# mikeoliphant/NeuralAudio

Measured on AMD Instinct MI355X. Metric: concurrent 48 kHz real-time streams + Msamples/s/GPU, NAM WaveNet Standard, higher is better.
Workload: dtype f32 (f16x3-split MFMA, f32 accumulate)

## Files before the change

### include/neuralaudio_amd.h

```cpp
#ifndef NEURALAUDIO_AMD_H
#define NEURALAUDIO_AMD_H

#include "NeuralAudioCApi.h"

#ifdef __cplusplus
extern "C" {
#endif

typedef struct NA_Batch NA_Batch;

NA_EXTERN const char* NA_GetLastError(void);
NA_EXTERN int NA_GetDeviceCount(void);
NA_EXTERN const char* NA_GetVersion(void);

NA_EXTERN NeuralModel* NA_CreateModelFromFileUtf8(NeuralModelLoader* loader, const char* utf8Path, int doPrewarm);
NA_EXTERN NeuralModel* NA_CreateModelFromString(NeuralModelLoader* loader, const char* jsonText, const char* extension, int doPrewarm);
NA_EXTERN void NA_SetDevice(NeuralModelLoader* loader, int device);
NA_EXTERN void NA_SetWaveNetMathMode(NeuralModelLoader* loader, int mathMode);
NA_EXTERN void NA_SetLSTMMathMode(NeuralModelLoader* loader, int mathMode);
NA_EXTERN void NA_SetCompositeModelLoadMode(NeuralModelLoader* loader, int loadMode);
NA_EXTERN int NA_IsQualityChangeRealtimeSafe(NeuralModel* model, float newQuality);
NA_EXTERN int NA_ProcessChecked(NeuralModel* model, float* input, float* output, size_t numSamples);
NA_EXTERN void NA_SetDefaultQualityScaleFactor(NeuralModelLoader* loader, float quality);
NA_EXTERN void NA_SetExternalSampleRate(NeuralModelLoader* loader, int sampleRate);
NA_EXTERN int NA_HasQualityScaling(NeuralModel* model);
NA_EXTERN float NA_GetQualityScaleFactor(NeuralModel* model);
NA_EXTERN void NA_SetQualityScaleFactor(NeuralModel* model, float quality);
NA_EXTERN int NA_GetReceptiveFieldSize(NeuralModel* model);
NA_EXTERN int NA_Prewarm(NeuralModel* model);
NA_EXTERN int NA_GetMetadata(NeuralModel* model, const char* fieldName, char* buf, int bufSize);
NA_EXTERN int NA_GetModelVersion(NeuralModel* model, char* buf, int bufSize);

NA_EXTERN NA_Batch* NA_BatchCreate(int device, void* hipStream);
NA_EXTERN void NA_BatchDestroy(NA_Batch* batch);
NA_EXTERN int NA_BatchAddStreams(NA_Batch* batch, NeuralModel* model, float quality, int count, int doPrewarm);
NA_EXTERN int NA_BatchRemoveStreams(NA_Batch* batch, int first, int count);
NA_EXTERN int NA_BatchReserveStreams(NA_Batch* batch, NeuralModel* model, int count, int doPrewarm);
NA_EXTERN int NA_BatchActivateStream(NA_Batch* batch, int stream, float quality);
NA_EXTERN int NA_BatchParkStream(NA_Batch* batch, int stream);
NA_EXTERN int NA_BatchIsParked(NA_Batch* batch, int stream);
NA_EXTERN int NA_BatchFindParked(NA_Batch* batch, NeuralModel* model);
NA_EXTERN int NA_BatchNumParked(NA_Batch* batch);
NA_EXTERN int NA_BatchEnableOutputStage(NA_Batch* batch);
NA_EXTERN int NA_BatchSetStreamGain(NA_Batch* batch, int stream, float gain, int rampSamples);
NA_EXTERN float NA_BatchGetStreamGain(NA_Batch* batch, int stream);
NA_EXTERN int NA_BatchHandover(NA_Batch* batch, int from, int to, float quality, int fadeSamples);
NA_EXTERN int NA_BatchHandoverRemaining(NA_Batch* batch, int stream);
NA_EXTERN int NA_BatchNumStreams(NA_Batch* batch);
NA_EXTERN int NA_BatchNumLiveStreams(NA_Batch* batch);
NA_EXTERN int NA_BatchIsLive(NA_Batch* batch, int stream);
NA_EXTERN int NA_BatchSetQuality(NA_Batch* batch, int stream, float quality);
NA_EXTERN int NA_BatchGetActiveSubModel(NA_Batch* batch, int stream);
NA_EXTERN int NA_BatchIsQualityChangeRealtimeSafe(NA_Batch* batch, int stream, float quality);
NA_EXTERN int NA_BatchPrewarm(NA_Batch* batch, int stream);
NA_EXTERN int NA_BatchProcess(NA_Batch* batch, const float* in, float* out, size_t n);
NA_EXTERN int NA_RegisterHostBuffer(void* ptr, size_t bytes);
NA_EXTERN int NA_UnregisterHostBuffer(void* ptr);
NA_EXTERN int NA_BatchSubmit(NA_Batch* batch, const float* in, size_t n);
NA_EXTERN int NA_BatchCollect(NA_Batch* batch, int ticket, float* out);
NA_EXTERN float* NA_BatchNextInput(NA_Batch* batch, size_t n);
NA_EXTERN const float* NA_BatchOutputView(NA_Batch* batch, int ticket);
NA_EXTERN int NA_BatchProcessDevice(NA_Batch* batch, const float* dIn, float* dOut, size_t n, long inStride, long outStride);
NA_EXTERN int NA_BatchWaitOutputs(NA_Batch* batch);
NA_EXTERN int NA_BatchSynchronize(NA_Batch* batch);
NA_EXTERN int NA_BatchSetWaitLimitMs(NA_Batch* batch, double milliseconds);
NA_EXTERN double NA_BatchGetWaitLimitMs(NA_Batch* batch);
NA_EXTERN int NA_BatchIsBroken(NA_Batch* batch);
NA_EXTERN void* NA_BatchGetHipStream(NA_Batch* batch);
NA_EXTERN int NA_BatchMarkTime(NA_Batch* batch, int which);
NA_EXTERN int NA_BatchWaitMarks(NA_Batch* batch);
NA_EXTERN float NA_BatchElapsedMs(NA_Batch* batch);
NA_EXTERN int NA_BatchUsesHalfLaunches(NA_Batch* batch);
NA_EXTERN int NA_BatchSetResidentLaunch(NA_Batch* batch, int on);
NA_EXTERN int NA_BatchUsesResidentLaunch(NA_Batch* batch);
NA_EXTERN double NA_BatchAlgorithmicBytesPerSample(NA_Batch* batch, int blockFrames);
NA_EXTERN double NA_BatchMacsPerSample(NA_Batch* batch);
NA_EXTERN double NA_BatchStateBytes(NA_Batch* batch);
NA_EXTERN int NA_BatchStreamPackFactor(NA_Batch* batch, int stream);
NA_EXTERN const char* NA_BatchStreamKernelName(NA_Batch* batch, int stream);
NA_EXTERN long long NA_BatchStreamSnapshotBytes(NA_Batch* batch, int stream);
NA_EXTERN long long NA_ModelSnapshotBytes(NeuralModel* model);
NA_EXTERN unsigned long long NA_ModelSnapshotFingerprint(NeuralModel* model);
NA_EXTERN int NA_BatchSaveStreams(NA_Batch* batch, const int* streams, int count, void* buf, size_t capacity, size_t* written);
NA_EXTERN int NA_BatchLoadStreams(NA_Batch* batch, const int* streams, int count, const void* buf, size_t bytes);
NA_EXTERN int NA_SaveModelState(NeuralModel* model, void* buf, size_t capacity, size_t* written);
NA_EXTERN int NA_LoadModelState(NeuralModel* model, const void* buf, size_t bytes);

typedef struct NA_MultiBatch NA_MultiBatch;
NA_EXTERN NA_MultiBatch* NA_MultiCreate(const int* devices, int numDevices);
NA_EXTERN void NA_MultiDestroy(NA_MultiBatch* multi);
NA_EXTERN int NA_MultiAddStreams(NA_MultiBatch* multi, NeuralModel* model, float quality, int count, int doPrewarm);
NA_EXTERN int NA_MultiCommit(NA_MultiBatch* multi);
NA_EXTERN int NA_MultiNumStreams(NA_MultiBatch* multi);
NA_EXTERN int NA_MultiNumShards(NA_MultiBatch* multi);
NA_EXTERN int NA_MultiShardRange(NA_MultiBatch* multi, int shard, int* begin, int* end, int* device);
NA_EXTERN int NA_MultiProcess(NA_MultiBatch* multi, const float* in, float* out, size_t n);
NA_EXTERN int NA_MultiSubmit(NA_MultiBatch* multi, const float* in, size_t n);
NA_EXTERN int NA_MultiCollect(NA_MultiBatch* multi, int ticket, float* out);
NA_EXTERN int NA_MultiSetQuality(NA_MultiBatch* multi, int stream, float quality);
NA_EXTERN int NA_MultiSetFanIn(NA_MultiBatch* multi, int mode);
NA_EXTERN const float* NA_MultiGatheredOutput(NA_MultiBatch* multi, int shard);
NA_EXTERN int NA_RcclAvailable(void);
NA_EXTERN int NA_ShardByCost(const double* cost, int n, int parts, int* bounds);
NA_EXTERN double NA_ModelStreamCost(NeuralModel* model, float quality);

NA_EXTERN int NA_ModelKernelInfo(NeuralModel* model, float quality, int streams, char* kernelBuf, int bufSize, float* inputLimit, int* rangeProven,
	int* weightsOk, int* packFactor);

NA_EXTERN float NA_BatchStreamInputLimit(NA_Batch* batch, int stream);
NA_EXTERN int NA_BatchStreamRangeEvents(NA_Batch* batch, int stream);

typedef struct NA_RenderJob
{
	NeuralModel* model;
	float quality;
	const float* input;
	float* output;
	size_t numSamples;
} NA_RenderJob;
typedef struct NA_RenderOptions
{
	size_t segmentSamples;
	size_t maxSamplesPerPass;
	double waitLimitMs;
} NA_RenderOptions;
typedef struct NA_RenderPlanInfo
{
	long long segments;
	int lead;
	long long segmentSamples;
	long long rowSamples;
	int passes;
	int streams;
	double estimatedMs;
	char kernel[64];
} NA_RenderPlanInfo;
NA_EXTERN int NA_RenderOffline(const NA_RenderJob* jobs, int numJobs, const NA_RenderOptions* opts);
NA_EXTERN int NA_RenderPlan(const NA_RenderJob* jobs, int numJobs, const NA_RenderOptions* opts, NA_RenderPlanInfo* info);

typedef struct NA_ResampleInfo {
	int externalRate, modelRate;
	int ticksExternal, ticksModel;
	int tapsUp, tapsDown;
	int quantum;
	int latencySamples;
	int prototypeLength;
} NA_ResampleInfo;
NA_EXTERN int NA_ResamplePlan(int externalRate, int modelRate, int quantum, NA_ResampleInfo* info);
NA_EXTERN int NA_ResamplePrototype(int externalRate, int modelRate, float* buf, int capacity);
NA_EXTERN long long NA_ResampleModelFrames(int externalRate, int modelRate, int quantum, long long externalSamples);
NA_EXTERN int NA_BatchSetResampling(NA_Batch* batch, int externalRate, int modelRate, int quantum, int maxFrames);
NA_EXTERN int NA_BatchGetResampleInfo(NA_Batch* batch, NA_ResampleInfo* info);
NA_EXTERN void NA_SetResampleToExternalRate(NeuralModelLoader* loader, int on);
NA_EXTERN int NA_GetProcessLatencySamples(NeuralModel* model);
NA_EXTERN int NA_GetModelProcessRate(NeuralModel* model);
NA_EXTERN int NA_RenderOfflineAtRate(const NA_RenderJob* jobs, int numJobs, const NA_RenderOptions* opts, int externalRate);
NA_EXTERN int NA_RenderPlanAtRate(const NA_RenderJob* jobs, int numJobs, const NA_RenderOptions* opts, int externalRate,
                                  NA_RenderPlanInfo* info, NA_ResampleInfo* resample);
NA_EXTERN int NA_MultiSetResampling(NA_MultiBatch* multi, int externalRate, int modelRate, int quantum, int maxFrames);
NA_EXTERN int NA_MultiGetResampleInfo(NA_MultiBatch* multi, NA_ResampleInfo* info);
#ifndef NA_RELEASE
NA_EXTERN int NA_DebugClassifyNam(const char* jsonText);
NA_EXTERN int NA_DebugPackedWeights(NeuralModel* model, int* packFactor, float* out, int capacity);
NA_EXTERN int NA_DebugSplitPlan(NeuralModel* model, int* stages, int stageCapacity, unsigned short* wsplit, long long wsplitCapacity, long long* wsplitCount);
NA_EXTERN void NA_DebugSetWaveNetSpec(int on);
NA_EXTERN int NA_DebugSetRecurrentQuadMin(int streams);
NA_EXTERN long long NA_DebugRecurrentQuadLaunches(void);
NA_EXTERN int NA_DebugRecurrentPlan(NeuralModel* model, int out[6]);
NA_EXTERN int NA_DebugRecurrentShapePlan(int cell, int hidden, int numLayers, int tailLayers, int tailWidth, int tailHistory, int rpl, int forceL2w, int out[6]);
NA_EXTERN long long NA_DebugSnapshotLaunches(void);
NA_EXTERN void NA_DebugSetRcclApi(int mode, int failSendAt, int rendezvousMs);
NA_EXTERN int NA_DebugStallDevice(NA_Batch* batch, double milliseconds);
NA_EXTERN long long NA_DebugDeviceResourceCalls(void);
NA_EXTERN int NA_DebugResampleTap(NA_Batch* batch, float* modelIn, float* modelOut, long long capacityPerRow, int* frames);
NA_EXTERN void NA_DebugSetRenderTap(float* modelIn, float* modelOut, long long capacity);
NA_EXTERN void NA_DebugSetTraceBuffer(void* deviceBuffer);
#endif

#ifdef __cplusplus
}
#endif
#endif
```

### neuralaudio_amd/capi.py

```python
import ctypes as C
import os

_HERE = os.path.dirname(os.path.abspath(__file__))
_SUFFIX = os.environ.get("NA_LIB_SUFFIX", "")
LIB_PATH = (os.path.join(os.path.dirname(_HERE), "tools", "variants", "libNeuralAudioCAPI%s.so" % _SUFFIX) if _SUFFIX
            else os.path.join(_HERE, "libNeuralAudioCAPI.so"))

LEGACY_SYMBOLS = [
    "CreateLoader", "DeleteLoader", "CreateModelFromFile", "DeleteModel", "SetLSTMLoadMode", "SetWaveNetLoadMode",
    "SetAudioInputLevelDBu", "SetDefaultMaxAudioBufferSize", "GetLoadMode", "IsStatic", "SetMaxAudioBufferSize",
    "GetRecommendedInputDBAdjustment", "GetRecommendedOutputDBAdjustment", "GetSampleRate", "Process",
]

NA_SYMBOLS = [
    "NA_GetLastError", "NA_GetDeviceCount", "NA_GetVersion", "NA_CreateModelFromFileUtf8", "NA_CreateModelFromString",
    "NA_SetDevice", "NA_SetDefaultQualityScaleFactor", "NA_SetExternalSampleRate", "NA_HasQualityScaling",
    "NA_GetQualityScaleFactor", "NA_SetQualityScaleFactor", "NA_GetReceptiveFieldSize", "NA_Prewarm", "NA_GetMetadata",
    "NA_GetModelVersion", "NA_BatchCreate", "NA_BatchDestroy", "NA_BatchAddStreams", "NA_BatchNumStreams",
    "NA_BatchSetQuality", "NA_BatchGetActiveSubModel", "NA_BatchPrewarm", "NA_BatchProcess", "NA_BatchProcessDevice",
    "NA_BatchSynchronize", "NA_BatchGetHipStream", "NA_BatchAlgorithmicBytesPerSample", "NA_BatchMacsPerSample",
    "NA_BatchStateBytes", "NA_BatchStreamPackFactor", "NA_BatchStreamKernelName", "NA_DebugSetTraceBuffer", "NA_DebugSetWaveNetSpec", "NA_DebugSetRecurrentQuadMin", "NA_DebugRecurrentQuadLaunches", "NA_RegisterHostBuffer", "NA_UnregisterHostBuffer", "NA_BatchStreamInputLimit", "NA_BatchRemoveStreams", "NA_MultiCreate", "NA_MultiDestroy", "NA_MultiAddStreams", "NA_MultiCommit", "NA_MultiNumStreams", "NA_MultiNumShards", "NA_MultiShardRange", "NA_MultiProcess", "NA_MultiSubmit", "NA_MultiCollect", "NA_MultiSetQuality", "NA_ShardByCost", "NA_ModelStreamCost", "NA_BatchNumLiveStreams", "NA_BatchIsLive", "NA_SetWaveNetMathMode", "NA_SetLSTMMathMode", "NA_SetCompositeModelLoadMode",
    "NA_IsQualityChangeRealtimeSafe", "NA_ProcessChecked", "NA_BatchSubmit", "NA_BatchCollect", "NA_BatchNextInput", "NA_BatchOutputView", "NA_BatchIsQualityChangeRealtimeSafe", "NA_DebugClassifyNam", "NA_DebugPackedWeights", "NA_DebugSplitPlan", "NA_ModelKernelInfo", "NA_BatchStreamRangeEvents", "NA_MultiSetFanIn", "NA_MultiGatheredOutput", "NA_RcclAvailable",
    "NA_BatchMarkTime", "NA_BatchWaitMarks", "NA_BatchElapsedMs", "NA_BatchUsesHalfLaunches", "NA_DebugSetRcclApi", "NA_BatchWaitOutputs", "NA_BatchUsesResidentLaunch", "NA_BatchSetResidentLaunch",
    "NA_BatchSetWaitLimitMs", "NA_BatchGetWaitLimitMs", "NA_BatchIsBroken", "NA_DebugStallDevice",
    "NA_RenderOffline", "NA_RenderPlan",
    "NA_BatchStreamSnapshotBytes", "NA_ModelSnapshotBytes", "NA_ModelSnapshotFingerprint", "NA_BatchSaveStreams", "NA_BatchLoadStreams",
    "NA_SaveModelState", "NA_LoadModelState", "NA_DebugSnapshotLaunches",
    "NA_ResamplePlan", "NA_ResamplePrototype", "NA_ResampleModelFrames", "NA_BatchSetResampling", "NA_BatchGetResampleInfo",
    "NA_SetResampleToExternalRate", "NA_GetProcessLatencySamples", "NA_GetModelProcessRate", "NA_DebugResampleTap",
    "NA_RenderOfflineAtRate", "NA_RenderPlanAtRate", "NA_DebugSetRenderTap", "NA_MultiSetResampling", "NA_MultiGetResampleInfo",
    "NA_BatchReserveStreams", "NA_BatchActivateStream", "NA_BatchParkStream", "NA_BatchIsParked", "NA_BatchFindParked", "NA_BatchNumParked",
    "NA_DebugDeviceResourceCalls", "NA_DebugRecurrentPlan", "NA_DebugRecurrentShapePlan",
    "NA_BatchEnableOutputStage", "NA_BatchSetStreamGain", "NA_BatchGetStreamGain", "NA_BatchHandover", "NA_BatchHandoverRemaining",
]


class NA_RenderJob(C.Structure):
    _fields_ = [("model", C.c_void_p), ("quality", C.c_float), ("input", C.POINTER(C.c_float)), ("output", C.POINTER(C.c_float)),
                ("numSamples", C.c_size_t)]


class NA_RenderOptions(C.Structure):
    _fields_ = [("segmentSamples", C.c_size_t), ("maxSamplesPerPass", C.c_size_t), ("waitLimitMs", C.c_double)]


class NA_RenderPlanInfo(C.Structure):
    _fields_ = [("segments", C.c_longlong), ("lead", C.c_int), ("segmentSamples", C.c_longlong), ("rowSamples", C.c_longlong),
                ("passes", C.c_int), ("streams", C.c_int), ("estimatedMs", C.c_double), ("kernel", C.c_char * 64)]


class NA_ResampleInfo(C.Structure):
    _fields_ = [("externalRate", C.c_int), ("modelRate", C.c_int), ("ticksExternal", C.c_int), ("ticksModel", C.c_int),
                ("tapsUp", C.c_int), ("tapsDown", C.c_int), ("quantum", C.c_int), ("latencySamples", C.c_int),
                ("prototypeLength", C.c_int)]

_lib = None


def load_library():
    global _lib
    if _lib is not None:
        return _lib
    if not os.path.exists(LIB_PATH):
        raise OSError("libNeuralAudioCAPI.so not found at %s -- build it with `python -c 'import __graft_entry__ as g; "
                      "g.build()'` (there is no CPU fallback)" % LIB_PATH)
    lib = C.CDLL(LIB_PATH, mode=C.RTLD_GLOBAL)
    fp = C.POINTER(C.c_float)
    vp = C.c_void_p
    sig = {
        "CreateLoader": (vp, []),
        "DeleteLoader": (None, [vp]),
        "CreateModelFromFile": (vp, [vp, C.c_wchar_p]),
        "DeleteModel": (None, [vp]),
        "SetLSTMLoadMode": (None, [vp, C.c_int]),
        "SetWaveNetLoadMode": (None, [vp, C.c_int]),
        "SetAudioInputLevelDBu": (None, [vp, C.c_float]),
        "SetDefaultMaxAudioBufferSize": (None, [vp, C.c_int]),
        "GetLoadMode": (C.c_int, [vp]),
        "IsStatic": (C.c_bool, [vp]),
        "SetMaxAudioBufferSize": (None, [vp, C.c_int]),
        "GetRecommendedInputDBAdjustment": (C.c_float, [vp]),
        "GetRecommendedOutputDBAdjustment": (C.c_float, [vp]),
        "GetSampleRate": (C.c_float, [vp]),
        "Process": (None, [vp, fp, fp, C.c_size_t]),
        "NA_GetLastError": (C.c_char_p, []),
        "NA_GetDeviceCount": (C.c_int, []),
        "NA_GetVersion": (C.c_char_p, []),
        "NA_CreateModelFromFileUtf8": (vp, [vp, C.c_char_p, C.c_int]),
        "NA_CreateModelFromString": (vp, [vp, C.c_char_p, C.c_char_p, C.c_int]),
        "NA_SetDevice": (None, [vp, C.c_int]),
        "NA_SetDefaultQualityScaleFactor": (None, [vp, C.c_float]),
        "NA_SetExternalSampleRate": (None, [vp, C.c_int]),
        "NA_HasQualityScaling": (C.c_int, [vp]),
        "NA_GetQualityScaleFactor": (C.c_float, [vp]),
        "NA_SetQualityScaleFactor": (None, [vp, C.c_float]),
        "NA_GetReceptiveFieldSize": (C.c_int, [vp]),
        "NA_Prewarm": (C.c_int, [vp]),
        "NA_GetMetadata": (C.c_int, [vp, C.c_char_p, C.c_char_p, C.c_int]),
        "NA_GetModelVersion": (C.c_int, [vp, C.c_char_p, C.c_int]),
        "NA_BatchCreate": (vp, [C.c_int, vp]),
        "NA_BatchDestroy": (None, [vp]),
        "NA_BatchAddStreams": (C.c_int, [vp, vp, C.c_float, C.c_int, C.c_int]),
        "NA_BatchNumStreams": (C.c_int, [vp]),
        "NA_BatchSetQuality": (C.c_int, [vp, C.c_int, C.c_float]),
        "NA_BatchGetActiveSubModel": (C.c_int, [vp, C.c_int]),
        "NA_BatchPrewarm": (C.c_int, [vp, C.c_int]),
        "NA_BatchProcess": (C.c_int, [vp, fp, fp, C.c_size_t]),
        "NA_BatchProcessDevice": (C.c_int, [vp, vp, vp, C.c_size_t, C.c_long, C.c_long]),
        "NA_BatchSynchronize": (C.c_int, [vp]),
        "NA_BatchGetHipStream": (vp, [vp]),
        "NA_BatchMarkTime": (C.c_int, [vp, C.c_int]),
        "NA_BatchWaitMarks": (C.c_int, [vp]),
        "NA_BatchElapsedMs": (C.c_float, [vp]),
        "NA_BatchUsesHalfLaunches": (C.c_int, [vp]),
        "NA_BatchUsesResidentLaunch": (C.c_int, [vp]),
        "NA_BatchSetResidentLaunch": (C.c_int, [vp, C.c_int]),
        "NA_BatchWaitOutputs": (C.c_int, [vp]),
        "NA_BatchSetWaitLimitMs": (C.c_int, [vp, C.c_double]),
        "NA_BatchGetWaitLimitMs": (C.c_double, [vp]),
        "NA_BatchIsBroken": (C.c_int, [vp]),
        "NA_DebugStallDevice": (C.c_int, [vp, C.c_double]),
        "NA_BatchAlgorithmicBytesPerSample": (C.c_double, [vp, C.c_int]),
        "NA_BatchMacsPerSample": (C.c_double, [vp]),
        "NA_BatchStateBytes": (C.c_double, [vp]),
        "NA_BatchStreamPackFactor": (C.c_int, [vp, C.c_int]),
        "NA_BatchStreamKernelName": (C.c_char_p, [vp, C.c_int]),
        "NA_DebugSetTraceBuffer": (None, [vp]),
        "NA_DebugSetWaveNetSpec": (None, [C.c_int]),
        "NA_DebugSetRcclApi": (None, [C.c_int, C.c_int, C.c_int]),
        "NA_DebugSetRecurrentQuadMin": (C.c_int, [C.c_int]),
        "NA_DebugRecurrentQuadLaunches": (C.c_longlong, []),
        "NA_RegisterHostBuffer": (C.c_int, [C.c_void_p, C.c_size_t]),
        "NA_UnregisterHostBuffer": (C.c_int, [C.c_void_p]),
        "NA_BatchStreamInputLimit": (C.c_float, [vp, C.c_int]),
        "NA_BatchRemoveStreams": (C.c_int, [vp, C.c_int, C.c_int]),
        "NA_BatchReserveStreams": (C.c_int, [vp, vp, C.c_int, C.c_int]),
        "NA_BatchActivateStream": (C.c_int, [vp, C.c_int, C.c_float]),
        "NA_BatchParkStream": (C.c_int, [vp, C.c_int]),
        "NA_BatchIsParked": (C.c_int, [vp, C.c_int]),
        "NA_BatchFindParked": (C.c_int, [vp, vp]),
        "NA_BatchNumParked": (C.c_int, [vp]),
        "NA_DebugDeviceResourceCalls": (C.c_longlong, []),
        "NA_BatchEnableOutputStage": (C.c_int, [vp]),
        "NA_BatchSetStreamGain": (C.c_int, [vp, C.c_int, C.c_float, C.c_int]),
        "NA_BatchGetStreamGain": (C.c_float, [vp, C.c_int]),
        "NA_BatchHandover": (C.c_int, [vp, C.c_int, C.c_int, C.c_float, C.c_int]),
        "NA_BatchHandoverRemaining": (C.c_int, [vp, C.c_int]),
        "NA_DebugRecurrentPlan": (C.c_int, [vp, C.POINTER(C.c_int)]),
        "NA_DebugRecurrentShapePlan": (C.c_int, [C.c_int] * 8 + [C.POINTER(C.c_int)]),
        "NA_MultiCreate": (vp, [C.POINTER(C.c_int), C.c_int]),
        "NA_MultiDestroy": (None, [vp]),
        "NA_MultiAddStreams": (C.c_int, [vp, vp, C.c_float, C.c_int, C.c_int]),
        "NA_MultiCommit": (C.c_int, [vp]),
        "NA_MultiNumStreams": (C.c_int, [vp]),
        "NA_MultiNumShards": (C.c_int, [vp]),
        "NA_MultiShardRange": (C.c_int, [vp, C.c_int, C.POINTER(C.c_int), C.POINTER(C.c_int), C.POINTER(C.c_int)]),
        "NA_MultiProcess": (C.c_int, [vp, C.POINTER(C.c_float), C.POINTER(C.c_float), C.c_size_t]),
        "NA_MultiSubmit": (C.c_int, [vp, C.POINTER(C.c_float), C.c_size_t]),
        "NA_MultiCollect": (C.c_int, [vp, C.c_int, C.POINTER(C.c_float)]),
        "NA_MultiSetQuality": (C.c_int, [vp, C.c_int, C.c_float]),
        "NA_ShardByCost": (C.c_int, [C.POINTER(C.c_double), C.c_int, C.c_int, C.POINTER(C.c_int)]),
        "NA_ModelStreamCost": (C.c_double, [vp, C.c_float]),
        "NA_BatchStreamRangeEvents": (C.c_int, [vp, C.c_int]),
        "NA_MultiSetFanIn": (C.c_int, [vp, C.c_int]),
        "NA_MultiGatheredOutput": (vp, [vp, C.c_int]),
        "NA_RcclAvailable": (C.c_int, []),
        "NA_ModelKernelInfo": (C.c_int, [vp, C.c_float, C.c_int, C.c_char_p, C.c_int, fp, C.POINTER(C.c_int), C.POINTER(C.c_int), C.POINTER(C.c_int)]),
        "NA_BatchNumLiveStreams": (C.c_int, [vp]),
        "NA_BatchIsLive": (C.c_int, [vp, C.c_int]),
        "NA_SetWaveNetMathMode": (None, [vp, C.c_int]),
        "NA_SetLSTMMathMode": (None, [vp, C.c_int]),
        "NA_SetCompositeModelLoadMode": (None, [vp, C.c_int]),
        "NA_IsQualityChangeRealtimeSafe": (C.c_int, [vp, C.c_float]),
        "NA_ProcessChecked": (C.c_int, [vp, fp, fp, C.c_size_t]),
        "NA_BatchSubmit": (C.c_int, [vp, fp, C.c_size_t]),
        "NA_BatchCollect": (C.c_int, [vp, C.c_int, fp]),
        "NA_BatchNextInput": (fp, [vp, C.c_size_t]),
        "NA_BatchOutputView": (fp, [vp, C.c_int]),
        "NA_BatchIsQualityChangeRealtimeSafe": (C.c_int, [vp, C.c_int, C.c_float]),
        "NA_DebugClassifyNam": (C.c_int, [C.c_char_p]),
        "NA_DebugPackedWeights": (C.c_int, [vp, C.POINTER(C.c_int), C.POINTER(C.c_float), C.c_int]),
        "NA_RenderOffline": (C.c_int, [C.POINTER(NA_RenderJob), C.c_int, C.POINTER(NA_RenderOptions)]),
        "NA_RenderPlan": (C.c_int, [C.POINTER(NA_RenderJob), C.c_int, C.POINTER(NA_RenderOptions), C.POINTER(NA_RenderPlanInfo)]),
        "NA_BatchStreamSnapshotBytes": (C.c_longlong, [vp, C.c_int]),
        "NA_ModelSnapshotBytes": (C.c_longlong, [vp]),
        "NA_ModelSnapshotFingerprint": (C.c_ulonglong, [vp]),
        "NA_BatchSaveStreams": (C.c_int, [vp, C.POINTER(C.c_int), C.c_int, vp, C.c_size_t, C.POINTER(C.c_size_t)]),
        "NA_BatchLoadStreams": (C.c_int, [vp, C.POINTER(C.c_int), C.c_int, vp, C.c_size_t]),
        "NA_SaveModelState": (C.c_int, [vp, vp, C.c_size_t, C.POINTER(C.c_size_t)]),
        "NA_LoadModelState": (C.c_int, [vp, vp, C.c_size_t]),
        "NA_DebugSnapshotLaunches": (C.c_longlong, []),
        "NA_ResamplePlan": (C.c_int, [C.c_int, C.c_int, C.c_int, C.POINTER(NA_ResampleInfo)]),
        "NA_ResamplePrototype": (C.c_int, [C.c_int, C.c_int, fp, C.c_int]),
        "NA_ResampleModelFrames": (C.c_longlong, [C.c_int, C.c_int, C.c_int, C.c_longlong]),
        "NA_BatchSetResampling": (C.c_int, [vp, C.c_int, C.c_int, C.c_int, C.c_int]),
        "NA_BatchGetResampleInfo": (C.c_int, [vp, C.POINTER(NA_ResampleInfo)]),
        "NA_SetResampleToExternalRate": (None, [vp, C.c_int]),
        "NA_GetProcessLatencySamples": (C.c_int, [vp]),
        "NA_GetModelProcessRate": (C.c_int, [vp]),
        "NA_DebugResampleTap": (C.c_int, [vp, fp, fp, C.c_longlong, C.POINTER(C.c_int)]),
        "NA_RenderOfflineAtRate": (C.c_int, [C.POINTER(NA_RenderJob), C.c_int, C.POINTER(NA_RenderOptions), C.c_int]),
        "NA_RenderPlanAtRate": (C.c_int, [C.POINTER(NA_RenderJob), C.c_int, C.POINTER(NA_RenderOptions), C.c_int, C.POINTER(NA_RenderPlanInfo),
                                          C.POINTER(NA_ResampleInfo)]),
        "NA_DebugSetRenderTap": (None, [fp, fp, C.c_longlong]),
        "NA_MultiSetResampling": (C.c_int, [vp, C.c_int, C.c_int, C.c_int, C.c_int]),
        "NA_MultiGetResampleInfo": (C.c_int, [vp, C.POINTER(NA_ResampleInfo)]),
        "NA_DebugSplitPlan": (C.c_int, [vp, C.POINTER(C.c_int), C.c_int, C.POINTER(C.c_ushort), C.c_longlong, C.POINTER(C.c_longlong)]),
    }
    for name, (res, args) in sig.items():
        try:
            fn = getattr(lib, name)
        except AttributeError:
            if os.environ.get("NA_LIB_SUFFIX") and name.startswith("NA_"):
                continue
            raise
        fn.restype = res
        fn.argtypes = args
    _lib = lib
    return lib


def last_error():
    return load_library().NA_GetLastError().decode("utf-8", "replace")


def device_count():
    return int(load_library().NA_GetDeviceCount())
```

### neuralaudio_amd/csrc/capi.cpp

```cpp
#include <cstring>
#include <cwchar>
#include <string>

#include "neuralaudio_amd.h"
#include "multi_gpu.h"
#include "offline_render.h"
#include "resample.h"
#include "stream_snapshot.h"
#include "neural_model_impl.h"
#include "lstm_launch.h"
#include "wavenet_launch.h"
#include "wavenet_plan.h"
#include "tuning.h"

struct NeuralModel
{
	NeuralAudio::NeuralModel* model;
};

struct NeuralModelLoader
{
	NeuralAudio::NeuralModelLoader* loader;
};

struct NA_Batch
{
	na::GpuBatch* batch;
};

struct NA_MultiBatch
{
	na::MultiGpuBatch* multi;
};

namespace
{
	thread_local std::string g_lastError;

	void SetError(const char* what) { g_lastError = what ? what : "unknown error"; }

	template <typename F>
	int Guard(F&& f)
	{
		try
		{
			f();
			return 0;
		}
		catch (const std::exception& e)
		{
			SetError(e.what());
		}
		catch (...)
		{
			SetError("unknown exception");
		}
		return -1;
	}

	std::string WideToUtf8(const wchar_t* w)
	{
		std::string out;
		if (!w) return out;
		for (; *w; ++w)
		{
			unsigned long cp = (unsigned long)*w;
			if (sizeof(wchar_t) == 2 && cp >= 0xD800 && cp <= 0xDBFF && w[1] >= 0xDC00 && w[1] <= 0xDFFF)
			{
				cp = 0x10000 + ((cp - 0xD800) << 10) + ((unsigned long)w[1] - 0xDC00);
				++w;
			}
			if (cp < 0x80) out.push_back((char)cp);
			else if (cp < 0x800)
			{
				out.push_back((char)(0xC0 | (cp >> 6)));
				out.push_back((char)(0x80 | (cp & 0x3F)));
			}
			else if (cp < 0x10000)
			{
				out.push_back((char)(0xE0 | (cp >> 12)));
				out.push_back((char)(0x80 | ((cp >> 6) & 0x3F)));
				out.push_back((char)(0x80 | (cp & 0x3F)));
			}
			else
			{
				out.push_back((char)(0xF0 | (cp >> 18)));
				out.push_back((char)(0x80 | ((cp >> 12) & 0x3F)));
				out.push_back((char)(0x80 | ((cp >> 6) & 0x3F)));
				out.push_back((char)(0x80 | (cp & 0x3F)));
			}
		}
		return out;
	}

	NeuralModel* Wrap(NeuralAudio::NeuralModel* m)
	{
		if (!m) return nullptr;
		NeuralModel* w = new NeuralModel();
		w->model = m;
		return w;
	}

	int CopyOut(const std::string& s, char* buf, int bufSize)
	{
		if (buf && bufSize > 0)
		{
			const size_t n = std::min((size_t)bufSize - 1, s.size());
			memcpy(buf, s.data(), n);
			buf[n] = 0;
		}
		return (int)s.size();
	}
}

extern "C" {


NeuralModelLoader* CreateLoader(void)
{
	NeuralModelLoader* loader = nullptr;
	Guard([&] {
		loader = new NeuralModelLoader();
		loader->loader = new NeuralAudio::NeuralModelLoader();
	});
	return loader;
}

void DeleteLoader(NeuralModelLoader* loader)
{
	if (!loader) return;
	delete loader->loader;
	delete loader;
}

NeuralModel* CreateModelFromFile(NeuralModelLoader* loader, const wchar_t* modelPath)
{
	NeuralModel* result = nullptr;
	Guard([&] {
		if (!loader || !modelPath) throw std::runtime_error("CreateModelFromFile: null argument");
		NeuralAudio::NeuralModel* m = loader->loader->CreateFromFile(std::filesystem::path(WideToUtf8(modelPath)));
		if (!m) SetError("model file not found or not supported");
		result = Wrap(m);
	});
	return result;
}

void DeleteModel(NeuralModel* model)
{
	if (!model) return;
	delete model->model;
	delete model;
}

void SetLSTMLoadMode(NeuralModelLoader* loader, int loadMode)
{
	if (loader) loader->loader->SetLSTMLoadMode((NeuralAudio::EModelLoadMode)loadMode);
}

void SetWaveNetLoadMode(NeuralModelLoader* loader, int loadMode)
{
	if (loader) loader->loader->SetWaveNetLoadMode((NeuralAudio::EModelLoadMode)loadMode);
}

void SetAudioInputLevelDBu(NeuralModelLoader* loader, float audioDBu)
{
	if (loader) loader->loader->SetAudioInputLevelDBu(audioDBu);
}

void SetDefaultMaxAudioBufferSize(NeuralModelLoader* loader, int maxSize)
{
	if (loader) loader->loader->SetDefaultMaxAudioBufferSize(maxSize);
}

int GetLoadMode(NeuralModel* model) { return model ? (int)model->model->GetLoadMode() : 0; }

bool IsStatic(NeuralModel* model) { return model ? model->model->IsStatic() : false; }

void SetMaxAudioBufferSize(NeuralModel* model, int maxSize)
{
	if (model) model->model->SetMaxAudioBufferSize(maxSize);
}

float GetRecommendedInputDBAdjustment(NeuralModel* model) { return model ? model->model->GetRecommendedInputDBAdjustment() : 0.0f; }

float GetRecommendedOutputDBAdjustment(NeuralModel* model) { return model ? model->model->GetRecommendedOutputDBAdjustment() : 0.0f; }

float GetSampleRate(NeuralModel* model) { return model ? model->model->GetSampleRate() : 0.0f; }

void Process(NeuralModel* model, float* input, float* output, size_t numSamples)
{
	(void)NA_ProcessChecked(model, input, output, numSamples);
}


const char* NA_GetLastError(void) { return g_lastError.c_str(); }

int NA_GetDeviceCount(void) { return na::VisibleDeviceCount(); }

const char* NA_GetVersion(void) { return "neuralaudio_amd 0.1.0 (gfx950)"; }

NeuralModel* NA_CreateModelFromFileUtf8(NeuralModelLoader* loader, const char* utf8Path, int doPrewarm)
{
	NeuralModel* result = nullptr;
	Guard([&] {
		if (!loader || !utf8Path) throw std::runtime_error("NA_CreateModelFromFileUtf8: null argument");
		NeuralAudio::NeuralModel* m = loader->loader->CreateFromFile(std::filesystem::path(std::string(utf8Path)), doPrewarm != 0);
		if (!m) SetError("model file not found or not supported");
		result = Wrap(m);
	});
	return result;
}

NeuralModel* NA_CreateModelFromString(NeuralModelLoader* loader, const char* jsonText, const char* extension, int doPrewarm)
{
	NeuralModel* result = nullptr;
	Guard([&] {
		if (!loader || !jsonText || !extension) throw std::runtime_error("NA_CreateModelFromString: null argument");
		NeuralAudio::NeuralModel* m = loader->loader->CreateFromString(jsonText, std::filesystem::path(std::string(extension)), doPrewarm != 0);
		if (!m) SetError("model not supported");
		result = Wrap(m);
	});
	return result;
}

int NA_ProcessChecked(NeuralModel* model, float* input, float* output, size_t numSamples)
{
	if (!model || !output)
	{
		SetError("Process: null argument");
		return -1;
	}
	const int rc = Guard([&] { model->model->Process(input, output, numSamples); });
	if (rc != 0) memset(output, 0, numSamples * sizeof(float));
	return rc;
}

void NA_SetWaveNetMathMode(NeuralModelLoader* loader, int mathMode)
{
	if (loader) loader->loader->SetWaveNetMathMode(mathMode == 1 ? NeuralAudio::EMathMode::StdMath : NeuralAudio::EMathMode::FastMath);
}

void NA_SetLSTMMathMode(NeuralModelLoader* loader, int mathMode)
{
	if (loader) loader->loader->SetLSTMMathMode(mathMode == 1 ? NeuralAudio::EMathMode::StdMath : NeuralAudio::EMathMode::FastMath);
}

void NA_SetCompositeModelLoadMode(NeuralModelLoader* loader, int loadMode)
{
	if (loader) loader->loader->SetCompositeModelLoadMode(loadMode == 1 ? NeuralAudio::ECompositeModelLoadMode::OnDemand : NeuralAudio::ECompositeModelLoadMode::LoadAll);
}

int NA_IsQualityChangeRealtimeSafe(NeuralModel* model, float newQuality)
{
	return (model && model->model->IsQualityChangeRealtimeSafe(newQuality)) ? 1 : 0;
}

#ifndef NA_RELEASE
int NA_DebugClassifyNam(const char* jsonText)
{
	int r = -1;
	Guard([&] {
		const na::Json j = na::Json::Parse(jsonText ? jsonText : "");
		const std::string v = (j.IsObject() && j.Contains("version") && j.At("version").IsString()) ? j.At("version").AsString() : "";
		r = (na::NAMIsA2(v) ? 1 : 0) | (na::NAMIsA2Standard(j) ? 2 : 0);
	});
	return r;
}
#endif

#ifndef NA_RELEASE
int NA_DebugPackedWeights(NeuralModel* model, int* packFactor, float* out, int capacity)
{
	int r = -1;
	Guard([&] {
		NeuralAudio::GpuModel* gm = model ? dynamic_cast<NeuralAudio::GpuModel*>(model->model) : nullptr;
		if (!gm) throw std::runtime_error("NA_DebugPackedWeights: not a model of this library");
		const auto& lm = gm->GetLoadedModel();
		if (lm->subModels.size() != 1 || lm->subModels[0].desc->kind != na::MODEL_WAVENET)
		{
			if (packFactor) *packFactor = 1;
			r = 0;
			return;
		}
		const na::WaveNetDesc& wn = lm->subModels[0].desc->wavenet;
		const int P = na::WaveNetPackFactor(wn);
		if (packFactor) *packFactor = P;
		if (P < 2)
		{
			r = 0;
			return;
		}
		const bool dense = na::Tuning::Get().wnDense != 0 && na::WaveNetPackCanBeDense(wn, P);
		const na::WaveNetDesc v = na::PackWaveNetDesc(wn, P, dense);
		na::ValidateWaveNetDesc(v);
		const na::WaveNetPlan plan = na::BuildPackedWaveNetPlan(wn, P, dense);
		if (plan.pack != P || plan.splitFastT != 2) throw std::runtime_error("NA_DebugPackedWeights: the packed plan is not a fast split-kernel plan");
		r = (int)v.weights.size();
		if (out)
			for (int i = 0; i < r && i < capacity; i++) out[i] = v.weights[(size_t)i];
	});
	return r;
}
#endif

#ifndef NA_RELEASE
int NA_DebugSplitPlan(NeuralModel* model, int* stages, int stageCapacity, unsigned short* wsplit, long long wsplitCapacity, long long* wsplitCount)
{
	int r = -1;
	Guard([&] {
		NeuralAudio::GpuModel* gm = model ? dynamic_cast<NeuralAudio::GpuModel*>(model->model) : nullptr;
		if (!gm) throw std::runtime_error("NA_DebugSplitPlan: not a model of this library");
		const auto& lm = gm->GetLoadedModel();
		if (lm->subModels.size() != 1 || lm->subModels[0].desc->kind != na::MODEL_WAVENET) throw std::runtime_error("NA_DebugSplitPlan: not a WaveNet");
		const na::WaveNetPlan plan = na::BuildWaveNetPlan(lm->subModels[0].desc->wavenet, true);
		static_assert(sizeof(na::WnSplitStage) == 16 * sizeof(int), "16 ints per stage");
		r = (int)plan.sstages.size();
		if (stages) memcpy(stages, plan.sstages.data(), sizeof(na::WnSplitStage) * (size_t)std::min(r, stageCapacity));
		if (wsplitCount) *wsplitCount = (long long)plan.wsplit.size();
		if (wsplit) memcpy(wsplit, plan.wsplit.data(), sizeof(uint16_t) * (size_t)std::min<long long>((long long)plan.wsplit.size(), wsplitCapacity));
	});
	return r;
}
#endif

#ifndef NA_RELEASE
int NA_DebugRecurrentShapePlan(int cell, int hidden, int numLayers, int tailLayers, int tailWidth, int tailHistory, int rpl, int forceL2w, int out[6])
{
	if (!out || (cell != 0 && cell != 1) || hidden < 1 || numLayers < 0 || tailLayers < 0) return -1;
	const na::RecurrentPlan p = na::RecurrentWavePlan(cell == 1 ? na::LSTM_CELL_GRU : na::LSTM_CELL_LSTM, hidden, numLayers, tailLayers, tailWidth, tailHistory, true, rpl, forceL2w);
	out[0] = p.runs; out[1] = p.waves; out[2] = p.rowsPerLane; out[3] = p.l2w; out[4] = p.headInLoop; out[5] = (int)p.ldsBytes;
	return na::RecurrentWaveShape(hidden, numLayers, tailLayers > 0 ? tailWidth : 0, tailLayers > 0 ? tailHistory : 0) ? 1 : 0;
}
#endif

#ifndef NA_RELEASE
int NA_DebugRecurrentPlan(NeuralModel* model, int out[6])
{
	int r = -1;
	Guard([&] {
		NeuralAudio::GpuModel* gm = model ? dynamic_cast<NeuralAudio::GpuModel*>(model->model) : nullptr;
		if (!gm || !out) throw std::runtime_error("NA_DebugRecurrentPlan: not a model of this library");
		const auto& lm = gm->GetLoadedModel();
		if (lm->subModels.size() != 1 || lm->subModels[0].desc->kind != na::MODEL_LSTM) throw std::runtime_error("NA_DebugRecurrentPlan: not a recurrent model");
		const na::LSTMDesc& d = lm->subModels[0].desc->lstm;
		int tailWidth = 0, tailHistory = 0;
		na::RecurrentTailDims(d, tailWidth, tailHistory);
		const na::RecurrentPlan p = na::RecurrentWavePlan(d.cell == na::CELL_GRU ? na::LSTM_CELL_GRU : na::LSTM_CELL_LSTM, d.hiddenSize, d.numLayers, (int)d.tail.size(),
			tailWidth, tailHistory);
		out[0] = p.runs; out[1] = p.waves; out[2] = p.rowsPerLane; out[3] = p.l2w; out[4] = p.headInLoop; out[5] = (int)p.ldsBytes;
		r = 0;
	});
	return r;
}
#endif

void NA_SetDevice(NeuralModelLoader* loader, int device)
{
	if (loader) loader->loader->SetDevice(device);
}

void NA_SetDefaultQualityScaleFactor(NeuralModelLoader* loader, float quality)
{
	if (loader) loader->loader->SetDefaultQualityScaleFactor(quality);
}

void NA_SetExternalSampleRate(NeuralModelLoader* loader, int sampleRate)
{
	if (loader) loader->loader->SetExternalSampleRate(sampleRate);
}

int NA_HasQualityScaling(NeuralModel* model) { return (model && model->model->HasQualityScaling()) ? 1 : 0; }

float NA_GetQualityScaleFactor(NeuralModel* model) { return model ? model->model->GetQualityScaleFactor() : 1.0f; }

void NA_SetQualityScaleFactor(NeuralModel* model, float quality)
{
	if (model) Guard([&] { model->model->SetQualityScaleFactor(quality); });
}

int NA_GetReceptiveFieldSize(NeuralModel* model) { return model ? model->model->GetReceptiveFieldSize() : -1; }

int NA_Prewarm(NeuralModel* model)
{
	if (!model) return -1;
	return Guard([&] { model->model->Prewarm(); });
}

int NA_GetMetadata(NeuralModel* model, const char* fieldName, char* buf, int bufSize)
{
	if (!model || !fieldName) return -1;
	return CopyOut(model->model->GetMetadata(fieldName), buf, bufSize);
}

int NA_GetModelVersion(NeuralModel* model, char* buf, int bufSize)
{
	if (!model) return -1;
	return CopyOut(model->model->GetModelVersion(), buf, bufSize);
}

NA_Batch* NA_BatchCreate(int device, void* hipStream)
{
	NA_Batch* b = nullptr;
	Guard([&] {
		na::GpuBatch* gb = new na::GpuBatch(device, reinterpret_cast<hipStream_t>(hipStream));
		b = new NA_Batch();
		b->batch = gb;
	});
	return b;
}

void NA_BatchDestroy(NA_Batch* batch)
{
	if (!batch) return;
	Guard([&] { delete batch->batch; });
	delete batch;
}

int NA_BatchAddStreams(NA_Batch* batch, NeuralModel* model, float quality, int count, int doPrewarm)
{
	int first = -1;
	const int rc = Guard([&] {
		if (!batch || !model || count < 1) throw std::runtime_error("NA_BatchAddStreams: bad argument");
		NeuralAudio::GpuModel* gm = dynamic_cast<NeuralAudio::GpuModel*>(model->model);
		if (!gm) throw std::runtime_error("NA_BatchAddStreams: model was not created by this library");
		first = batch->batch->AddStreams(gm->GetLoadedModel(), quality, count, doPrewarm != 0, gm->IsOnDemand());
	});
	return rc == 0 ? first : -1;
}

int NA_BatchReserveStreams(NA_Batch* batch, NeuralModel* model, int count, int doPrewarm)
{
	int first = -1;
	const int rc = Guard([&] {
		if (!batch) throw std::runtime_error("NA_BatchReserveStreams: null batch (NA_BatchCreate fails where no HIP device is visible: there is no CPU fallback)");
		if (!model || count < 1) throw std::runtime_error("NA_BatchReserveStreams: bad argument");
		NeuralAudio::GpuModel* gm = dynamic_cast<NeuralAudio::GpuModel*>(model->model);
		if (!gm) throw std::runtime_error("NA_BatchReserveStreams: model was not created by this library");
		first = batch->batch->ReserveStreams(gm->GetLoadedModel(), count, doPrewarm != 0);
	});
	return rc == 0 ? first : -1;
}

int NA_BatchActivateStream(NA_Batch* batch, int stream, float quality)
{
	return Guard([&] {
		if (!batch) throw std::runtime_error("NA_BatchActivateStream: null batch (NA_BatchCreate fails where no HIP device is visible: there is no CPU fallback)");
		batch->batch->ActivateStream(stream, quality);
	});
}

int NA_BatchParkStream(NA_Batch* batch, int stream)
{
	return Guard([&] {
		if (!batch) throw std::runtime_error("NA_BatchParkStream: null batch (NA_BatchCreate fails where no HIP device is visible: there is no CPU fallback)");
		batch->batch->ParkStream(stream);
	});
}

int NA_BatchIsParked(NA_Batch* batch, int stream) { return (batch && batch->batch->IsParked(stream)) ? 1 : 0; }

int NA_BatchFindParked(NA_Batch* batch, NeuralModel* model)
{
	NeuralAudio::GpuModel* gm = (batch && model) ? dynamic_cast<NeuralAudio::GpuModel*>(model->model) : nullptr;
	return gm ? batch->batch->FindParked(gm->GetLoadedModel().get()) : -1;
}

int NA_BatchNumParked(NA_Batch* batch) { return batch ? batch->batch->NumParked() : -1; }

int NA_BatchEnableOutputStage(NA_Batch* batch)
{
	return Guard([&] {
		if (!batch) throw std::runtime_error("NA_BatchEnableOutputStage: null batch (NA_BatchCreate fails where no HIP device is visible: there is no CPU fallback)");
		batch->batch->EnableOutputStage();
	});
}

int NA_BatchSetStreamGain(NA_Batch* batch, int stream, float gain, int rampSamples)
{
	return Guard([&] {
		if (!batch) throw std::runtime_error("NA_BatchSetStreamGain: null batch (NA_BatchCreate fails where no HIP device is visible: there is no CPU fallback)");
		batch->batch->SetStreamGain(stream, gain, rampSamples);
	});
}

float NA_BatchGetStreamGain(NA_Batch* batch, int stream)
{
	float gain = -1.0f;
	const int rc = Guard([&] {
		if (!batch) throw std::runtime_error("NA_BatchGetStreamGain: null batch (NA_BatchCreate fails where no HIP device is visible: there is no CPU fallback)");
		gain = batch->batch->GetStreamGain(stream);
	});
	return rc == 0 ? gain : -1.0f;
}

int NA_BatchHandover(NA_Batch* batch, int from, int to, float quality, int fadeSamples)
{
	return Guard([&] {
		if (!batch) throw std::runtime_error("NA_BatchHandover: null batch (NA_BatchCreate fails where no HIP device is visible: there is no CPU fallback)");
		batch->batch->Handover(from, to, quality, fadeSamples);
	});
}

int NA_BatchHandoverRemaining(NA_Batch* batch, int stream)
{
	int left = 0;
	const int rc = Guard([&] {
		if (!batch) throw std::runtime_error("NA_BatchHandoverRemaining: null batch (NA_BatchCreate fails where no HIP device is visible: there is no CPU fallback)");
		left = batch->batch->HandoverRemaining(stream);
	});
	return rc == 0 ? left : -1;
}

#ifndef NA_RELEASE
long long NA_DebugDeviceResourceCalls(void) { return na::DeviceResourceCalls(); }
#endif

int NA_BatchNumStreams(NA_Batch* batch) { return batch ? batch->batch->NumStreams() : -1; }

int NA_BatchNumLiveStreams(NA_Batch* batch) { return batch ? batch->batch->NumLiveStreams() : -1; }

int NA_BatchIsLive(NA_Batch* batch, int stream) { return (batch && batch->batch->IsLive(stream)) ? 1 : 0; }

int NA_BatchRemoveStreams(NA_Batch* batch, int first, int count)
{
	if (!batch) return -1;
	return Guard([&] { batch->batch->RemoveStreams(first, count); });
}

namespace
{
	NeuralAudio::GpuModel* OwnModel(NeuralModel* model, const char* who)
	{
		NeuralAudio::GpuModel* gm = model ? dynamic_cast<NeuralAudio::GpuModel*>(model->model) : nullptr;
		if (!gm) throw std::runtime_error(std::string(who) + ": model is null or was not created by this library");
		return gm;
	}
}

long long NA_BatchStreamSnapshotBytes(NA_Batch* batch, int stream)
{
	long long n = -1;
	Guard([&] {
		if (!batch) throw std::runtime_error("NA_BatchStreamSnapshotBytes: null batch");
		n = (long long)batch->batch->StreamSnapshotBytes(stream);
	});
	return n;
}

long long NA_ModelSnapshotBytes(NeuralModel* model)
{
	long long n = -1;
	Guard([&] { n = (long long)na::SnapshotBytes(*OwnModel(model, "NA_ModelSnapshotBytes")->GetLoadedModel()); });
	return n;
}

unsigned long long NA_ModelSnapshotFingerprint(NeuralModel* model)
{
	unsigned long long f = 0;
	Guard([&] { f = na::ModelFingerprint(*OwnModel(model, "NA_ModelSnapshotFingerprint")->GetLoadedModel()); });
	return f;
}

int NA_BatchSaveStreams(NA_Batch* batch, const int* streams, int count, void* buf, size_t capacity, size_t* written)
{
	if (written) *written = 0;
	return Guard([&] {
		if (!batch) throw std::runtime_error("NA_BatchSaveStreams: null batch (a batch needs a HIP device: there is no host-side stream state)");
		const size_t need = batch->batch->SaveStreams(streams, count, buf, capacity);
		if (written) *written = need;
		if (need > capacity) throw std::runtime_error("NA_BatchSaveStreams: buffer too small: " + std::to_string(need) + " bytes needed, " + std::to_string(capacity) + " given");
	});
}

int NA_BatchLoadStreams(NA_Batch* batch, const int* streams, int count, const void* buf, size_t bytes)
{
	return Guard([&] {
		if (!batch) throw std::runtime_error("NA_BatchLoadStreams: null batch (a batch needs a HIP device: there is no host-side stream state)");
		batch->batch->LoadStreams(streams, count, buf, bytes);
	});
}

int NA_SaveModelState(NeuralModel* model, void* buf, size_t capacity, size_t* written)
{
	if (written) *written = 0;
	return Guard([&] {
		const size_t need = OwnModel(model, "NA_SaveModelState")->SaveState(buf, capacity);
		if (written) *written = need;
		if (need > capacity) throw std::runtime_error("NA_SaveModelState: buffer too small: " + std::to_string(need) + " bytes needed, " + std::to_string(capacity) + " given");
	});
}

int NA_LoadModelState(NeuralModel* model, const void* buf, size_t bytes)
{
	return Guard([&] { OwnModel(model, "NA_LoadModelState")->LoadState(buf, bytes); });
}

#ifndef NA_RELEASE
long long NA_DebugSnapshotLaunches(void) { return na::SnapshotKernelLaunches(); }
#endif

int NA_BatchSetQuality(NA_Batch* batch, int stream, float quality)
{
	if (!batch) return -1;
	return Guard([&] { batch->batch->SetQuality(stream, quality); });
}

int NA_BatchIsQualityChangeRealtimeSafe(NA_Batch* batch, int stream, float quality)
{
	int safe = 0;
	if (!batch) return 0;
	Guard([&] { safe = batch->batch->IsQualityChangeRealtimeSafe(stream, quality) ? 1 : 0; });
	return safe;
}

int NA_BatchGetActiveSubModel(NA_Batch* batch, int stream)
{
	int idx = -1;
	if (!batch) return -1;
	Guard([&] { idx = batch->batch->GetActiveSubModel(stream); });
	return idx;
}

int NA_BatchPrewarm(NA_Batch* batch, int stream)
{
	if (!batch) return -1;
	return Guard([&] {
		if (stream >= 0) batch->batch->Prewarm(stream);
		else
			for (int s = 0; s < batch->batch->NumStreams(); s++)
				if (!batch->batch->IsParked(s)) batch->batch->Prewarm(s);
	});
}

int NA_BatchProcess(NA_Batch* batch, const float* in, float* out, size_t n)
{
	if (!batch || !out)
	{
		SetError("NA_BatchProcess: null argument");
		return -1;
	}
	const int rc = Guard([&] { batch->batch->ProcessHost(in, out, n); });
	if (rc != 0) memset(out, 0, (size_t)batch->batch->NumStreams() * n * sizeof(float));
	return rc;
}

int NA_RegisterHostBuffer(void* ptr, size_t bytes)
{
	return Guard([&] {
		std::string error;
		if (!na::RegisterHostBuffer(ptr, bytes, error)) throw std::runtime_error(error);
	});
}

int NA_UnregisterHostBuffer(void* ptr) { return na::UnregisterHostBuffer(ptr) ? 0 : -1; }

int NA_BatchSubmit(NA_Batch* batch, const float* in, size_t n)
{
	int ticket = -1;
	if (!batch) return -1;
	const int rc = Guard([&] { ticket = batch->batch->Submit(in, n); });
	return rc == 0 ? ticket : -1;
}

int NA_BatchCollect(NA_Batch* batch, int ticket, float* out)
{
	if (!batch) return -1;
	return Guard([&] { batch->batch->Collect(ticket, out); });
}

float* NA_BatchNextInput(NA_Batch* batch, size_t n)
{
	float* ptr = nullptr;
	if (!batch) return nullptr;
	Guard([&] { ptr = batch->batch->NextInput(n); });
	return ptr;
}

const float* NA_BatchOutputView(NA_Batch* batch, int ticket)
{
	const float* ptr = nullptr;
	if (!batch) return nullptr;
	Guard([&] { ptr = batch->batch->OutputView(ticket); });
	return ptr;
}

int NA_BatchProcessDevice(NA_Batch* batch, const float* dIn, float* dOut, size_t n, long inStride, long outStride)
{
	if (!batch) return -1;
	return Guard([&] { batch->batch->ProcessDevice(dIn, dOut, n, inStride, outStride); });
}

int NA_BatchSynchronize(NA_Batch* batch)
{
	if (!batch) return -1;
	return Guard([&] { batch->batch->Synchronize(); });
}

int NA_BatchSetWaitLimitMs(NA_Batch* batch, double milliseconds)
{
	if (!batch) return -1;
	batch->batch->SetWaitLimitMs(milliseconds);
	return 0;
}

double NA_BatchGetWaitLimitMs(NA_Batch* batch) { return batch ? batch->batch->GetWaitLimitMs() : 0.0; }

int NA_BatchIsBroken(NA_Batch* batch) { return (batch && batch->batch->IsBroken()) ? 1 : 0; }

#ifndef NA_RELEASE
int NA_DebugStallDevice(NA_Batch* batch, double milliseconds)
{
	if (!batch) return -1;
	return Guard([&] { batch->batch->DebugStallDevice(milliseconds); });
}
#endif

void* NA_BatchGetHipStream(NA_Batch* batch) { return batch ? reinterpret_cast<void*>(batch->batch->GetStream()) : nullptr; }

int NA_BatchMarkTime(NA_Batch* batch, int which)
{
	if (!batch) return -1;
	return Guard([&] { batch->batch->MarkTime(which); });
}

int NA_BatchWaitMarks(NA_Batch* batch)
{
	if (!batch) return -1;
	return Guard([&] { batch->batch->WaitMarks(); });
}

float NA_BatchElapsedMs(NA_Batch* batch)
{
	if (!batch) return -1.0f;
	float ms = -1.0f;
	return Guard([&] { ms = batch->batch->ElapsedMs(); }) == 0 ? ms : -1.0f;
}

int NA_BatchUsesHalfLaunches(NA_Batch* batch) { return batch && batch->batch->UsesHalfLaunches() ? 1 : 0; }
int NA_BatchSetResidentLaunch(NA_Batch* batch, int on)
{
	if (!batch) return -1;
	return Guard([&] { batch->batch->SetResidentLaunch(on != 0); });
}
int NA_BatchUsesResidentLaunch(NA_Batch* batch) { return batch && batch->batch->UsesResidentLaunch() ? 1 : 0; }

int NA_BatchWaitOutputs(NA_Batch* batch)
{
	if (!batch) return -1;
	return Guard([&] { batch->batch->WaitOutputs(); });
}

double NA_BatchAlgorithmicBytesPerSample(NA_Batch* batch, int blockFrames)
{
	return batch ? batch->batch->AlgorithmicBytesPerSample(blockFrames) : 0.0;
}

double NA_BatchMacsPerSample(NA_Batch* batch) { return batch ? batch->batch->MacsPerSample() : 0.0; }

float NA_BatchStreamInputLimit(NA_Batch* batch, int stream)
{
	try { return batch ? batch->batch->StreamInputLimit(stream) : 0.0f; }
	catch (...) { return 0.0f; }
}

int NA_ShardByCost(const double* cost, int n, int parts, int* bounds)
{
	return Guard([&] {
		if (!cost && n > 0) throw std::runtime_error("NA_ShardByCost: bad argument");
		if (!bounds) throw std::runtime_error("NA_ShardByCost: bad argument");
		const std::vector<int> b = na::ShardByCost(cost, n, parts);
		for (size_t i = 0; i < b.size(); i++) bounds[i] = b[i];
	});
}

double NA_ModelStreamCost(NeuralModel* model, float quality)
{
	double c = -1.0;
	Guard([&] {
		NeuralAudio::GpuModel* gm = model ? dynamic_cast<NeuralAudio::GpuModel*>(model->model) : nullptr;
		if (!gm) throw std::runtime_error("NA_ModelStreamCost: model was not created by this library");
		c = na::EstimateStreamCost(*gm->GetLoadedModel(), quality);
	});
	return c;
}

int NA_ModelKernelInfo(NeuralModel* model, float quality, int streams, char* kernelBuf, int bufSize, float* inputLimit, int* rangeProven, int* weightsOk, int* packFactor)
{
	int r = -1;
	Guard([&] {
		NeuralAudio::GpuModel* gm = model ? dynamic_cast<NeuralAudio::GpuModel*>(model->model) : nullptr;
		if (!gm) throw std::runtime_error("NA_ModelKernelInfo: model was not created by this library");
		const na::ModelKernelInfo info = na::PredictModelKernel(*gm->GetLoadedModel(), quality, streams);
		if (kernelBuf && bufSize > 0)
		{
			strncpy(kernelBuf, info.kernel, (size_t)bufSize - 1);
			kernelBuf[bufSize - 1] = 0;
		}
		if (inputLimit) *inputLimit = info.inputLimit;
		if (rangeProven) *rangeProven = info.rangeProven ? 1 : 0;
		if (weightsOk) *weightsOk = info.weightsOk ? 1 : 0;
		if (packFactor) *packFactor = info.pack;
		r = 0;
	});
	return r;
}

int NA_BatchStreamRangeEvents(NA_Batch* b, int stream)
{
	int r = -1;
	Guard([&] {
		if (!b) throw std::runtime_error("NA_BatchStreamRangeEvents: null batch");
		r = b->batch->StreamRangeEvents(stream);
	});
	return r;
}

NA_MultiBatch* NA_MultiCreate(const int* devices, int numDevices)
{
	NA_MultiBatch* mb = nullptr;
	Guard([&] {
		if (!devices || numDevices < 1) throw std::runtime_error("NA_MultiCreate: bad argument");
		na::MultiGpuBatch* m = new na::MultiGpuBatch(std::vector<int>(devices, devices + numDevices));
		mb = new NA_MultiBatch{ m };
	});
	return mb;
}

void NA_MultiDestroy(NA_MultiBatch* mb)
{
	if (!mb) return;
	Guard([&] { delete mb->multi; });
	delete mb;
}

int NA_MultiAddStreams(NA_MultiBatch* mb, NeuralModel* model, float quality, int count, int doPrewarm)
{
	int first = -1;
	const int rc = Guard([&] {
		NeuralAudio::GpuModel* gm = (mb && model) ? dynamic_cast<NeuralAudio::GpuModel*>(model->model) : nullptr;
		if (!gm || count < 1) throw std::runtime_error("NA_MultiAddStreams: bad argument");
		first = mb->multi->AddStreams(gm->GetLoadedModel(), quality, count, doPrewarm != 0, gm->IsOnDemand());
	});
	return rc == 0 ? first : -1;
}

int NA_MultiCommit(NA_MultiBatch* mb)
{
	if (!mb) return -1;
	return Guard([&] { mb->multi->Commit(); });
}

int NA_MultiNumStreams(NA_MultiBatch* mb) { return mb ? mb->multi->NumStreams() : -1; }
int NA_MultiNumShards(NA_MultiBatch* mb) { return mb ? mb->multi->NumShards() : -1; }

int NA_MultiShardRange(NA_MultiBatch* mb, int shard, int* begin, int* end, int* device)
{
	if (!mb) return -1;
	return Guard([&] {
		int b = 0, e = 0, d = 0;
		mb->multi->ShardRange(shard, b, e, d);
		if (begin) *begin = b;
		if (end) *end = e;
		if (device) *device = d;
	});
}

int NA_MultiProcess(NA_MultiBatch* mb, const float* in, float* out, size_t n)
{
	if (!mb || !in || !out) return -1;
	return Guard([&] { mb->multi->Process(in, out, n); });
}

int NA_MultiSubmit(NA_MultiBatch* mb, const float* in, size_t n)
{
	int ticket = -1;
	if (!mb || !in) return -1;
	const int rc = Guard([&] { ticket = mb->multi->Submit(in, n); });
	return rc == 0 ? ticket : -1;
}

int NA_MultiCollect(NA_MultiBatch* mb, int ticket, float* out)
{
	if (!mb) return -1;
	return Guard([&] { mb->multi->Collect(ticket, out); });
}

int NA_MultiSetFanIn(NA_MultiBatch* mb, int mode)
{
	if (!mb) return -1;
	return Guard([&] {
		if (mode != 0 && mode != 1) throw std::runtime_error("NA_MultiSetFanIn: mode must be 0 (host rows) or 1 (RCCL)");
		mb->multi->SetFanIn(mode == 1 ? na::MultiGpuBatch::FanIn::Rccl : na::MultiGpuBatch::FanIn::HostRows);
	});
}

const float* NA_MultiGatheredOutput(NA_MultiBatch* mb, int shard)
{
	const float* p = nullptr;
	if (!mb) return nullptr;
	Guard([&] { p = mb->multi->GatheredOutput(shard); });
	return p;
}

int NA_RcclAvailable(void)
{
	int ok = 0;
	Guard([&] {
		std::string error;
		if (na::rccl::Load(error) == nullptr) throw std::runtime_error(error);
		ok = 1;
	});
	return ok;
}

#ifndef NA_RELEASE
void NA_DebugSetRcclApi(int mode, int failSendAt, int rendezvousMs)
{
	na::rccl::LoopbackConfigure(failSendAt, rendezvousMs);
	na::rccl::SetOverride(mode == 1 ? na::rccl::LoopbackApi() : nullptr);
}
#endif

int NA_MultiSetQuality(NA_MultiBatch* mb, int stream, float quality)
{
	if (!mb) return -1;
	return Guard([&] { mb->multi->SetQuality(stream, quality); });
}

#ifndef NA_RELEASE
void NA_DebugSetWaveNetSpec(int on) { na::SetWaveNetSpecEnabled(on != 0); }
#endif

#ifndef NA_RELEASE
int NA_DebugSetRecurrentQuadMin(int streams) { return na::SetRecurrentQuadMinStreams(streams); }
#endif

#ifndef NA_RELEASE
long long NA_DebugRecurrentQuadLaunches(void) { return (long long)na::RecurrentQuadLaunches(); }
#endif

#ifndef NA_RELEASE
void NA_DebugSetTraceBuffer(void* deviceBuffer) { na::SetWaveNetTraceBuffer(reinterpret_cast<long long*>(deviceBuffer)); }
#endif

double NA_BatchStateBytes(NA_Batch* batch) { return batch ? (double)batch->batch->StateBytes() : 0.0; }

const char* NA_BatchStreamKernelName(NA_Batch* batch, int stream)
{
	try { return batch ? batch->batch->StreamKernelName(stream) : ""; }
	catch (...) { return ""; }
}

int NA_BatchStreamPackFactor(NA_Batch* batch, int stream)
{
	try { return batch ? batch->batch->StreamPackFactor(stream) : 0; }
	catch (...) { return 0; }
}


namespace
{
	int RenderJobs(const NA_RenderJob* jobs, int numJobs, const NA_RenderOptions* opts, std::vector<na::RenderJobDesc>& out, na::RenderOptionsDesc& o)
	{
		if (!jobs) throw std::runtime_error("offline render: jobs is NULL");
		if (numJobs <= 0) throw std::runtime_error("offline render: numJobs must be >= 1");
		int device = -1;
		out.clear();
		for (int j = 0; j < numJobs; j++)
		{
			const NA_RenderJob& job = jobs[j];
			NeuralAudio::GpuModel* gm = job.model ? dynamic_cast<NeuralAudio::GpuModel*>(job.model->model) : nullptr;
			if (!job.model) throw std::runtime_error("offline render: job " + std::to_string(j) + " has a NULL model");
			if (!gm) throw std::runtime_error("offline render: job " + std::to_string(j) + ": model was not created by this library");
			if (device < 0) device = gm->GetDevice();
			else if (gm->GetDevice() != device) throw std::runtime_error("offline render: the jobs' models are on different devices");
			na::RenderJobDesc d;
			d.model = gm->GetLoadedModel();
			d.quality = job.quality;
			d.input = job.input;
			d.output = job.output;
			d.numSamples = job.numSamples;
			out.push_back(d);
		}
		o = na::RenderOptionsDesc();
		if (opts)
		{
			o.segmentSamples = opts->segmentSamples;
			o.maxSamplesPerPass = opts->maxSamplesPerPass;
			o.waitLimitMs = opts->waitLimitMs;
		}
		return device;
	}
}

namespace
{
	void FillRenderPlanInfo(const na::RenderPlan& p, const std::string& kernel, NA_RenderPlanInfo* info)
	{
		memset(info, 0, sizeof(*info));
		info->segments = p.segments;
		info->lead = p.lead;
		info->segmentSamples = p.stride > 0 ? p.stride : 0;
		info->rowSamples = p.rowSamples;
		info->passes = p.passes;
		info->streams = p.rows;
		info->estimatedMs = p.estimatedMs;
		strncpy(info->kernel, kernel.c_str(), sizeof(info->kernel) - 1);
	}
}

int NA_RenderOffline(const NA_RenderJob* jobs, int numJobs, const NA_RenderOptions* opts)
{
	return Guard([&] {
		std::vector<na::RenderJobDesc> js;
		na::RenderOptionsDesc o;
		const int device = RenderJobs(jobs, numJobs, opts, js, o);
		na::RenderOffline(js, o, device);
	});
}

int NA_RenderPlan(const NA_RenderJob* jobs, int numJobs, const NA_RenderOptions* opts, NA_RenderPlanInfo* info)
{
	return Guard([&] {
		if (!info) throw std::runtime_error("NA_RenderPlan: info is NULL");
		std::vector<na::RenderJobDesc> js;
		na::RenderOptionsDesc o;
		const int device = RenderJobs(jobs, numJobs, opts, js, o);
		std::string kernel;
		FillRenderPlanInfo(na::PlanOfflineRenderOn(js, o, device, &kernel), kernel, info);
	});
}


namespace
{
	void FillResampleInfo(const na::ResamplePlan& p, NA_ResampleInfo* info);
}

int NA_RenderOfflineAtRate(const NA_RenderJob* jobs, int numJobs, const NA_RenderOptions* opts, int externalRate)
{
	return Guard([&] {
		std::vector<na::RenderJobDesc> js;
		na::RenderOptionsDesc o;
		const int device = RenderJobs(jobs, numJobs, opts, js, o);
		na::RenderOfflineAtRate(js, o, device, externalRate);
	});
}

int NA_RenderPlanAtRate(const NA_RenderJob* jobs, int numJobs, const NA_RenderOptions* opts, int externalRate, NA_RenderPlanInfo* info, NA_ResampleInfo* resample)
{
	return Guard([&] {
		if (!info) throw std::runtime_error("NA_RenderPlanAtRate: info is NULL");
		std::vector<na::RenderJobDesc> js;
		na::RenderOptionsDesc o;
		const int device = RenderJobs(jobs, numJobs, opts, js, o);
		std::string kernel;
		na::ResamplePlan first;
		FillRenderPlanInfo(na::PlanOfflineRenderAtRateOn(js, o, device, externalRate, &kernel, &first), kernel, info);
		if (resample) FillResampleInfo(first, resample);
	});
}

#ifndef NA_RELEASE
void NA_DebugSetRenderTap(float* modelIn, float* modelOut, long long capacity) { na::SetRenderTap(modelIn, modelOut, capacity); }
#endif

int NA_MultiSetResampling(NA_MultiBatch* mb, int externalRate, int modelRate, int quantum, int maxFrames)
{
	return Guard([&] {
		if (!mb) throw std::runtime_error("NA_MultiSetResampling: null multi batch");
		mb->multi->SetResampling(externalRate, modelRate, quantum, maxFrames);
	});
}

int NA_MultiGetResampleInfo(NA_MultiBatch* mb, NA_ResampleInfo* info)
{
	return Guard([&] {
		if (!mb || !info) throw std::runtime_error("NA_MultiGetResampleInfo: null argument");
		FillResampleInfo(mb->multi->ResamplingPlan(), info);
	});
}

namespace
{
	void FillResampleInfo(const na::ResamplePlan& p, NA_ResampleInfo* info)
	{
		memset(info, 0, sizeof(*info));
		info->externalRate = p.externalRate;
		info->modelRate = p.modelRate;
		info->ticksExternal = p.te;
		info->ticksModel = p.tm;
		info->tapsUp = p.tapsUp;
		info->tapsDown = p.tapsDown;
		info->quantum = p.quantum;
		info->latencySamples = p.latency;
		info->prototypeLength = p.K;
	}
}

int NA_ResamplePlan(int externalRate, int modelRate, int quantum, NA_ResampleInfo* info)
{
	return Guard([&] {
		if (!info) throw std::runtime_error("NA_ResamplePlan: info is NULL");
		FillResampleInfo(na::PlanResampling(externalRate, modelRate, quantum), info);
	});
}

int NA_ResamplePrototype(int externalRate, int modelRate, float* buf, int capacity)
{
	int k = -1;
	Guard([&] {
		const na::ResamplePlan p = na::PlanResampling(externalRate, modelRate, 0);
		const std::vector<float> h = na::ResamplePrototype(p);
		if (buf && capacity > 0) memcpy(buf, h.data(), sizeof(float) * std::min((size_t)capacity, h.size()));
		k = (int)h.size();
	});
	return k;
}

long long NA_ResampleModelFrames(int externalRate, int modelRate, int quantum, long long externalSamples)
{
	long long frames = -1;
	Guard([&] {
		if (externalSamples < 0) throw std::runtime_error("NA_ResampleModelFrames: negative sample count");
		frames = na::PlanResampling(externalRate, modelRate, quantum).ModelFrames(externalSamples);
	});
	return frames;
}

int NA_BatchSetResampling(NA_Batch* batch, int externalRate, int modelRate, int quantum, int maxFrames)
{
	return Guard([&] {
		if (!batch) throw std::runtime_error("NA_BatchSetResampling: null batch");
		batch->batch->SetResampling(externalRate, modelRate, quantum, maxFrames);
	});
}

int NA_BatchGetResampleInfo(NA_Batch* batch, NA_ResampleInfo* info)
{
	return Guard([&] {
		if (!batch || !info) throw std::runtime_error("NA_BatchGetResampleInfo: null argument");
		FillResampleInfo(batch->batch->ResamplingPlan(), info);
	});
}

void NA_SetResampleToExternalRate(NeuralModelLoader* loader, int on)
{
	if (loader) loader->loader->SetResampleToExternalRate(on != 0);
}

int NA_GetProcessLatencySamples(NeuralModel* model)
{
	NeuralAudio::GpuModel* gm = model ? dynamic_cast<NeuralAudio::GpuModel*>(model->model) : nullptr;
	return gm ? gm->GetProcessLatencySamples() : 0;
}

int NA_GetModelProcessRate(NeuralModel* model)
{
	NeuralAudio::GpuModel* gm = model ? dynamic_cast<NeuralAudio::GpuModel*>(model->model) : nullptr;
	return gm ? gm->GetLoadedModel()->ProcessRate() : 0;
}

#ifndef NA_RELEASE
int NA_DebugResampleTap(NA_Batch* batch, float* modelIn, float* modelOut, long long capacityPerRow, int* frames)
{
	return Guard([&] {
		if (!batch) throw std::runtime_error("NA_DebugResampleTap: null batch");
		const int f = batch->batch->DebugResampleTap(modelIn, modelOut, capacityPerRow);
		if (frames) *frames = f;
	});
}
#endif

}
```

### neuralaudio_amd/csrc/wavenet_launch.h

```cpp
#pragma once

#include <cstring>
#include <vector>

#include <hip/hip_runtime_api.h>

#include "device_resources.h"
#include "tuning.h"
#include "wavenet_dev.h"

namespace na
{
	constexpr int WN_FRAME_MAX_GROUPS = 8;
	struct WnFrameGroup
	{
		const WnModelDev* model;
		float* state;
		const int* slots;
		const int* rows;
		int numStreams, slot0, row0;
		int pack;
	};
	hipError_t LaunchWaveNetFrameFused(const WnFrameGroup* groups, int numGroups, const float* in, float* out, long inStride, long outStride, int n,
		hipStream_t stream);

	hipError_t LaunchWaveNetSplitFused(const WnFrameGroup* groups, int numGroups, const float* in, float* out, long inStride, long outStride, int n,
		hipStream_t stream, int sharing = 1);

	constexpr int WN_SHARING_BEYOND_CACHE = 1 << 16;
	inline int WnBeyondCacheBit(size_t stateBytes)
	{
		const Tuning& t = Tuning::Get();
		return (!t.wnNtOff && stateBytes > ((size_t)t.wnNtFromMB << 20)) ? WN_SHARING_BEYOND_CACHE : 0;
	}
	hipError_t LaunchWaveNetSpecFused(const WnFrameGroup* groups, int numGroups, const float* in, float* out, long inStride, long outStride, int n,
		hipStream_t stream, int sharing = 1);
	hipError_t LaunchStallKernel(double ms, hipStream_t stream);
	struct WnLaunchTable
	{
		struct Entry
		{
			void* dev = nullptr;
			std::vector<char> host;
		};
		std::vector<Entry> entries;
		unsigned long generation = 0;
		bool prepareOnly = false;
		WnLaunchTable() = default;
		WnLaunchTable(const WnLaunchTable&) = delete;
		WnLaunchTable& operator=(const WnLaunchTable&) = delete;
		~WnLaunchTable() { Clear(); }
		void Clear()
		{
			for (Entry& e : entries)
				if (e.dev) (void)CountedHipFree(e.dev);
			entries.clear();
		}
		void NewGeneration(unsigned long g)
		{
			if (g != generation) Clear();
			generation = g;
		}
		hipError_t Ensure(const void* fresh, size_t bytes, hipStream_t stream, const void** dev)
		{
			for (const Entry& e : entries)
				if (e.host.size() == bytes && memcmp(e.host.data(), fresh, bytes) == 0)
				{
					*dev = e.dev;
					return hipSuccess;
				}
			hipStreamCaptureStatus capturing = hipStreamCaptureStatusNone;
			(void)hipStreamIsCapturing(stream, &capturing);
			if (capturing != hipStreamCaptureStatusNone) return hipErrorStreamCaptureUnsupported;
			if (entries.size() >= 16) Clear();
			Entry e;
			hipError_t err = CountedHipMalloc(&e.dev, bytes);
			if (err != hipSuccess) return err;
			err = hipMemcpy(e.dev, fresh, bytes, hipMemcpyHostToDevice);
			if (err != hipSuccess)
			{
				(void)CountedHipFree(e.dev);
				return err;
			}
			e.host.assign(static_cast<const char*>(fresh), static_cast<const char*>(fresh) + bytes);
			*dev = e.dev;
			entries.push_back(std::move(e));
			return hipSuccess;
		}
	};
	hipError_t LaunchWaveNetSpecTable(const WnFrameGroup* groups, int numGroups, const float* in, float* out, long inStride, long outStride, int n,
		hipStream_t stream, WnLaunchTable& table);

	constexpr int RESIDENT_RING = 64;
	struct ResidentCmd
	{
		const float* in;
		float* out;
		long inStride, outStride;
		unsigned long long seq;
		unsigned long long check;
		unsigned long long pad[2];
	};
#ifdef __HIPCC__
	__host__ __device__
#endif
	inline unsigned long long ResidentCmdCheck(unsigned long long in, unsigned long long out, unsigned long long inStride, unsigned long long outStride, unsigned long long seq)
	{
		return seq * 0x9E3779B97F4A7C15ull + in * 0xC2B2AE3D27D4EB4Full + out * 0x165667B19E3779F9ull + inStride * 0xD6E8FEB86659FD93ull + outStride * 0xFF51AFD7ED558CCDull + 1ull;
	}
	struct ResidentCtrl
	{
		unsigned long long exitAfter;
		unsigned long long pad0[7];
		ResidentCmd cmd[RESIDENT_RING];
	};
	struct ResidentStatus
	{
		unsigned long long completed;
		unsigned long long pad1[7];
	};
	static_assert(sizeof(ResidentCmd) == 64 && sizeof(ResidentCtrl) == 64 + 64 * RESIDENT_RING && sizeof(ResidentStatus) == 64, "command ring layout");
	struct ResidentArgs
	{
		const ResidentCtrl* ctrl;
		ResidentStatus* status;
		unsigned* doneCount;
		unsigned* wgDone;
		unsigned long long base;
		int numBlocks;
		unsigned idleTicks;
		unsigned startDelay;
	};
	hipError_t LaunchWaveNetSpecResident(const WnFrameGroup* groups, int numGroups, int n, const ResidentArgs& ra, hipStream_t stream, int* gridOut);
	int WaveNetSpecResidentGrid(const WnFrameGroup* groups, int numGroups, int n);

	bool WaveNetSpecEnabled();
	void SetWaveNetSpecEnabled(bool on);
	int WaveNetSpecArchId(const WnSplitStage* stages, int nstages, int stateF4, int wsplitQuads);

	hipError_t LaunchWaveNetGeneric(const WnPrewarmLayer* layers, int numLayers, const float* weights, const int* ringOffF4, const int* ringFrames,
		const int* ringG, int nrings, int stateF4, int maxChannels, float headScale, float condLimit, bool saturate, float* state, const int* slots, const int* rows,
		int numStreams, int slot0, int row0, const float* in, float* out, long inStride, long outStride, int n, hipStream_t stream);

	hipError_t LaunchWaveNetFrame(const WnModelDev& m, float* state, const int* slots, const int* rows, int numStreams, const float* in,
		float* out, long inStride, long outStride, int n, hipStream_t stream, int slot0 = 0, int row0 = 0);

	void SetWaveNetTraceBuffer(long long* deviceBuffer);
	long long* GetWaveNetTraceBuffer();

	hipError_t LaunchWaveNetPrewarmColumns(const WnPrewarmLayer* layers, int numLayers, const float* weights, float* cols,
		hipStream_t stream);

	hipError_t LaunchWaveNetFillRings(float* state, int stateF4, const int* slots, int numStreams, int numRings, const int* ringOffF4,
		const int* ringFrames, const int* ringG, const float* cols, hipStream_t stream, bool splitFormat, const int* sub = nullptr, int pack = 1,
		bool zero = false);

	hipError_t LaunchWaveNetRearm(float* state, int stateF4, const int* entries, int numEntries, int numRings, const int* ringOffF4,
		const int* ringFrames, const int* ringG, const float* cols, hipStream_t stream, bool splitFormat, int pack);
}
```

### neuralaudio_amd/csrc/wavenet_spec_impl.h

```cpp
#pragma once

#include <algorithm>
#include <atomic>
#include <cstddef>
#include <cstdlib>

#include <hip/hip_runtime.h>

#include "device_once.h"
#include <cstring>
#include <type_traits>
#include <vector>

#include "tuning.h"
#include "wavenet_split_dev.h"

namespace na
{
	namespace spk
	{
		using namespace sp;

#ifndef NA_SPK_NT_DIL
#define NA_SPK_NT_DIL 256
#endif
#ifndef NA_SPK_NT_LD
#define NA_SPK_NT_LD 0
#endif
#ifndef NA_SPK_NT_ST
#define NA_SPK_NT_ST 0
#endif
#ifndef NA_SPK_DELAY
#define NA_SPK_DELAY 0
#endif
#ifndef NA_SPK_AUX2
#define NA_SPK_AUX2 0
#endif
		typedef __attribute__((address_space(3))) char* LdsPtr;
		__device__ __forceinline__ u32x4 LdsRead16(unsigned addr) { return *reinterpret_cast<__attribute__((address_space(3))) const u32x4*>((LdsPtr)(size_t)addr); }
		__device__ __forceinline__ u32x2 LdsRead8(unsigned addr) { return *reinterpret_cast<__attribute__((address_space(3))) const u32x2*>((LdsPtr)(size_t)addr); }
		__device__ __forceinline__ void LdsWrite16(unsigned addr, u32x4 v) { *reinterpret_cast<__attribute__((address_space(3))) u32x4*>((LdsPtr)(size_t)addr) = v; }

		template <bool COH>
		__device__ __forceinline__ float LoadIn(const float* p)
		{
			if constexpr (COH) return __builtin_bit_cast(float, __hip_atomic_load(reinterpret_cast<const unsigned*>(p), __ATOMIC_RELAXED, __HIP_MEMORY_SCOPE_SYSTEM));
			else return *p;
		}
		template <bool COH>
		__device__ __forceinline__ void StoreOut(float* p, float v)
		{
			if constexpr (COH) __hip_atomic_store(reinterpret_cast<unsigned*>(p), __builtin_bit_cast(unsigned, v), __ATOMIC_RELAXED, __HIP_MEMORY_SCOPE_SYSTEM);
			else *p = v;
		}

		struct ArchA1Base
		{
			static constexpr int K(int, int) { return 3; }
			static constexpr int HEADK = 1;
			static constexpr bool LEAKY = false;
			static constexpr int T = 2, CHUNK = 10;
			static constexpr bool COARSE = false;
			static constexpr bool GUARDHIST = false;
			static constexpr bool FOLD = false;
			static constexpr int SKEW = 0;
			static constexpr bool COMPACT = true;
#ifndef NA_A1_NT_DIL
#define NA_A1_NT_DIL 128
#endif
			static constexpr int NT_DIL = NA_A1_NT_DIL;
		};
#ifndef NA_SPK_SKEW
#define NA_SPK_SKEW 0
#endif
		struct ArchStd : ArchA1Base
		{
			static constexpr int SKEW = NA_SPK_SKEW;
			static constexpr bool FOLD = true;
			static constexpr int NA = 2;
			static constexpr int CH[2] = { 16, 8 };
			static constexpr int NLA[2] = { 10, 10 };
			static constexpr int DIL[2][16] = { { 1, 2, 4, 8, 16, 32, 64, 128, 256, 512 }, { 1, 2, 4, 8, 16, 32, 64, 128, 256, 512 } };
		};
		struct ArchLite : ArchA1Base
		{
			static constexpr int NA = 2;
			static constexpr int CH[2] = { 16, 8 };
			static constexpr int NLA[2] = { 7, 13 };
			static constexpr int DIL[2][16] = { { 1, 2, 4, 8, 16, 32, 64 }, { 128, 256, 512, 1, 2, 4, 8, 16, 32, 64, 128, 256, 512 } };
		};
		struct ArchLite16 : ArchA1Base
		{
			static constexpr int NA = 2;
			static constexpr int CH[2] = { 16, 16 };
			static constexpr int NLA[2] = { 7, 13 };
			static constexpr int DIL[2][16] = { { 1, 2, 4, 8, 16, 32, 64 }, { 128, 256, 512, 1, 2, 4, 8, 16, 32, 64, 128, 256, 512 } };
		};

		struct ArchLite16T1 : ArchLite16 { static constexpr int T = 1; };

		struct ArchA2Base
		{
			static constexpr int NA = 1;
			static constexpr int NLA[2] = { 23, 0 };
			static constexpr int DIL[2][32] = { { 1, 3, 7, 17, 41, 101, 239, 1, 3, 7, 17, 41, 101, 239, 1, 13, 1, 3, 7, 17, 41, 101, 239 }, { 0 } };
			static constexpr int K(int, int l) { return (l == 14 || l == 15) ? 15 : 6; }
			static constexpr int HEADK = 16;
			static constexpr bool LEAKY = true;
			static constexpr int CHUNK = 16;
			static constexpr bool COARSE = true;
			static constexpr bool GUARDHIST = true;
			static constexpr bool FOLD = false;
			static constexpr int SKEW = 0;
			static constexpr bool COMPACT = false;
			static constexpr int NT_DIL = 100;
		};
		struct ArchA2Full : ArchA2Base { static constexpr int CH[2] = { 8, 0 }; static constexpr int T = 2; };
		struct ArchA2Lite : ArchA2Base { static constexpr int CH[2] = { 4, 0 }; static constexpr int T = 4; };

		struct FamStd { typedef ArchStd A0; typedef ArchStd A1; static constexpr int N = 1; };
		struct FamLite { typedef ArchLite A0; typedef ArchLite A1; static constexpr int N = 1; };
		struct FamLitePacked { typedef ArchLite A0; typedef ArchLite16 A1; static constexpr int N = 2; };
		struct FamA2 { typedef ArchA2Full A0; typedef ArchA2Lite A1; static constexpr int N = 2; };
		struct FamLite16T1 { typedef ArchLite16T1 A0; typedef ArchLite16T1 A1; static constexpr int N = 1; };

		enum TapClass { TAP_LDS = 0, TAP_HIST = 1, TAP_BOTH = 2 };

		template <class A>
		struct Tab
		{
			static constexpr int NA = A::NA;
			static constexpr int TotalLayers() { int n = 0; for (int a = 0; a < NA; a++) n += A::NLA[a]; return n; }
			static constexpr int NL = TotalLayers();
			static constexpr int NSTAGES = NL + NA + 1;
			static constexpr int ArrOf(int L) { int a = 0; while (L >= A::NLA[a]) { L -= A::NLA[a]; a++; } return a; }
			static constexpr int InArr(int L) { int a = 0; while (L >= A::NLA[a]) { L -= A::NLA[a]; a++; } return L; }
			static constexpr int Dil(int L) { return A::DIL[ArrOf(L)][InArr(L)]; }
			static constexpr int GPof(int a) { return A::CH[a] / 4; }
			static constexpr bool FirstOfArr(int L) { return InArr(L) == 0; }
			static constexpr bool LastOfArr(int L) { return InArr(L) == A::NLA[ArrOf(L)] - 1; }
			static constexpr int KS(int L) { return A::K(ArrOf(L), InArr(L)); }
			static constexpr bool Fold(int L) { return A::FOLD && KS(L) == 3 && GPof(ArrOf(L)) >= 2; }
			static constexpr int HEADK = A::HEADK;
			static constexpr int NRINGS = NL + (HEADK > 1 ? 1 : 0);
			static constexpr bool ExactRing(int L) { return L < NL && !FirstOfArr(L) && Dil(L) >= FRAMES && (KS(L) - 1) * Dil(L) >= 2 * FRAMES && ((KS(L) - 1) * Dil(L)) % 16 == 0; }
			static constexpr int HistFrames(int L) { return L < NL ? ((KS(L) - 1) * Dil(L) + 15) / 16 * 16 : (HEADK - 1 + 15) / 16 * 16; }
			static constexpr bool CompactRing(int L) { return A::COMPACT && L < NL && KS(L) > 1 && HistFrames(L) <= WN_COMPACT_MAX_HISTORY; }
			static constexpr int RingFrames(int L)
			{
				if (ExactRing(L)) return (KS(L) - 1) * Dil(L);
				if (CompactRing(L)) return 3 * HistFrames(L);
				return HistFrames(L) + FRAMES;
			}
			static constexpr int RingKeep(int L) { return ExactRing(L) ? RingFrames(L) : (CompactRing(L) ? HistFrames(L) : RingFrames(L) - FRAMES); }
			static constexpr int RingG(int L) { return GPof(L < NL ? ArrOf(L) : NA - 1); }
			static constexpr int RingOff(int L)
			{
				int o = WN_HEADER_F4;
				for (int l = 0; l < L; l++) o += RingFrames(l) * RingG(l);
				return o;
			}
			static constexpr int StateF4 = (RingOff(NRINGS) + 15) / 16 * 16;
			static constexpr int StageOfLayer(int L) { return 1 + L + ArrOf(L); }
			static constexpr int FirstLayerOfArr(int a) { int L = 0; for (int i = 0; i < a; i++) L += A::NLA[i]; return L; }
			static constexpr int LinkStage(int a) { return FirstLayerOfArr(a) + a; }
			static constexpr int LinkNC(int a) { const int Po = 4 / GPof(a - 1), Pn = 4 / GPof(a); return Po > Pn ? Po : Pn; }
			static constexpr int LayerOfStage(int s)
			{
				for (int L = 0; L < NL; L++)
					if (StageOfLayer(L) == s) return L;
				return -1;
			}
			static constexpr int StageOps(int s)
			{
				if (s == 0) return 1;
				if (s == NSTAGES - 1) return 2 * HEADK + 1;
				for (int a = 1; a < NA; a++)
					if (s == LinkStage(a)) return 4 * LinkNC(a) + 1;
				return 2 * KS(LayerOfStage(s)) + 4;
			}
			static constexpr int AOff(int s) { int o = 0; for (int i = 0; i < s; i++) o += StageOps(i) * 64; return o; }
			static constexpr int WsplitQuads = AOff(NSTAGES);
			static constexpr int CHUNK = A::CHUNK;
			static constexpr int TapOps(int s) { return s == NSTAGES - 1 ? 2 * HEADK : 2 * KS(LayerOfStage(s)); }
			static constexpr bool Chunked(int s) { return StageOps(s) > CHUNK; }
			static constexpr int TapChunks(int s) { return (TapOps(s) + CHUNK - 1) / CHUNK; }
			static constexpr int NumChunks(int s) { return Chunked(s) ? TapChunks(s) + 1 : 1; }
			static constexpr int ChunkBegin(int s, int c)
			{
				if (!Chunked(s)) return 0;
				if (c >= TapChunks(s)) return TapOps(s);
				const int pairs = TapOps(s) / 2, n = TapChunks(s);
				return 2 * ((pairs * c + n - 1) / n);
			}
			static constexpr int ChunkEnd(int s, int c) { return !Chunked(s) ? StageOps(s) : (c >= TapChunks(s) ? StageOps(s) : ChunkBegin(s, c + 1)); }
			static constexpr int ChunkIndex(int s, int c) { int n = 0; for (int i = 0; i < s; i++) n += NumChunks(i); return n + c; }
			static constexpr int MaxChunkOps()
			{
				int m = 0;
				for (int s = 0; s < NSTAGES; s++)
					for (int c = 0; c < NumChunks(s); c++) m = (ChunkEnd(s, c) - ChunkBegin(s, c)) > m ? (ChunkEnd(s, c) - ChunkBegin(s, c)) : m;
				return m;
			}
			static constexpr int MaxGP() { int m = 0; for (int a = 0; a < NA; a++) m = GPof(a) > m ? GPof(a) : m; return m; }
		};

		template <class A_, int NF_, int SPB_, bool PK_, bool COH_ = false, bool NT_ = false>
		struct Cfg
		{
			static constexpr bool COH = COH_;
			static constexpr bool NT = NT_;
			typedef A_ A;
			typedef Tab<A_> TB;
			static constexpr int NF = NF_, T = A_::T, FW = 16 * T, WPS = NF_ / FW, SPB = SPB_ * T / 2, NTHREADS = 64 * WPS * SPB;
			static_assert(WPS >= 1 && WPS * FW == NF_, "block length is a whole number of waves");
			static constexpr bool PK = PK_;
			static constexpr int MAXOPS = A_::CHUNK;
			static_assert(TB::MaxChunkOps() <= MAXOPS, "stage operand chunk");
			static constexpr int HPF = 5;
			static constexpr int SKEW = (SPB == 2 && !PK_ && T == 2 && A_::SKEW > 0) ? A_::SKEW : 0;
			static constexpr int NWB = SKEW > 0 ? SPB : 1;
			static constexpr int STG_THREADS = NTHREADS / NWB;
			static constexpr bool AUX16 = !PK_ && SKEW == 0;
			static constexpr int AUX_OFF = 0;
			static constexpr int IMG_OFF = AUX_OFF + SPB * FRAMES * (PK_ ? 32 : (AUX16 ? 16 : 8));
			static constexpr int IMG_ONE = TB::MaxGP() * PLANE * 16;
			static constexpr int WBUF_OFF = IMG_OFF + SPB * 2 * IMG_ONE;
			static constexpr int WBUF_ONE = MAXOPS * 1024;
			static constexpr int IDOP_OFF = WBUF_OFF + NWB * 2 * WBUF_ONE;
			static constexpr int DUMP_OFF = IDOP_OFF + 1024;
			static constexpr int FLAG_OFF = DUMP_OFF + 1024;
			static constexpr int BCAST_OFF = FLAG_OFF + 16 * SPB;
			static constexpr int LDS_BYTES = BCAST_OFF + (COH_ ? 64 : 0);
			static_assert(LDS_BYTES <= 80 * 1024, "two workgroups per CU");
		};

		template <int GP, int T>
		struct Geo
		{
			static_assert(GP == 4 || GP == 2 || GP == 1, "full lane modes of 16 / 8 / 4 channels");
			static constexpr int P = 4 / GP;
			static_assert(T % P == 0, "every tile slot of a set is a tile of the wave");
			static constexpr int S = T / P;
		};

		constexpr int TapClassOf(int F0, int P, int i, int shift)
		{
			const int lo = F0 + 16 * P * i - shift, hi = lo + 16 * P - 1;
			return hi < 0 ? TAP_HIST : (lo >= 0 ? TAP_LDS : TAP_BOTH);
		}

		template <class C, int RG>
		constexpr bool SmallRing() { return C::A::GUARDHIST && C::TB::RingKeep(RG) <= GUARD; }

		template <class C>
		constexpr int WaveTapClass(int w, int P, int i, int shift, bool small)
		{
			if (small) return TAP_LDS;
			if (!C::A::COARSE || w == 0 || C::WPS <= 2) return TapClassOf(C::FW * w, P, i, shift);
			const int first = TapClassOf(C::FW * 1, P, i, shift);
			for (int v = 2; v < C::WPS; v++)
				if (TapClassOf(C::FW * v, P, i, shift) != first) return TAP_BOTH;
			return first;
		}

		template <class C, int L>
		struct LayerSig
		{
			typedef typename C::TB TB;
			static constexpr int GP = TB::GPof(TB::ArrOf(L)), P = Geo<GP, C::T>::P, S = Geo<GP, C::T>::S, d = TB::Dil(L), K = TB::KS(L);
			static constexpr bool NEXT = !TB::LastOfArr(L);
			static constexpr int LN = NEXT ? L + 1 : L;
			static constexpr int dn = NEXT ? TB::Dil(LN) : 0, Kn = NEXT ? TB::KS(LN) : 1;
			static constexpr bool FOLD = TB::Fold(L) && !C::PK;
			static constexpr unsigned long long Of(int w)
			{
				unsigned long long s = 0;
				for (int k = 0; k < K - 1; k++)
					for (int i = 0; i < S; i++) s = s * 3 + (unsigned)WaveTapClass<C>(w, P, i, d * (K - 1 - k), SmallRing<C, L>());
				for (int k = 0; k < Kn - 1 && k < C::HPF; k++)
					for (int i = 0; i < S; i++) s = s * 3 + (unsigned)WaveTapClass<C>(w, P, i, dn * (Kn - 1 - k), SmallRing<C, LN>());
				return s;
			}
			static constexpr int Rep(int w) { int r = w; for (int v = w - 1; v >= 0; v--) if (Of(v) == Of(w)) r = v; return r; }
			static constexpr unsigned MaskOf(int r) { unsigned m = 0; for (int w = 0; w < C::WPS; w++) if (Rep(w) == r) m |= 1u << w; return m; }
			static constexpr bool LastRep(int r) { for (int w = r + 1; w < C::WPS; w++) if (Rep(w) == w) return false; return true; }
		};

		struct Ctx
		{
			__amdgpu_buffer_rsrc_t srsrc;
			__amdgpu_buffer_rsrc_t wrsrc;
			int myPos;
			int wave, sub, waveAll;
			int lane;
			int gs0, gs1;
			unsigned wbuf;
			int stgWave;
#ifdef NA_SP_TRACE
			long long* trace;
			int nwaves;
#endif
		};

#ifdef NA_SP_TRACE
#define SPK_STAMP(stage, point) do { __builtin_amdgcn_sched_barrier(0); if (cx.trace != nullptr && cx.lane == 0) cx.trace[(((stage) * 8 + (point)) * cx.nwaves) + cx.waveAll] = (long long)__builtin_readcyclecounter(); __builtin_amdgcn_sched_barrier(0); } while (0)
#else
#define SPK_STAMP(stage, point) (void)0
#endif

		template <class C, int GP>
		struct Lanes
		{
			int fl;
			int cg;
			unsigned img;
			unsigned aux;
			unsigned ring;
			bool dual;

			__device__ __forceinline__ void Init(const Ctx& cx, int gs)
			{
				const int q = cx.lane >> 4, j = cx.lane & 15;
				const int p = q / GP;
				cg = q % GP;
				fl = 16 * p + j;
				const int f = C::FW * cx.wave + fl;
				img = (unsigned)(C::IMG_OFF + cx.sub * 2 * C::IMG_ONE + (cg * PLANE + GUARD + f) * 16);
				ring = (unsigned)((fl * GP + cg) * 16);
				dual = C::PK && gs < 0;
				if constexpr (C::PK) aux = (unsigned)(C::AUX_OFF + ((cx.sub * 4 + (gs < 0 ? 2 * cg : (cg >> gs))) * FRAMES + f) * 8);
				else aux = (unsigned)(C::AUX_OFF + (cx.sub * FRAMES + f) * (C::AUX16 ? 16 : 8));
			}
		};

		template <class C, int GP>
		__device__ __forceinline__ u32x4 AuxRead(const Lanes<C, GP>& ln, int i)
		{
			constexpr int P = Geo<GP, C::T>::P;
			if constexpr (C::AUX16) return LdsRead16(ln.aux + (unsigned)(16 * P * i * 16));
			else
			{
				const u32x2 v = LdsRead8(ln.aux + (unsigned)(16 * P * i * 8));
				if constexpr (C::PK)
				{
					if (ln.dual)
					{
						const u32x2 w = LdsRead8(ln.aux + (unsigned)(16 * P * i * 8) + (unsigned)(FRAMES * 8));
						return u32x4{ v.x, v.y, (v.x & 0xffffu) | (w.x << 16), (w.y & 0xffffu) | (w.x << 16) };
					}
				}
				return u32x4{ v.x, v.y, v.x & 0xffffu, 0u };
			}
		}

		struct State
		{
			f32x4 xc[2];
			f32x4 hd[2];
			u32x4 xs[2];
			u32x4 hist[5][2];
		};

		template <class C>
		__device__ __forceinline__ u32x4 Split(f32x4 v, const Ctx& cx)
		{
#ifdef NA_NO_SAT
			return SplitQuad(v);
#else
			if constexpr (C::A::LEAKY) return SplitQuadSat(v, (unsigned)(C::FLAG_OFF + 16 * cx.sub));
			else return SplitQuad(v);
#endif
		}

		template <int GP, int R>
		__device__ __forceinline__ int RingWrap(unsigned laneRing, int base)
		{
			unsigned a = laneRing + (unsigned)base * (unsigned)(GP * 16);
			return (int)__builtin_elementwise_min(a, a - (unsigned)(R * GP * 16));
		}

		template <class C, int RG, int WR>
		__device__ __forceinline__ u32x4 HistLoadAt(const Ctx& cx, unsigned laneRing, int fl, int shift, int i)
		{
			typedef typename C::TB TB;
			constexpr int GP = TB::RingG(RG), P = Geo<GP, C::T>::P, R = TB::RingFrames(RG), OFF = TB::RingOff(RG);
			const int cls = WaveTapClass<C>(WR, P, i, shift, SmallRing<C, RG>());
			if ((NA_ABL & 4) || cls == TAP_LDS) return RingLoad(cx.srsrc, OOB);
			const int pos0 = __builtin_amdgcn_readlane(cx.myPos, RG);
			int base = pos0 - shift + C::FW * cx.wave + 16 * P * i;
			if (base < 0) base += R;
			if (base >= R) base -= R;
			const int addr = RingWrap<GP, R>(laneRing, base);
			constexpr int NT_LD = C::NT ? 2 : NA_SPK_NT_LD, NT_DIL = C::NT ? C::A::NT_DIL : NA_SPK_NT_DIL;
			constexpr bool LONG = RG < TB::NL && TB::Dil(RG < TB::NL ? RG : 0) >= NT_DIL;
			if constexpr (LONG && NT_LD != 0)
			{
				if (cls == TAP_HIST) return RingLoadAux<NT_LD>(cx.srsrc, addr, OFF * 16);
				return RingLoadAux<NT_LD>(cx.srsrc, (C::FW * cx.wave + 16 * P * i + fl < shift) ? addr : OOB, OFF * 16);
			}
			if (cls == TAP_HIST) return RingLoad(cx.srsrc, addr, OFF * 16);
			return RingLoad(cx.srsrc, (C::FW * cx.wave + 16 * P * i + fl < shift) ? addr : OOB, OFF * 16);
		}

		template <class C, int L>
		constexpr int ShiftOf(int k) { return C::TB::Dil(L) * (C::TB::KS(L) - 1 - k); }

		template <class C, int GP>
		constexpr bool HistNeededAt(int shift, int i, bool small) { return !small && TapClassOf(0, Geo<GP, C::T>::P, i, shift) != TAP_LDS; }

		template <class C, int L>
		constexpr int PrefetchTaps() { return (C::TB::KS(L) - 1) < C::HPF ? (C::TB::KS(L) - 1) : C::HPF; }
		template <class C, int L>
		constexpr int HistLoadsOf()
		{
			typedef typename C::TB TB;
			constexpr int GP = TB::GPof(TB::ArrOf(L)), S = Geo<GP, C::T>::S;
			int n = 0;
			for (int k = 0; k < PrefetchTaps<C, L>(); k++)
				for (int i = 0; i < S; i++) n += HistNeededAt<C, GP>(ShiftOf<C, L>(k), i, SmallRing<C, L>()) ? 1 : 0;
			return n;
		}

		template <class C, int L, int WR>
		__device__ __forceinline__ void HistPrefetch(const Ctx& cx, unsigned laneRing, int fl, State& st)
		{
			constexpr int GP = C::TB::GPof(C::TB::ArrOf(L)), S = Geo<GP, C::T>::S;
#pragma unroll
			for (int k = 0; k < PrefetchTaps<C, L>(); k++)
#pragma unroll
				for (int i = 0; i < S; i++)
					if (HistNeededAt<C, GP>(ShiftOf<C, L>(k), i, SmallRing<C, L>())) st.hist[k][i] = HistLoadAt<C, L, WR>(cx, laneRing, fl, ShiftOf<C, L>(k), i);
		}

		template <class C, int RG>
		constexpr bool StoreNeeded(int i)
		{
			typedef typename C::TB TB;
			constexpr int P = Geo<TB::RingG(RG), C::T>::P, KEEP = TB::RingKeep(RG);
			return (C::NF - C::FW) + 16 * P * (i + 1) - 1 >= C::NF - KEEP;
		}
		template <class C, int RG>
		constexpr int StoresOf()
		{
			constexpr int S = Geo<C::TB::RingG(RG), C::T>::S;
			int n = 0;
			for (int i = 0; i < S; i++) n += StoreNeeded<C, RG>(i) ? 1 : 0;
			return n;
		}

		template <class C, int RG, int GP, int MINSHIFT>
		__device__ __forceinline__ void Publish(const Ctx& cx, const Lanes<C, GP>& ln, u32x4 v, int i, int imgWrite)
		{
			typedef typename C::TB TB;
			constexpr int P = Geo<GP, C::T>::P, R = TB::RingFrames(RG), OFF = TB::RingOff(RG), KEEP = TB::RingKeep(RG);
			static_assert(GP == TB::RingG(RG), "lane mode of the receiving ring");
			if (!(NA_ABL & 64) && MINSHIFT < C::NF)
				LdsWrite16(ln.img + (unsigned)(imgWrite * C::IMG_ONE + 16 * P * i * 16), v);
			if ((NA_ABL & 4) || !StoreNeeded<C, RG>(i)) return;
			const int pos0 = __builtin_amdgcn_readlane(cx.myPos, RG);
			int base;
			if constexpr (TB::CompactRing(RG))
			{
				int end = pos0 + C::NF % R;
				if (end >= R) end -= R;
				base = end - C::NF + C::FW * cx.wave + 16 * P * i + R;
			}
			else
			{
				base = pos0 + C::FW * cx.wave + 16 * P * i;
				if (base >= R) base -= R;
			}
			const int addr = RingWrap<GP, R>(ln.ring, base);
			constexpr int NT_ST = C::NT ? 2 : NA_SPK_NT_ST, NT_DIL = C::NT ? C::A::NT_DIL : NA_SPK_NT_DIL;
			constexpr bool LONG = RG < TB::NL && TB::Dil(RG < TB::NL ? RG : 0) >= NT_DIL;
			if constexpr (LONG && NT_ST != 0)
			{
				if (KEEP >= C::NF) RingStoreAux<NT_ST>(cx.srsrc, v, addr, OFF * 16);
				else RingStoreAux<NT_ST>(cx.srsrc, v, (C::FW * cx.wave + 16 * P * i + ln.fl >= C::NF - KEEP) ? addr : OOB, OFF * 16);
				return;
			}
			if (KEEP >= C::NF) RingStore(cx.srsrc, v, addr, OFF * 16);
			else RingStore(cx.srsrc, v, (C::FW * cx.wave + 16 * P * i + ln.fl >= C::NF - KEEP) ? addr : OOB, OFF * 16);
		}

		template <class C, int RG, int GP>
		__device__ __forceinline__ void GuardStage(const Ctx& cx, const Lanes<C, GP>& ln, int imgBuf)
		{
			typedef typename C::TB TB;
			static_assert(GP == TB::RingG(RG), "lane mode of the ring");
			constexpr int R = TB::RingFrames(RG), OFF = TB::RingOff(RG);
			if constexpr (!C::A::GUARDHIST) return;
			if (cx.wave != 0) return;
			if constexpr (SmallRing<C, RG>())
			{
				if (NA_ABL & 4) return;
				const int pos0 = __builtin_amdgcn_readlane(cx.myPos, RG);
				int base = pos0 - GUARD;
				if (base < 0) base += R;
				if (cx.lane < 16)
				{
#pragma unroll
					for (int cg = 0; cg < GP; cg++)
					{
						const int addr = RingWrap<GP, R>((unsigned)((cx.lane * GP + cg) * 16), base);
						const unsigned dst = (unsigned)(C::IMG_OFF + imgBuf * C::IMG_ONE + cg * PLANE * 16) + (unsigned)(cx.sub * 2 * C::IMG_ONE);
						__builtin_amdgcn_raw_ptr_buffer_load_lds(cx.srsrc, (__attribute__((address_space(3))) void*)(LdsPtr)(size_t)dst, 16, addr, OFF * 16, 0, 0);
					}
				}
			}
			else
			{
				if ((cx.lane >> 4) < GP && (cx.lane & 15) == 15) LdsWrite16(ln.img + (unsigned)(imgBuf * C::IMG_ONE) - 16u * 16u, u32x4{ 0, 0, 0, 0 });
			}
		}

		template <class C, int SN, int CN>
		struct Stager
		{
			typedef typename C::TB TB;
			static constexpr int QUADS = (TB::ChunkEnd(SN, CN) - TB::ChunkBegin(SN, CN)) * 64;
			static constexpr int SRC = TB::AOff(SN) + TB::ChunkBegin(SN, CN) * 64;
			static constexpr int BUF = TB::ChunkIndex(SN, CN) & 1;
			static constexpr int NCOPY = (QUADS + C::STG_THREADS - 1) / C::STG_THREADS;
			static __device__ __forceinline__ void Begin(const Ctx& cx)
			{
				if (NA_ABL & 16) return;
#pragma unroll
				for (int c = 0; c < NCOPY; c++)
				{
					const int i0 = c * C::STG_THREADS + cx.stgWave * 64;
					const bool mine = i0 < QUADS;
					const unsigned dst = mine ? cx.wbuf + (unsigned)(BUF * C::WBUF_ONE) + (unsigned)i0 * 16u : (unsigned)C::DUMP_OFF;
					__builtin_amdgcn_raw_ptr_buffer_load_lds(cx.wrsrc, (__attribute__((address_space(3))) void*)(LdsPtr)(size_t)dst, 16,
						mine ? (SRC + i0 + cx.lane) * 16 : OOB, 0, 0, 0);
				}
			}
			template <int LATER>
			static __device__ __forceinline__ void End()
			{
				__builtin_amdgcn_s_waitcnt((LATER & 15) | ((LATER >> 4) << 14) | (7 << 4) | (15 << 8));
			}
		};
		template <class C, int s, int c>
		struct NextChunk
		{
			static constexpr bool SAME = c + 1 < C::TB::NumChunks(s);
			static constexpr int S = SAME ? s : s + 1, CN = SAME ? c + 1 : 0;
			typedef Stager<C, S, CN> St;
		};

		template <class C>
		__device__ __forceinline__ u32x4 WOp(const Ctx& cx, int s, int c, int m)
		{
			const int buf = C::TB::ChunkIndex(s, c) & 1, local = m - C::TB::ChunkBegin(s, c);
			return LdsRead16(cx.wbuf + (unsigned)(buf * C::WBUF_ONE + ((NA_ABL & 128) ? 0 : local) * 1024) + (unsigned)cx.lane * 16u);
		}

		template <bool PACKED>
		__device__ __forceinline__ f32x4 ActivateTanh(f32x4 a)
		{
			if (PACKED)
			{
				const f32x2 lo = FastTanh2(f32x2{ a.x, a.y }), hi = FastTanh2(f32x2{ a.z, a.w });
				return f32x4{ lo.x, lo.y, hi.x, hi.y };
			}
			return f32x4{ FastTanh(a.x), FastTanh(a.y), FastTanh(a.z), FastTanh(a.w) };
		}

		template <class C, int GP>
		__device__ __forceinline__ u32x4 TapLds(const Ctx& cx, const Lanes<C, GP>& ln, int imgRead, int shift, int i, int cls)
		{
			constexpr int P = Geo<GP, C::T>::P;
			if (NA_ABL & 256) return u32x4{ (unsigned)shift, 0, 0, 0 };
			if (cls == TAP_LDS) return LdsRead16(ln.img + (unsigned)(imgRead * C::IMG_ONE) + (unsigned)((16 * P * i - shift) * 16));
			int off = C::FW * cx.wave + 16 * P * i + ln.fl - shift;
			off = off < -1 ? -1 : off;
			return LdsRead16((unsigned)(C::IMG_OFF + imgRead * C::IMG_ONE + GUARD * 16) + (unsigned)(cx.sub * 2 * C::IMG_ONE) + (unsigned)((ln.cg * PLANE + off) * 16));
		}

		template <class C, int RG, int GP, int WR>
		__device__ __forceinline__ f32x4 ConvTap(const Ctx& cx, const Lanes<C, GP>& ln, int imgRead, int shift, int i, u32x4 ah, u32x4 al, u32x4 hist, f32x4 acc)
		{
			constexpr int P = Geo<GP, C::T>::P;
			const int cls = WaveTapClass<C>(WR, P, i, shift, SmallRing<C, RG>());
			if (cls != TAP_LDS)
			{
				acc = Mfma(ah, hist, acc);
				acc = MfmaLo<1>(al, hist, acc);
			}
			if (cls != TAP_HIST)
			{
				const u32x4 b = TapLds<C, GP>(cx, ln, imgRead, shift, i, cls);
				acc = Mfma(ah, b, acc);
				acc = MfmaLo<1>(al, b, acc);
			}
			return acc;
		}

		template <class C, int RG, int GP, int WR>
		__device__ __forceinline__ f32x4 ConvTapFold(const Ctx& cx, const Lanes<C, GP>& ln, int imgRead, int shift, int i, u32x4 ah, u32x4 hist, f32x4 acc, u32x2& th)
		{
			constexpr int P = Geo<GP, C::T>::P;
			const int cls = WaveTapClass<C>(WR, P, i, shift, SmallRing<C, RG>());
			th = u32x2{ 0, 0 };
			if (cls != TAP_LDS)
			{
				acc = Mfma(ah, hist, acc);
				th = u32x2{ hist.x, hist.y };
			}
			if (cls != TAP_HIST)
			{
				const u32x4 b = TapLds<C, GP>(cx, ln, imgRead, shift, i, cls);
				acc = Mfma(ah, b, acc);
				th = cls == TAP_LDS ? u32x2{ b.x, b.y } : u32x2{ th.x | b.x, th.y | b.y };
			}
			return acc;
		}

		template <class C, int L, int WR, int c>
		__device__ __forceinline__ void LayerChunk(const Ctx& cx, const Lanes<C, C::TB::GPof(C::TB::ArrOf(L))>& ln, State& st, u32x4 (&ax)[LayerSig<C, L>::S],
			f32x4 (&acc)[LayerSig<C, L>::S])
		{
			typedef typename C::TB TB;
			typedef LayerSig<C, L> SG;
			constexpr int GP = SG::GP, S = SG::S, K = SG::K, s = TB::StageOfLayer(L), NCH = TB::NumChunks(s), CB = TB::ChunkBegin(s, c), CE = TB::ChunkEnd(s, c);
			constexpr int imgRead = s & 1, imgWrite = (s + 1) & 1, LN = SG::LN;
			constexpr bool LASTLAYER = TB::LastOfArr(L) && TB::ArrOf(L) == TB::NA - 1;
			constexpr int NEXTMINSHIFT = SG::NEXT ? TB::Dil(LN) : (1 << 20);
			constexpr bool OWN = 2 * (K - 1) >= CB && 2 * (K - 1) < CE;
			constexpr bool TAIL = 2 * K >= CB && 2 * K < CE;
			constexpr int LATER = ((OWN && SG::NEXT) ? HistLoadsOf<C, LN>() : 0) + ((TAIL && SG::NEXT && !LASTLAYER) ? StoresOf<C, LN>() : 0);
			typedef typename NextChunk<C, s, c>::St NextStager;
			if constexpr (c == 0)
			{
				if constexpr (SG::NEXT) GuardStage<C, LN, GP>(cx, ln, imgWrite);
				else if constexpr (LASTLAYER && TB::HEADK > 1) GuardStage<C, TB::NL, GP>(cx, ln, (TB::NSTAGES - 1 + 1) & 1);
			}
			NextStager::Begin(cx);
			if constexpr (c == 0)
			{
#pragma unroll
				for (int i = 0; i < S; i++) ax[i] = AuxRead<C, GP>(ln, i);
			}
			constexpr int KLO = CB / 2, KHI = (CE / 2 < K - 1) ? CE / 2 : K - 1;
			constexpr int NX = (KHI > C::HPF) ? KHI - (KLO > C::HPF ? KLO : C::HPF) : 0;
			u32x4 hx[NX > 0 ? NX : 1][S];
#pragma unroll
			for (int k = KLO; k < KHI; k++)
			{
				if (k < C::HPF) continue;
#pragma unroll
				for (int i = 0; i < S; i++)
					if (WaveTapClass<C>(WR, SG::P, i, ShiftOf<C, L>(k), SmallRing<C, L>()) != TAP_LDS) hx[k - (KLO > C::HPF ? KLO : C::HPF)][i] = HistLoadAt<C, L, WR>(cx, ln.ring, ln.fl, ShiftOf<C, L>(k), i);
			}
			static_assert(!SG::FOLD || (NCH == 1 && K == 3), "folded operands: K = 3 layers in one chunk");
			u32x2 th[SG::FOLD ? 2 : 1][S];
#pragma unroll
			for (int k = KLO; k < KHI; k++)
			{
				const u32x4 ah = WOp<C>(cx, s, c, 2 * k), al = SG::FOLD ? ah : WOp<C>(cx, s, c, 2 * k + 1);
#pragma unroll
				for (int i = 0; i < S; i++)
				{
					u32x4 h = u32x4{ 0, 0, 0, 0 };
					if (WaveTapClass<C>(WR, SG::P, i, ShiftOf<C, L>(k), SmallRing<C, L>()) != TAP_LDS)
						h = (k < C::HPF) ? st.hist[k < C::HPF ? k : 0][i] : hx[k >= C::HPF ? k - (KLO > C::HPF ? KLO : C::HPF) : 0][i];
					if constexpr (SG::FOLD) acc[i] = ConvTapFold<C, L, GP, WR>(cx, ln, imgRead, ShiftOf<C, L>(k), i, ah, h, acc[i], th[k < 2 ? k : 0][i]);
					else acc[i] = ConvTap<C, L, GP, WR>(cx, ln, imgRead, ShiftOf<C, L>(k), i, ah, al, h, acc[i]);
				}
			}
			if constexpr (SG::FOLD)
			{
				const u32x4 al01 = WOp<C>(cx, s, c, 1);
#pragma unroll
				for (int i = 0; i < S; i++) acc[i] = Mfma(al01, u32x4{ th[0][i].x, th[0][i].y, th[1][i].x, th[1][i].y }, acc[i]);
			}
			if constexpr (OWN)
			{
				if constexpr (SG::NEXT) HistPrefetch<C, LN, WR>(cx, ln.ring, ln.fl, st);
				const u32x4 ah = WOp<C>(cx, s, c, 2 * K - 2), al = WOp<C>(cx, s, c, 2 * K - 1);
#pragma unroll
				for (int i = 0; i < S; i++)
				{
					acc[i] = Mfma(ah, st.xs[i], acc[i]);
					if constexpr (SG::FOLD) acc[i] = Mfma(al, u32x4{ st.xs[i].x, st.xs[i].y, ax[i].x, ax[i].y }, acc[i]);
					else acc[i] = MfmaLo<1>(al, st.xs[i], acc[i]);
				}
			}
			if constexpr (TAIL)
			{
				if constexpr (!SG::FOLD)
				{
					const u32x4 xa = WOp<C>(cx, s, c, 2 * K);
#pragma unroll
					for (int i = 0; i < S; i++) acc[i] = Mfma(xa, ax[i], acc[i]);
				}
				SPK_STAMP(s, 1);
				f32x4 z[S];
#pragma unroll
				for (int i = 0; i < S; i++)
				{
					if constexpr (C::A::LEAKY) z[i] = f32x4{ LeakyReLU(acc[i].x), LeakyReLU(acc[i].y), LeakyReLU(acc[i].z), LeakyReLU(acc[i].w) };
					else z[i] = ActivateTanh<(NA_PK_TANH != 0) && (C::NTHREADS < 512)>(acc[i]);
				}
				SPK_STAMP(s, 2);
				const u32x4 idop = LdsRead16((unsigned)C::IDOP_OFF + (unsigned)cx.lane * 16u);
				const u32x4 w1h = WOp<C>(cx, s, c, 2 * K + 1), w1l = WOp<C>(cx, s, c, 2 * K + 2), b1a = SG::FOLD ? w1l : WOp<C>(cx, s, c, 2 * K + 3);
#pragma unroll
				for (int i = 0; i < S; i++)
				{
					const u32x4 zs = SplitQuad(z[i]);
					st.hd[i] = Mfma(idop, zs, st.hd[i]);
					if constexpr (!LASTLAYER)
					{
						f32x4 y = st.xc[i];
						y = Mfma(w1h, zs, y);
						const u32x4 axi = NA_SPK_AUX2 ? AuxRead<C, GP>(ln, i) : ax[i];
						if constexpr (SG::FOLD) y = Mfma(w1l, u32x4{ zs.x, zs.y, axi.x, axi.y }, y);
						else
						{
							y = MfmaLo<2>(w1l, zs, y);
							y = Mfma(b1a, axi, y);
						}
						st.xc[i] = y;
						if constexpr (SG::NEXT)
						{
							st.xs[i] = Split<C>(y, cx);
							Publish<C, LN, GP, NEXTMINSHIFT>(cx, ln, st.xs[i], i, imgWrite);
						}
					}
				}
				SPK_STAMP(s, 3);
			}
			NextStager::template End<LATER>();
			SPK_STAMP(s, 4);
			BlockBarrier<C::NTHREADS / 64>();
			if constexpr (c + 1 < NCH) LayerChunk<C, L, WR, c + 1>(cx, ln, st, ax, acc);
		}

		template <class C, int L, int WR>
		__device__ __forceinline__ void LayerBody(const Ctx& cx, const Lanes<C, C::TB::GPof(C::TB::ArrOf(L))>& ln, State& st)
		{
			constexpr int S = LayerSig<C, L>::S;
			SPK_STAMP(C::TB::StageOfLayer(L), 0);
			u32x4 ax[S];
			f32x4 acc[S];
#pragma unroll
			for (int i = 0; i < S; i++) acc[i] = f32x4{ 0.0f, 0.0f, 0.0f, 0.0f };
			LayerChunk<C, L, WR, 0>(cx, ln, st, ax, acc);
			SPK_STAMP(C::TB::StageOfLayer(L), 5);
		}

		template <class C, int L, int W>
		__device__ __forceinline__ void LayerDispatch(const Ctx& cx, const Lanes<C, C::TB::GPof(C::TB::ArrOf(L))>& ln, State& st)
		{
			typedef LayerSig<C, L> SG;
			if constexpr (W < C::WPS)
			{
				if constexpr (SG::Rep(W) != W) LayerDispatch<C, L, W + 1>(cx, ln, st);
				else if constexpr (SG::LastRep(W)) LayerBody<C, L, W>(cx, ln, st);
				else
				{
					constexpr unsigned MASK = SG::MaskOf(W);
					if ((MASK >> cx.wave) & 1u) LayerBody<C, L, W>(cx, ln, st);
					else LayerDispatch<C, L, W + 1>(cx, ln, st);
				}
			}
		}

		template <class C, int L, int W>
		__device__ __forceinline__ void FirstHistDispatch(const Ctx& cx, unsigned laneRing, int fl, State& st)
		{
			typedef typename C::TB TB;
			constexpr int GP = TB::GPof(TB::ArrOf(L)), P = Geo<GP, C::T>::P, S = Geo<GP, C::T>::S;
			if constexpr (W < C::WPS)
			{
				constexpr bool same = [] {
					bool r = true;
					for (int w = W + 1; w < C::WPS; w++)
						for (int k = 0; k < PrefetchTaps<C, L>(); k++)
							for (int i = 0; i < S; i++) r = r && WaveTapClass<C>(w, P, i, ShiftOf<C, L>(k), SmallRing<C, L>()) == WaveTapClass<C>(W, P, i, ShiftOf<C, L>(k), SmallRing<C, L>());
					return r;
				}();
				if constexpr (same) HistPrefetch<C, L, W>(cx, laneRing, fl, st);
				else
				{
					if (cx.wave == W) HistPrefetch<C, L, W>(cx, laneRing, fl, st);
					else FirstHistDispatch<C, L, W + 1>(cx, laneRing, fl, st);
				}
			}
		}

		template <class C>
		__device__ __forceinline__ void RechStage(const Ctx& cx, const Lanes<C, C::TB::GPof(0)>& ln, State& st)
		{
			constexpr int GP = C::TB::GPof(0), S = Geo<GP, C::T>::S;
			SPK_STAMP(0, 0);
			GuardStage<C, 0, GP>(cx, ln, 1);
			const u32x4 ra = WOp<C>(cx, 0, 0, 0);
#pragma unroll
			for (int i = 0; i < S; i++)
			{
				const u32x4 ax = AuxRead<C, GP>(ln, i);
				f32x4 x = f32x4{ 0.0f, 0.0f, 0.0f, 0.0f };
				x = Mfma(ra, ax, x);
				st.xc[i] = x;
				st.hd[i] = f32x4{ 0.0f, 0.0f, 0.0f, 0.0f };
				st.xs[i] = Split<C>(x, cx);
				Publish<C, 0, GP, C::TB::Dil(0)>(cx, ln, st.xs[i], i, 1);
			}
			FirstHistDispatch<C, 0, 0>(cx, ln.ring, ln.fl, st);
			SPK_STAMP(0, 1); SPK_STAMP(0, 2); SPK_STAMP(0, 3);
			Stager<C, 1, 0>::template End<StoresOf<C, 0>() + HistLoadsOf<C, 0>()>();
			SPK_STAMP(0, 4);
			BlockBarrier<C::NTHREADS / 64>();
			SPK_STAMP(0, 5);
		}

		template <class C, int AN>
		__device__ __forceinline__ void LinkStage(const Ctx& cx, const Lanes<C, C::TB::GPof(AN)>& ln, State& st)
		{
			typedef typename C::TB TB;
			constexpr int GPO = TB::GPof(AN - 1), GPN = TB::GPof(AN), Po = 4 / GPO, Pn = 4 / GPN, NC = Po > Pn ? Po : Pn;
			constexpr int So = Geo<GPO, C::T>::S, Sn = Geo<GPN, C::T>::S, s = TB::LinkStage(AN), LN = TB::FirstLayerOfArr(AN);
			static_assert(C::T == 1 || C::T == 2, "array links are written for one or two tiles per wave");
			SPK_STAMP(s, 0);
			GuardStage<C, LN, GPN>(cx, ln, (s + 1) & 1);
			Stager<C, s + 1, 0>::Begin(cx);
			u32x4 hs[So], xq[So];
#pragma unroll
			for (int i = 0; i < So; i++)
			{
				hs[i] = Split<C>(st.hd[i], cx);
				xq[i] = Split<C>(st.xc[i], cx);
			}
			f32x4 hn[Sn], xn[Sn];
#pragma unroll
			for (int i = 0; i < Sn; i++)
			{
				hn[i] = f32x4{ 0.0f, 0.0f, 0.0f, 0.0f };
				xn[i] = f32x4{ 0.0f, 0.0f, 0.0f, 0.0f };
				hn[i] = Mfma(WOp<C>(cx, s, 0, 4 * NC), AuxRead<C, GPN>(ln, i), hn[i]);
			}
#pragma unroll
			for (int t = 0; t < C::T; t++)
			{
				const int u = t % NC, so = t / Po, sn = t / Pn;
hn[sn] = Mfma(WOp<C>(cx, s, 0, 4 * u), hs[so], hn[sn]);
				hn[sn] = MfmaLo<4>(WOp<C>(cx, s, 0, 4 * u + 1), hs[so], hn[sn]);
				xn[sn] = Mfma(WOp<C>(cx, s, 0, 4 * u + 2), xq[so], xn[sn]);
				xn[sn] = MfmaLo<4>(WOp<C>(cx, s, 0, 4 * u + 3), xq[so], xn[sn]);
			}
#pragma unroll
			for (int i = 0; i < Sn; i++)
			{
				st.hd[i] = hn[i];
				st.xc[i] = xn[i];
				st.xs[i] = Split<C>(xn[i], cx);
				Publish<C, LN, GPN, TB::Dil(LN)>(cx, ln, st.xs[i], i, (s + 1) & 1);
			}
			FirstHistDispatch<C, LN, 0>(cx, ln.ring, ln.fl, st);
			SPK_STAMP(s, 1); SPK_STAMP(s, 2); SPK_STAMP(s, 3);
			Stager<C, s + 1, 0>::template End<StoresOf<C, LN>() + HistLoadsOf<C, LN>()>();
			SPK_STAMP(s, 4);
			BlockBarrier<C::NTHREADS / 64>();
			SPK_STAMP(s, 5);
		}

		template <class C, int WR>
		__device__ __forceinline__ void HeadBody(const Ctx& cx, const Lanes<C, C::TB::GPof(C::TB::NA - 1)>& ln, State& st, float* __restrict__ out, size_t outBase,
			const long (&outRow)[4], int pack, float headScale, bool live)
		{
			typedef typename C::TB TB;
			constexpr int GP = TB::GPof(TB::NA - 1), P = Geo<GP, C::T>::P, S = Geo<GP, C::T>::S, s = TB::NSTAGES - 1, K = TB::HEADK, NCH = TB::NumChunks(s), RG = TB::NL;
			constexpr int imgHead = (s + 1) & 1;
			u32x4 hs[S];
			f32x4 acc[S];
#pragma unroll
			for (int i = 0; i < S; i++)
			{
				hs[i] = Split<C>(st.hd[i], cx);
				acc[i] = f32x4{ 0.0f, 0.0f, 0.0f, 0.0f };
			}
#pragma unroll
			for (int c = 0; c < NCH; c++)
			{
				if constexpr (K > 1)
				{
					if (c + 1 < NCH)
					{
						if (c == 0) Stager<C, s, 1>::Begin(cx);
						else if (c + 1 < NCH) Stager<C, s, (NCH > 2 ? 2 : 1)>::Begin(cx);
					}
					if (c == 0)
					{
#pragma unroll
						for (int i = 0; i < S; i++) Publish<C, RG, GP, 1>(cx, ln, hs[i], i, imgHead);
						BlockBarrier<C::NTHREADS / 64>();
					}
#pragma unroll
					for (int k = 0; k < K - 1; k++)
					{
						if (2 * k < TB::ChunkBegin(s, c) || 2 * k >= TB::ChunkEnd(s, c)) continue;
						const u32x4 ah = WOp<C>(cx, s, c, 2 * k), al = WOp<C>(cx, s, c, 2 * k + 1);
#pragma unroll
						for (int i = 0; i < S; i++)
						{
							u32x4 h = u32x4{ 0, 0, 0, 0 };
							if (WaveTapClass<C>(WR, P, i, K - 1 - k, SmallRing<C, RG>()) != TAP_LDS) h = HistLoadAt<C, RG, WR>(cx, ln.ring, ln.fl, K - 1 - k, i);
							acc[i] = ConvTap<C, RG, GP, WR>(cx, ln, imgHead, K - 1 - k, i, ah, al, h, acc[i]);
						}
					}
				}
				if (2 * (K - 1) >= TB::ChunkBegin(s, c) && 2 * (K - 1) < TB::ChunkEnd(s, c))
				{
					const u32x4 ah = WOp<C>(cx, s, c, 2 * K - 2), al = WOp<C>(cx, s, c, 2 * K - 1);
#pragma unroll
					for (int i = 0; i < S; i++)
					{
						acc[i] = Mfma(ah, hs[i], acc[i]);
						acc[i] = MfmaLo<8>(al, hs[i], acc[i]);
					}
				}
				if (2 * K >= TB::ChunkBegin(s, c) && 2 * K < TB::ChunkEnd(s, c))
				{
					const u32x4 ba = WOp<C>(cx, s, c, 2 * K);
#pragma unroll
					for (int i = 0; i < S; i++)
					{
						acc[i] = Mfma(ba, AuxRead<C, GP>(ln, i), acc[i]);
						const int f = C::FW * cx.wave + 16 * P * i + ln.fl;
						if (live && ln.cg == 0)
						{
							if constexpr (C::PK)
							{
								const float v[4] = { acc[i].x, acc[i].y, acc[i].z, acc[i].w };
#pragma unroll
								for (int q = 0; q < 4; q++)
									if (q < pack && outRow[q] >= 0) StoreOut<C::COH>(out + outRow[q] + f, headScale * v[q]);
							}
							else StoreOut<C::COH>(out + outBase + f, headScale * acc[i].x);
						}
					}
				}
				if (c + 1 < NCH)
				{
					__builtin_amdgcn_s_waitcnt(0 | (7 << 4) | (15 << 8));
					BlockBarrier<C::NTHREADS / 64>();
				}
			}
		}

		template <class C>
		__device__ __forceinline__ void HeadDispatch(const Ctx& cx, const Lanes<C, C::TB::GPof(C::TB::NA - 1)>& ln, State& st, float* __restrict__ out, size_t outBase,
			const long (&outRow)[4], int pack, float headScale, bool live)
		{
			if constexpr (C::TB::HEADK == 1 || C::WPS == 1 || SmallRing<C, C::TB::NL>()) HeadBody<C, 0>(cx, ln, st, out, outBase, outRow, pack, headScale, live);
			else
			{
				if (cx.wave == 0) HeadBody<C, 0>(cx, ln, st, out, outBase, outRow, pack, headScale, live);
				else HeadBody<C, C::WPS - 1>(cx, ln, st, out, outBase, outRow, pack, headScale, live);
			}
		}

		template <class C, int L, int LEND>
		__device__ __forceinline__ void RunLayers(const Ctx& cx, const Lanes<C, C::TB::GPof(C::TB::ArrOf(L))>& ln, State& st)
		{
			LayerDispatch<C, L, 0>(cx, ln, st);
			if constexpr (L + 1 < LEND) RunLayers<C, L + 1, LEND>(cx, ln, st);
		}

		template <class C, int AN>
		__device__ __forceinline__ void RunArrays(const Ctx& cx, State& st, float* __restrict__ out, size_t outBase, const long (&outRow)[4], int pack, float headScale, bool live)
		{
			typedef typename C::TB TB;
			Lanes<C, TB::GPof(AN)> ln;
			ln.Init(cx, AN == 0 ? cx.gs0 : cx.gs1);
			if constexpr (AN == 0) RechStage<C>(cx, ln, st);
			else LinkStage<C, AN>(cx, ln, st);
			RunLayers<C, TB::FirstLayerOfArr(AN), TB::FirstLayerOfArr(AN) + C::A::NLA[AN]>(cx, ln, st);
			if constexpr (AN + 1 < TB::NA) RunArrays<C, AN + 1>(cx, st, out, outBase, outRow, pack, headScale, live);
			else HeadDispatch<C>(cx, ln, st, out, outBase, outRow, pack, headScale, live);
		}

		template <class C>
		__device__ __forceinline__ void RunWorkgroup(const GroupArgs& ga, int groupBlock, const float* __restrict__ in, float* __restrict__ out, long inStride, long outStride
#ifdef NA_SP_TRACE
			, long long* trace
#endif
			, const int tid = (int)threadIdx.x
			)
		{
			typedef typename C::TB TB;
			constexpr bool PK = C::PK;
			constexpr int SPB = C::SPB, NF = C::NF;
			const int lane = tid & 63;
			const int waveAll = __builtin_amdgcn_readfirstlane(tid >> 6);
			const int sub = waveAll / C::WPS, wave = waveAll % C::WPS;

			int sidx = groupBlock * SPB + sub;
			const bool live = sidx < ga.numStreams;
			if (!live) sidx = ga.numStreams - 1;
			const int slot = ga.slots ? ga.slots[sidx] : ga.slot0 + sidx;
			const int row = PK ? 0 : (ga.slots ? ga.rows[sidx] : ga.row0 + sidx);
			u32x4* stt = ga.state + (size_t)slot * (size_t)ga.stateF4;
			int* header = reinterpret_cast<int*>(stt);

			Ctx cx;
			cx.srsrc = MakeRsrc(stt, live ? (unsigned)ga.stateF4 * 16u : 0u);
			cx.wrsrc = MakeRsrc(ga.wsplit, (unsigned)ga.wsplitQuads * 16u);
			cx.myPos = header[lane];
			cx.wave = wave; cx.sub = sub; cx.waveAll = waveAll; cx.lane = lane;
			cx.wbuf = (unsigned)(C::WBUF_OFF + (C::SKEW > 0 ? sub : 0) * 2 * C::WBUF_ONE);
			cx.stgWave = C::SKEW > 0 ? wave : waveAll;
#ifdef NA_SP_TRACE
			cx.trace = trace;
			cx.nwaves = C::NTHREADS / 64;
			if (cx.trace != nullptr && lane == 0) cx.trace[((C::TB::NSTAGES * 8 + 0) * cx.nwaves) + waveAll] = (long long)__builtin_readcyclecounter();
#endif
			Stager<C, 1, 0>::Begin(cx);
			const int pack = PK ? ga.pack : 1;
			cx.gs0 = PK ? ((ga.gps0 >> 1) & 3) : 0;
			cx.gs1 = PK ? (ga.gps1 == 0 ? -1 : ((ga.gps1 >> 1) & 3)) : 0;
			long outRow[4];
			int rowOf[4];
#pragma unroll
			for (int q = 0; q < 4; q++)
			{
				const int r = (PK && live && q < ga.pack) ? ga.rows[sidx * ga.pack + q] : -1;
				rowOf[q] = r;
				outRow[q] = r >= 0 ? (long)r * outStride : -1;
			}

			if constexpr (PK)
			{
				for (int i = wave * 64 + lane; i < FRAMES; i += C::WPS * 64)
				{
					float c[4];
#pragma unroll
					for (int q = 0; q < 4; q++) c[q] = (rowOf[q] >= 0 && i < NF) ? LoadIn<C::COH>(in + (size_t)rowOf[q] * inStride + i) : 0.0f;
#pragma unroll
					for (int q = 0; q < 4; q++)
					{
						const float cc = ClampCond(c[q], ga.condLimit);
						const _Float16 ch = (_Float16)cc, cl = (_Float16)(cc - (float)ch);
						const f16x2 a = { ch, (_Float16)1.0f }, b = { cl, (_Float16)1.0f };
						*reinterpret_cast<__attribute__((address_space(3))) u32x2*>((LdsPtr)(size_t)(unsigned)(C::AUX_OFF + ((sub * 4 + q) * FRAMES + i) * 8)) =
							u32x2{ __builtin_bit_cast(unsigned, a), __builtin_bit_cast(unsigned, b) };
					}
				}
			}
			else
			{
				for (int i = wave * 64 + lane; i < FRAMES; i += C::WPS * 64)
				{
					const float c = (i < NF) ? ClampCond(LoadIn<C::COH>(in + (size_t)row * inStride + i), ga.condLimit) : 0.0f;
					const _Float16 ch = (_Float16)c, cl = (_Float16)(c - (float)ch);
					const f16x2 a = { ch, (_Float16)1.0f }, b = { cl, (_Float16)1.0f }, d = { ch, (_Float16)0.0f };
					if constexpr (C::AUX16)
						LdsWrite16((unsigned)(C::AUX_OFF + (sub * FRAMES + i) * 16), u32x4{ __builtin_bit_cast(unsigned, a), __builtin_bit_cast(unsigned, b), __builtin_bit_cast(unsigned, d), 0u });
					else
						*reinterpret_cast<__attribute__((address_space(3))) u32x2*>((LdsPtr)(size_t)(unsigned)(C::AUX_OFF + (sub * FRAMES + i) * 8)) =
							u32x2{ __builtin_bit_cast(unsigned, a), __builtin_bit_cast(unsigned, b) };
				}
			}
			for (int i = tid; i < SPB * 2 * TB::MaxGP(); i += C::NTHREADS) LdsWrite16((unsigned)(C::IMG_OFF + (i * PLANE + GUARD - 1) * 16), u32x4{ 0, 0, 0, 0 });
			if (tid < 64)
			{
				const int i = lane & 15, q = lane >> 4;
				const unsigned one = 0x3c00u;
				const unsigned lo = (q == (i >> 2)) ? (((i & 3) == 0) ? one : ((i & 3) == 1) ? (one << 16) : 0u) : 0u;
				const unsigned hi = (q == (i >> 2)) ? (((i & 3) == 2) ? one : ((i & 3) == 3) ? (one << 16) : 0u) : 0u;
				LdsWrite16((unsigned)C::IDOP_OFF + (unsigned)lane * 16u, u32x4{ lo, hi, lo, hi });
			}
			if constexpr (C::A::LEAKY)
			{
				if (tid < SPB) *reinterpret_cast<__attribute__((address_space(3))) unsigned*>((LdsPtr)(size_t)(unsigned)(C::FLAG_OFF + 16 * tid)) = 0u;
			}
			if (cx.stgWave == 0) LdsWrite16(cx.wbuf + (unsigned)lane * 16u, BufLoad(cx.wrsrc, lane * 16));
			BlockBarrier<C::NTHREADS / 64>();

			if constexpr (C::SKEW > 0)
			{
				if (sub != 0)
					for (int k = 0; k < C::SKEW; k++) BlockBarrier<C::NTHREADS / 64>();
			}
			State st;
			RunArrays<C, 0>(cx, st, out, (size_t)row * outStride, outRow, pack, ga.headScale, live);
			if constexpr (C::SKEW > 0)
			{
				if (sub == 0)
					for (int k = 0; k < C::SKEW; k++) BlockBarrier<C::NTHREADS / 64>();
			}

#ifdef NA_SP_TRACE
			if (cx.trace != nullptr && lane == 0) cx.trace[((C::TB::NSTAGES * 8 + 1) * cx.nwaves) + waveAll] = (long long)__builtin_readcyclecounter();
#endif
			if constexpr (C::A::LEAKY)
			{
				BlockBarrier<C::NTHREADS / 64>();
				if (wave == 0) CountRangeEvent(header, (int)*reinterpret_cast<__attribute__((address_space(3))) unsigned*>((LdsPtr)(size_t)(unsigned)(C::FLAG_OFF + 16 * sub)), lane, live);
			}
			if (wave == 0 && live && lane < ga.nrings)
			{
				const int R = ga.ringFrames[lane];
				int p = cx.myPos + NF;
				if (p >= R) p -= R;
				if (p >= R) p -= R;
				if (p >= R) p -= R;
				header[lane] = p;
			}
		}

#ifndef NA_SPK_OCC
#define NA_SPK_OCC(nf, spb) (((nf) * (spb) / 64) < 1 ? 1 : ((nf) * (spb) / 64))
#endif
		template <class F, int NF, int SPB>
		constexpr int OccOf() { return F::A0::T == 1 ? (NA_SPK_OCC(NF, SPB) / 2 < 1 ? 1 : NA_SPK_OCC(NF, SPB) / 2) : NA_SPK_OCC(NF, SPB); }
		template <class F, int NF, int SPB, bool PK, bool NT = false>
		__global__ void __launch_bounds__(64 * (NF / (16 * F::A0::T)) * (SPB * F::A0::T / 2)) __attribute__((amdgpu_waves_per_eu(OccOf<F, NF, SPB>()))) WaveNetSpecKernel(const LaunchArgs args,
			const float* __restrict__ in, float* __restrict__ out, long inStride, long outStride
#ifdef NA_SP_TRACE
			, long long* __restrict__ trace, int traceBlock
#endif
			)
		{
			typedef Cfg<typename F::A0, NF, SPB, PK, false, NT> C;
			typedef Cfg<typename F::A1, NF, SPB, PK, false, NT> C1;
			static_assert(C::NTHREADS == C1::NTHREADS, "members of a family launch the same workgroup");
			extern __shared__ __attribute__((aligned(16))) char dynSmem[];
			asm volatile("" : : "s"((unsigned)(size_t)(LdsPtr)dynSmem));

			int gi = 0;
			for (int i = 1; i < args.numGroups; i++)
				if ((int)blockIdx.x >= args.g[i].firstBlock) gi = i;
			const GroupArgs& ga = args.g[gi];
			const int groupBlock = (int)blockIdx.x - ga.firstBlock;
#if NA_SPK_DELAY > 0
			if (blockIdx.x >= gridDim.x / 2)
				for (int k = 0; k < NA_SPK_DELAY; k += 100) __builtin_amdgcn_s_sleep(100);
#endif
#ifdef NA_SP_TRACE
			long long* tr = ((int)blockIdx.x == traceBlock) ? trace : nullptr;
			if (F::N > 1 && ga.arch == 1) RunWorkgroup<C1>(ga, groupBlock, in, out, inStride, outStride, tr);
			else RunWorkgroup<C>(ga, groupBlock, in, out, inStride, outStride, tr);
#else
			if (F::N > 1 && ga.arch == 1) RunWorkgroup<C1>(ga, groupBlock, in, out, inStride, outStride);
			else RunWorkgroup<C>(ga, groupBlock, in, out, inStride, outStride);
#endif
		}

		template <class F, int NF, int SPB, bool PK>
		__global__ void __launch_bounds__(64 * (NF / (16 * F::A0::T)) * (SPB * F::A0::T / 2)) __attribute__((amdgpu_waves_per_eu(OccOf<F, NF, SPB>()))) WaveNetSpecResidentKernel(const LaunchArgs args,
			const ResidentArgs ra
#ifdef NA_SP_TRACE
			, long long* __restrict__ trace, int traceBlock
#endif
			)
		{
			typedef Cfg<typename F::A0, NF, SPB, PK, true> C;
			typedef Cfg<typename F::A1, NF, SPB, PK, true> C1;
			static_assert(C::NTHREADS == C1::NTHREADS && C::BCAST_OFF == C1::BCAST_OFF, "members of a family launch the same workgroup");
			extern __shared__ __attribute__((aligned(16))) char dynSmem[];
			asm volatile("" : : "s"((unsigned)(size_t)(LdsPtr)dynSmem));
			typedef __attribute__((address_space(3))) unsigned long long* Lds64;
			Lds64 const bc = reinterpret_cast<Lds64>((LdsPtr)(size_t)(unsigned)C::BCAST_OFF);
			if (threadIdx.x == 0)
			{
				bc[5] = ra.base + ra.wgDone[blockIdx.x];
				bc[6] = ~0ull;
				if (ra.startDelay > 0 && 2 * blockIdx.x >= gridDim.x)
				{
					const unsigned long long t0 = __builtin_amdgcn_s_memrealtime();
					while (__builtin_amdgcn_s_memrealtime() - t0 < ra.startDelay) __builtin_amdgcn_s_sleep(16);
				}
			}
			for (;;)
			{
				if (threadIdx.x == 0)
				{
					int z = 0;
					asm volatile("" : "+v"(z));
					const ResidentArgs& r = (&ra)[__builtin_amdgcn_readfirstlane(z)];
					unsigned long long k = bc[5];
					long blk = (long)bc[6];
					unsigned long long go = 1;
					if (blk >= 0) blk += (long)gridDim.x;
					if (blk < 0 || blk >= (long)r.numBlocks)
					{
						const bool finished = blk >= 0;
						if (finished) k++;
						const unsigned slot = (unsigned)(k % RESIDENT_RING);
						if (finished) __hip_atomic_store(&r.wgDone[blockIdx.x], (unsigned)(k - r.base), __ATOMIC_RELAXED, __HIP_MEMORY_SCOPE_AGENT);
						const ResidentCmd* cmd = &r.ctrl->cmd[(k + 1) % RESIDENT_RING];
						auto word = [](const void* p) { return __hip_atomic_load(reinterpret_cast<const unsigned long long*>(p), __ATOMIC_RELAXED, __HIP_MEMORY_SCOPE_SYSTEM); };
						unsigned long long cIn = word(&cmd->in), cOut = word(&cmd->out), cIs = word(&cmd->inStride), cOs = word(&cmd->outStride);
						unsigned long long cSeq = word(&cmd->seq), cChk = word(&cmd->check);
						if (finished)
						{
							const unsigned before = __hip_atomic_fetch_add(&r.doneCount[slot], 1u, __ATOMIC_RELAXED, __HIP_MEMORY_SCOPE_AGENT);
							if (before == gridDim.x - 1)
							{
								__hip_atomic_store(&r.doneCount[slot], 0u, __ATOMIC_RELAXED, __HIP_MEMORY_SCOPE_AGENT);
								__hip_atomic_store(&r.status->completed, k, __ATOMIC_RELAXED, __HIP_MEMORY_SCOPE_SYSTEM);
							}
						}
						const unsigned long long t0 = __builtin_amdgcn_s_memrealtime();
						bool leaving = false;
						while (cSeq != k + 1 || cChk != ResidentCmdCheck(cIn, cOut, cIs, cOs, cSeq))
						{
							if (leaving) { go = 0; break; }
							leaving = word(&r.ctrl->exitAfter) <= k || __builtin_amdgcn_s_memrealtime() - t0 > r.idleTicks;
							if (!leaving) __builtin_amdgcn_s_sleep(4);
							cIn = word(&cmd->in), cOut = word(&cmd->out), cIs = word(&cmd->inStride), cOs = word(&cmd->outStride);
							cSeq = word(&cmd->seq), cChk = word(&cmd->check);
						}
						if (go)
						{
							bc[1] = cIn;
							bc[2] = cOut;
							bc[3] = cIs;
							bc[4] = cOs;
						}
						blk = (long)blockIdx.x;
					}
					bc[0] = go;
					bc[5] = k;
					bc[6] = (unsigned long long)blk;
				}
				BlockBarrier<C::NTHREADS / 64>();
				if (__builtin_amdgcn_readfirstlane((int)bc[0]) == 0) break;
				{
					auto uni = [](unsigned long long v) {
						return ((unsigned long long)(unsigned)__builtin_amdgcn_readfirstlane((int)(v >> 32)) << 32) | (unsigned)__builtin_amdgcn_readfirstlane((int)v);
					};
					const float* in = reinterpret_cast<const float*>(uni(bc[1]));
					float* out = reinterpret_cast<float*>(uni(bc[2]));
					const long inStride = (long)uni(bc[3]), outStride = (long)uni(bc[4]);
					const int blk = __builtin_amdgcn_readfirstlane((int)bc[6]);
					int gi = 0;
					for (int i = 1; i < args.numGroups; i++)
						if (blk >= args.g[i].firstBlock) gi = i;
					asm volatile("" : "+v"(gi));
					const GroupArgs& ga = args.g[__builtin_amdgcn_readfirstlane(gi)];
					int tid = (int)threadIdx.x;
					asm volatile("" : "+v"(tid));
					const int groupBlock = blk - ga.firstBlock;
#ifdef NA_SP_TRACE
					long long* tr = ((int)blockIdx.x == traceBlock) ? trace : nullptr;
					if (tr != nullptr && threadIdx.x == 0)
					{
						tr[(C::TB::NSTAGES * 8 + 4) * (C::NTHREADS / 64)] = tr[(C::TB::NSTAGES * 8 + 2) * (C::NTHREADS / 64)];
						tr[(C::TB::NSTAGES * 8 + 3) * (C::NTHREADS / 64)] = (long long)__builtin_readcyclecounter();
					}
					if (F::N > 1 && ga.arch == 1) RunWorkgroup<C1>(ga, groupBlock, in, out, inStride, outStride, tr, tid);
					else RunWorkgroup<C>(ga, groupBlock, in, out, inStride, outStride, tr, tid);
#else
					if (F::N > 1 && ga.arch == 1) RunWorkgroup<C1>(ga, groupBlock, in, out, inStride, outStride, tid);
					else RunWorkgroup<C>(ga, groupBlock, in, out, inStride, outStride, tid);
#endif
				}
				__builtin_amdgcn_s_waitcnt(0 | (7 << 4) | (15 << 8));
				BlockBarrier<C::NTHREADS / 64>();
#ifdef NA_SP_TRACE
				if ((int)blockIdx.x == traceBlock && trace != nullptr && threadIdx.x == 0) trace[(C::TB::NSTAGES * 8 + 2) * (C::NTHREADS / 64)] = (long long)__builtin_readcyclecounter();
#endif
			}
		}

		template <class A>
		static bool Matches(const WnSplitStage* st, int nstages, int stateF4, int wsplitQuads)
		{
			typedef Tab<A> TB;
			if (nstages != TB::NSTAGES || stateF4 != TB::StateF4 || wsplitQuads != TB::WsplitQuads) return false;
			for (int s = 0; s < nstages; s++)
				if (st[s].a_off != TB::AOff(s) || st[s].a_ops != TB::StageOps(s)) return false;
			if (st[0].type != WN_ST_RECHANNEL_COND || st[0].Gp != TB::GPof(0) || st[0].G != TB::GPof(0) || st[0].out_ring_id != 0) return false;
			for (int L = 0; L < TB::NL; L++)
			{
				const WnSplitStage& d = st[TB::StageOfLayer(L)];
				const int a = TB::ArrOf(L);
				if (d.type != WN_ST_LAYER || d.Gp != TB::GPof(a) || d.G != TB::GPof(a) || d.ksize != TB::KS(L) || d.dilation != TB::Dil(L)) return false;
				if (d.ring_id != L || d.ring_off != TB::RingOff(L) || d.ring_frames != TB::RingFrames(L)) return false;
				if (((d.flags & WN_FLAG_LEAKY) != 0) != A::LEAKY || (d.flags & WN_FLAG_STD_TANH)) return false;
				if (((d.flags & WN_FLAG_FOLD) != 0) != TB::Fold(L)) return false;
				if (!TB::LastOfArr(L) && (d.out_ring_id != L + 1 || !(d.flags & WN_FLAG_PUBLISH))) return false;
			}
			for (int a = 1; a < TB::NA; a++)
			{
				const WnSplitStage& d = st[TB::LinkStage(a)];
				if (d.type != WN_ST_ARRAY_LINK || d.Gp != TB::GPof(a - 1) || d.ksize != TB::GPof(a) || d.out_ring_id != TB::FirstLayerOfArr(a)) return false;
			}
			const WnSplitStage& h = st[nstages - 1];
			if (h.ksize != TB::HEADK || h.Gp != TB::GPof(TB::NA - 1)) return false;
			if (TB::HEADK == 1) return h.type == WN_ST_HEAD_DENSE_OUT;
			return h.type == WN_ST_HEAD_CONV_OUT && h.dilation == 1 && h.ring_id == TB::NL && h.ring_off == TB::RingOff(TB::NL) && h.ring_frames == TB::RingFrames(TB::NL);
		}

		template <class F, int NF, int SPB, bool PK>
		static hipError_t FillGroupArgs(const WnFrameGroup* groups, int numGroups, GroupArgs* out, int* blocksOut)
		{
			typedef Cfg<typename F::A0, NF, SPB, PK> C;
			typedef Cfg<typename F::A1, NF, SPB, PK> C1;
			int blocks = 0;
			const bool reverse = Tuning::Get().spReverse;
			for (int i = 0; i < numGroups; i++)
			{
				const WnFrameGroup& g = groups[reverse ? numGroups - 1 - i : i];
				const WnModelDev& m = *g.model;
				out[i] = {};
				GroupArgs& a = out[i];
				a.stages = m.sstages; a.wsplit = m.wsplit; a.ringFrames = m.ring_frames;
				a.state = reinterpret_cast<u32x4*>(g.state); a.slots = g.slots; a.rows = g.rows;
				a.nstages = m.nstages; a.nrings = m.nrings; a.stateF4 = m.state_f4; a.wsplitQuads = m.wsplit_quads;
				a.headScale = m.head_scale;
				a.condLimit = m.cond_limit;
				a.saturate = m.saturate;
				a.numStreams = g.numStreams; a.slot0 = g.slot0; a.row0 = g.row0;
				a.maxG = m.max_G;
				a.firstBlock = blocks;
				a.pack = g.pack > 1 ? g.pack : 1;
				a.arch = (F::N > 1 && (m.spec_arch == WN_SPEC_LITE16 || m.spec_arch == WN_SPEC_A2LITE)) ? 1 : 0;
				const int c0 = a.arch == 1 ? F::A1::CH[0] : F::A0::CH[0], c1 = a.arch == 1 ? F::A1::CH[1] : F::A0::CH[1];
				a.gps0 = std::max(1, c0 / 4 / a.pack);
				a.gps1 = (a.pack > 1 && c1 < 4 * a.pack) ? 0 : std::max(1, c1 / 4 / a.pack);
				if (a.pack > 1 && !PK) return hipErrorInvalidValue;
				if (PK && g.slots == nullptr) return hipErrorInvalidValue;
				const int spbArch = a.arch == 1 ? C1::SPB : C::SPB;
				blocks += (g.numStreams + spbArch - 1) / spbArch;
			}
			*blocksOut = blocks;
			return hipSuccess;
		}

		template <class F, int NF, int SPB, bool PK>
		static hipError_t FillLaunchArgs(const WnFrameGroup* groups, int numGroups, LaunchArgs& args, int* blocksOut)
		{
			args = {};
			args.numGroups = numGroups;
			return FillGroupArgs<F, NF, SPB, PK>(groups, numGroups, args.g, blocksOut);
		}

		template <class F, int NF, int SPB, bool PK>
		__global__ void __launch_bounds__(64 * (NF / (16 * F::A0::T)) * (SPB * F::A0::T / 2)) __attribute__((amdgpu_waves_per_eu(OccOf<F, NF, SPB>()))) WaveNetSpecTableKernel(
			const GroupArgs* __restrict__ table, int numGroups, const float* __restrict__ in, float* __restrict__ out, long inStride, long outStride)
		{
			typedef Cfg<typename F::A0, NF, SPB, PK> C;
			typedef Cfg<typename F::A1, NF, SPB, PK> C1;
			extern __shared__ __attribute__((aligned(16))) char dynSmem[];
			asm volatile("" : : "s"((unsigned)(size_t)(LdsPtr)dynSmem));
			typedef const __attribute__((address_space(4))) GroupArgs* TablePtr;
			TablePtr tab = (TablePtr)(size_t)table;
			int lo = 0, hi = numGroups - 1;
			while (lo < hi)
			{
				const int mid = (lo + hi + 1) >> 1;
				if (tab[mid].firstBlock <= (int)blockIdx.x) lo = mid;
				else hi = mid - 1;
			}
			GroupArgs ga;
			{
				const auto& e = tab[lo];
				ga.stages = e.stages; ga.wsplit = e.wsplit; ga.ringFrames = e.ringFrames; ga.state = e.state; ga.slots = e.slots; ga.rows = e.rows;
				ga.nstages = e.nstages; ga.nrings = e.nrings; ga.stateF4 = e.stateF4; ga.wsplitQuads = e.wsplitQuads;
				ga.headScale = e.headScale;
				ga.numStreams = e.numStreams; ga.slot0 = e.slot0; ga.row0 = e.row0;
				ga.maxG = e.maxG; ga.firstBlock = e.firstBlock; ga.pack = e.pack; ga.condLimit = e.condLimit; ga.arch = e.arch;
				ga.gps0 = e.gps0; ga.gps1 = e.gps1; ga.saturate = e.saturate;
			}
			const int groupBlock = (int)blockIdx.x - ga.firstBlock;
#ifdef NA_SP_TRACE
			if (F::N > 1 && ga.arch == 1) RunWorkgroup<C1>(ga, groupBlock, in, out, inStride, outStride, nullptr);
			else RunWorkgroup<C>(ga, groupBlock, in, out, inStride, outStride, nullptr);
#else
			if (F::N > 1 && ga.arch == 1) RunWorkgroup<C1>(ga, groupBlock, in, out, inStride, outStride);
			else RunWorkgroup<C>(ga, groupBlock, in, out, inStride, outStride);
#endif
		}

		template <class F, int NF, int SPB, bool PK>
		static hipError_t LaunchTable(const WnFrameGroup* groups, int numGroups, const float* in, float* out, long inStride, long outStride, hipStream_t stream, WnLaunchTable& t)
		{
			typedef Cfg<typename F::A0, NF, SPB, PK> C;
			typedef Cfg<typename F::A1, NF, SPB, PK> C1;
			std::vector<GroupArgs> fresh((size_t)numGroups);
			int blocks = 0;
			const hipError_t fe = FillGroupArgs<F, NF, SPB, PK>(groups, numGroups, fresh.data(), &blocks);
			if (fe != hipSuccess) return fe;
			const void* dev = nullptr;
			const hipError_t ee = t.Ensure(fresh.data(), fresh.size() * sizeof(GroupArgs), stream, &dev);
			if (ee != hipSuccess) return ee;
			if (t.prepareOnly) return hipSuccess;
			constexpr int LDS_BYTES = C::LDS_BYTES > C1::LDS_BYTES ? C::LDS_BYTES : C1::LDS_BYTES;
			if (LDS_BYTES > 64 * 1024)
			{
				static PerDeviceOnce attr;
				const hipError_t e = attr.Run([] { return hipFuncSetAttribute(reinterpret_cast<const void*>(WaveNetSpecTableKernel<F, NF, SPB, PK>), hipFuncAttributeMaxDynamicSharedMemorySize, LDS_BYTES); });
				if (e != hipSuccess) return e;
			}
			hipLaunchKernelGGL((WaveNetSpecTableKernel<F, NF, SPB, PK>), dim3((unsigned)blocks), dim3(C::NTHREADS), LDS_BYTES, stream,
				reinterpret_cast<const GroupArgs*>(dev), numGroups, in, out, inStride, outStride);
			return hipGetLastError();
		}

		template <class F, int NF, int SPB, bool PK, bool NT = false>
		static hipError_t Launch(const WnFrameGroup* groups, int numGroups, const float* in, float* out, long inStride, long outStride, hipStream_t stream)
		{
			typedef Cfg<typename F::A0, NF, SPB, PK> C;
			typedef Cfg<typename F::A1, NF, SPB, PK> C1;
			LaunchArgs args;
			int blocks = 0;
			const hipError_t fe = FillLaunchArgs<F, NF, SPB, PK>(groups, numGroups, args, &blocks);
			if (fe != hipSuccess) return fe;
			constexpr int LDS_BYTES = C::LDS_BYTES > C1::LDS_BYTES ? C::LDS_BYTES : C1::LDS_BYTES;
			if (LDS_BYTES > 64 * 1024)
			{
				static PerDeviceOnce attr;
				const hipError_t e = attr.Run([] { return hipFuncSetAttribute(reinterpret_cast<const void*>(WaveNetSpecKernel<F, NF, SPB, PK, NT>), hipFuncAttributeMaxDynamicSharedMemorySize, LDS_BYTES); });
				if (e != hipSuccess) return e;
			}
			hipLaunchKernelGGL((WaveNetSpecKernel<F, NF, SPB, PK, NT>), dim3((unsigned)blocks), dim3(C::NTHREADS), LDS_BYTES, stream, args, in, out, inStride, outStride
#ifdef NA_SP_TRACE
				, GetWaveNetTraceBuffer(), Tuning::Get().traceBlock
#endif
				);
			return hipGetLastError();
		}

		template <class F, int NF, int SPB, bool PK>
		static hipError_t LaunchResident(const WnFrameGroup* groups, int numGroups, ResidentArgs ra, hipStream_t stream, int* gridOut)
		{
			typedef Cfg<typename F::A0, NF, SPB, PK, true> C;
			typedef Cfg<typename F::A1, NF, SPB, PK, true> C1;
			LaunchArgs args;
			int blocks = 0;
			const hipError_t fe = FillLaunchArgs<F, NF, SPB, PK>(groups, numGroups, args, &blocks);
			if (fe != hipSuccess) return fe;
			constexpr int LDS_BYTES = C::LDS_BYTES > C1::LDS_BYTES ? C::LDS_BYTES : C1::LDS_BYTES;
			static PerDeviceOnce attr;
			static std::atomic<int> perCU[kMaxHipDevices];
			int device = 0;
			hipError_t e = hipGetDevice(&device);
			if (e != hipSuccess) return e;
			if (device < 0 || device >= kMaxHipDevices) return hipErrorInvalidDevice;
			e = attr.Run([device] {
				hipError_t r = hipSuccess;
				if (LDS_BYTES > 64 * 1024)
					r = hipFuncSetAttribute(reinterpret_cast<const void*>(WaveNetSpecResidentKernel<F, NF, SPB, PK>), hipFuncAttributeMaxDynamicSharedMemorySize, LDS_BYTES);
				if (r != hipSuccess) return r;
				int nb = 0;
				r = hipOccupancyMaxActiveBlocksPerMultiprocessor(&nb, reinterpret_cast<const void*>(WaveNetSpecResidentKernel<F, NF, SPB, PK>), C::NTHREADS, LDS_BYTES);
				perCU[device].store(nb);
				return r;
			});
			if (e != hipSuccess) return e;
			const int resident = perCU[device].load() * CurrentDeviceCUs();
			int grid = std::min(blocks, resident);
			if (Tuning::Get().residentGrid > 0) grid = std::min(grid, Tuning::Get().residentGrid);
			*gridOut = grid;
			if (grid < 1) return hipErrorInvalidValue;
			if (stream == nullptr) return hipSuccess;
			ra.numBlocks = blocks;
			hipLaunchKernelGGL((WaveNetSpecResidentKernel<F, NF, SPB, PK>), dim3((unsigned)grid), dim3(C::NTHREADS), LDS_BYTES, stream, args, ra
#ifdef NA_SP_TRACE
				, GetWaveNetTraceBuffer(), Tuning::Get().traceBlock
#endif
				);
			return hipGetLastError();
		}

		template <class F, bool PK>
		static hipError_t LaunchNF(const WnFrameGroup* groups, int numGroups, const float* in, float* out, long inStride, long outStride, int n, int spb, hipStream_t stream,
			bool beyondCache = false)
		{
#ifdef NA_SP_QUICK
			(void)spb; (void)n; (void)beyondCache;
			return Launch<F, 128, 2, PK>(groups, numGroups, in, out, inStride, outStride, stream);
#else
			if constexpr (F::A0::T != 1)
				if (beyondCache && n == 128 && spb >= 2) return Launch<F, 128, 2, PK, true>(groups, numGroups, in, out, inStride, outStride, stream);
			if constexpr (F::A0::T == 1)
			{
				if (n == 128) return Launch<F, 128, 2, PK>(groups, numGroups, in, out, inStride, outStride, stream);
				if (n == 64) return Launch<F, 64, 2, PK>(groups, numGroups, in, out, inStride, outStride, stream);
				return Launch<F, 32, 2, PK>(groups, numGroups, in, out, inStride, outStride, stream);
			}
			else
			{
			if (n == 128) return spb >= 2 ? Launch<F, 128, 2, PK>(groups, numGroups, in, out, inStride, outStride, stream) : Launch<F, 128, 1, PK>(groups, numGroups, in, out, inStride, outStride, stream);
			if (n == 64) return spb >= 2 ? Launch<F, 64, 2, PK>(groups, numGroups, in, out, inStride, outStride, stream) : Launch<F, 64, 1, PK>(groups, numGroups, in, out, inStride, outStride, stream);
			if constexpr (F::A0::T == 2 && F::A1::T == 2)
				return spb >= 2 ? Launch<F, 32, 2, PK>(groups, numGroups, in, out, inStride, outStride, stream) : Launch<F, 32, 1, PK>(groups, numGroups, in, out, inStride, outStride, stream);
			else return hipErrorNotSupported;
			}
#endif
		}

		hipError_t LaunchSpecLite(const WnFrameGroup* groups, int numGroups, const float* in, float* out, long inStride, long outStride, int n, int spb, bool packed,
			hipStream_t stream, bool oneTilePerWave = false, bool beyondCache = false);
		hipError_t LaunchSpecA2(const WnFrameGroup* groups, int numGroups, const float* in, float* out, long inStride, long outStride, int n, int spb, hipStream_t stream,
			bool beyondCache = false);
		hipError_t LaunchSpecA2Table(const WnFrameGroup* groups, int numGroups, const float* in, float* out, long inStride, long outStride, int n, int spb, hipStream_t stream,
			WnLaunchTable& table);
		hipError_t LaunchSpecLiteTable(const WnFrameGroup* groups, int numGroups, const float* in, float* out, long inStride, long outStride, int n, int spb, bool packed,
			hipStream_t stream, WnLaunchTable& table);
	}
}
```

### neuralaudio_amd/csrc/wavenet_spec_kernels.hip

```cpp
#include "wavenet_spec_impl.h"

namespace na
{
	static int& SpecSwitch()
	{
		static int on = Tuning::Get().wnSpecOff ? 0 : 1;
		return on;
	}
	bool WaveNetSpecEnabled() { return SpecSwitch() != 0; }
	void SetWaveNetSpecEnabled(bool on) { SpecSwitch() = on ? 1 : 0; }

	int WaveNetSpecArchId(const WnSplitStage* stages, int nstages, int stateF4, int wsplitQuads)
	{
		if (spk::Matches<spk::ArchStd>(stages, nstages, stateF4, wsplitQuads)) return WN_SPEC_STD;
		if (spk::Matches<spk::ArchLite>(stages, nstages, stateF4, wsplitQuads)) return WN_SPEC_LITE;
		if (spk::Matches<spk::ArchLite16>(stages, nstages, stateF4, wsplitQuads)) return WN_SPEC_LITE16;
		if (spk::Matches<spk::ArchA2Full>(stages, nstages, stateF4, wsplitQuads)) return WN_SPEC_A2FULL;
		if (spk::Matches<spk::ArchA2Lite>(stages, nstages, stateF4, wsplitQuads)) return WN_SPEC_A2LITE;
		return WN_SPEC_NONE;
	}

	hipError_t LaunchWaveNetSpecTable(const WnFrameGroup* groups, int numGroups, const float* in, float* out, long inStride, long outStride, int n,
		hipStream_t stream, WnLaunchTable& table)
	{
#ifdef NA_SP_QUICK
		return hipErrorNotSupported;
#else
		if (numGroups <= WN_FRAME_MAX_GROUPS || (n != 128 && n != 64) || !WaveNetSpecEnabled() || Tuning::Get().spSpb > 0) return hipErrorNotSupported;
		const int arch = groups[0].model->spec_arch;
		const bool lite = arch == WN_SPEC_LITE || arch == WN_SPEC_LITE16, a2 = arch == WN_SPEC_A2FULL || arch == WN_SPEC_A2LITE;
		if (arch != WN_SPEC_STD && !lite && !a2) return hipErrorNotSupported;
		bool packed = false;
		long streams = 0, slots2 = 0;
		for (int i = 0; i < numGroups; i++)
		{
			const int a = groups[i].model->spec_arch;
			const bool same = lite ? (a == WN_SPEC_LITE || a == WN_SPEC_LITE16) : (a2 ? (a == WN_SPEC_A2FULL || a == WN_SPEC_A2LITE) : a == WN_SPEC_STD);
			if (groups[i].numStreams <= 0 || !same) return hipErrorNotSupported;
			packed = packed || groups[i].pack > 1;
			const int per2 = a == WN_SPEC_A2LITE ? 4 : 2;
			streams += groups[i].numStreams;
			slots2 += (groups[i].numStreams + per2 - 1) / per2 * per2;
		}
		if (!lite && packed) return hipErrorNotSupported;
		if (packed)
			for (int i = 0; i < numGroups; i++)
				if (groups[i].slots == nullptr) return hipErrorNotSupported;
		if (!packed)
			for (int i = 0; i < numGroups; i++)
				if (groups[i].model->spec_arch == WN_SPEC_LITE16) return hipErrorNotSupported;
		const int spb = (slots2 * 4 > streams * 5) ? 1 : 2;
		if (a2) return spk::LaunchSpecA2Table(groups, numGroups, in, out, inStride, outStride, n, spb, stream, table);
		if (!lite)
		{
			if (n == 64) return spb == 2 ? spk::LaunchTable<spk::FamStd, 64, 2, false>(groups, numGroups, in, out, inStride, outStride, stream, table)
										 : spk::LaunchTable<spk::FamStd, 64, 1, false>(groups, numGroups, in, out, inStride, outStride, stream, table);
			return spb == 2 ? spk::LaunchTable<spk::FamStd, 128, 2, false>(groups, numGroups, in, out, inStride, outStride, stream, table)
							: spk::LaunchTable<spk::FamStd, 128, 1, false>(groups, numGroups, in, out, inStride, outStride, stream, table);
		}
		return spk::LaunchSpecLiteTable(groups, numGroups, in, out, inStride, outStride, n, spb, packed, stream, table);
#endif
	}

	hipError_t LaunchWaveNetSpecFused(const WnFrameGroup* groups, int numGroups, const float* in, float* out, long inStride, long outStride, int n,
		hipStream_t stream, int sharing)
	{
		if (numGroups <= 0 || numGroups > WN_FRAME_MAX_GROUPS || (n != 128 && n != 64 && n != 32)) return hipErrorNotSupported;
		if (!WaveNetSpecEnabled()) return hipErrorNotSupported;
		const int arch = groups[0].model->spec_arch;
		if (arch == WN_SPEC_NONE) return hipErrorNotSupported;
		auto familyOf = [](int a) { return (a == WN_SPEC_LITE || a == WN_SPEC_LITE16) ? 1 : ((a == WN_SPEC_A2FULL || a == WN_SPEC_A2LITE) ? 2 : 0); };
		const int fam = familyOf(arch);
		bool packed = false, lite16 = false;
		for (int i = 0; i < numGroups; i++)
		{
			const int a = groups[i].model->spec_arch;
			if (groups[i].numStreams <= 0 || a == WN_SPEC_NONE || familyOf(a) != fam || (fam == 0 && a != arch)) return hipErrorNotSupported;
			packed = packed || groups[i].pack > 1;
			lite16 = lite16 || a == WN_SPEC_LITE16;
		}
		if (packed)
			for (int i = 0; i < numGroups; i++)
				if (groups[i].slots == nullptr) return hipErrorNotSupported;
		const int spbEnv = Tuning::Get().spSpb;
		const int residentHalf = 2 * CurrentDeviceCUs();
		int halfGroups = 0;
		for (int i = 0; i < numGroups; i++)
		{
			const int per = groups[i].model->spec_arch == WN_SPEC_A2LITE ? 2 : 1;
			halfGroups += (groups[i].numStreams + per - 1) / per;
		}
		const bool beyondCache = (sharing & WN_SHARING_BEYOND_CACHE) != 0;
		sharing &= ~WN_SHARING_BEYOND_CACHE;
		const int spb = spbEnv > 0 ? spbEnv : (halfGroups * std::max(sharing, 1) > residentHalf ? 2 : 1);
#ifdef NA_SP_QUICK
		if (arch != WN_SPEC_STD || packed) return hipErrorNotSupported;
		return spk::LaunchNF<spk::FamStd, false>(groups, numGroups, in, out, inStride, outStride, n, spb, stream);
#else
		if (fam == 0) return packed ? hipErrorNotSupported : spk::LaunchNF<spk::FamStd, false>(groups, numGroups, in, out, inStride, outStride, n, spb, stream, beyondCache);
		if (fam == 2) return packed ? hipErrorNotSupported : spk::LaunchSpecA2(groups, numGroups, in, out, inStride, outStride, n, spb, stream, beyondCache);
		if (!packed && lite16) return hipErrorNotSupported;
		const bool noT1 = Tuning::Get().spNoT1;
		bool all16 = packed && !noT1;
		int virtualStreams = 0;
		for (int i = 0; i < numGroups; i++)
		{
			all16 = all16 && groups[i].model->spec_arch == WN_SPEC_LITE16;
			virtualStreams += groups[i].numStreams;
		}
		const bool t1 = all16 && spbEnv == 0 && virtualStreams <= CurrentDeviceCUs();
		return spk::LaunchSpecLite(groups, numGroups, in, out, inStride, outStride, n, spb, packed, stream, t1, beyondCache);
#endif
	}
}
```

Before: 3667.

## Issue per-wave vmem loads/stores and exact waitcnts in spec WaveNet chain

Ring history loads and ring stores are now issued only by the waves that actually need them, instead of using dummy out-of-bounds buffer ops. Each wave then waits with a vmem counter matching the number of ops it really issued, and ring publishes move to after the tap loop. Folded K=3 layers stage only the operand quads they read, and the conv tap merges the history and LDS halves before a single MFMA. The intent is less memory traffic, shorter waitcnt stalls and fewer MFMAs, at the cost of heavy template logic where a miscounted waitcnt could cause races. A debug API exposing the per-wave vmem table is added.

```diff
diff --git a/include/neuralaudio_amd.h b/include/neuralaudio_amd.h
--- a/include/neuralaudio_amd.h
+++ b/include/neuralaudio_amd.h
@@ -164,6 +164,7 @@
 NA_EXTERN int NA_DebugPackedWeights(NeuralModel* model, int* packFactor, float* out, int capacity);
 NA_EXTERN int NA_DebugSplitPlan(NeuralModel* model, int* stages, int stageCapacity, unsigned short* wsplit, long long wsplitCapacity, long long* wsplitCount);
 NA_EXTERN void NA_DebugSetWaveNetSpec(int on);
+NA_EXTERN int NA_DebugChainVmem(int frames, int streamsPerWorkgroup, int* out, int capacity);
 NA_EXTERN int NA_DebugSetRecurrentQuadMin(int streams);
 NA_EXTERN long long NA_DebugRecurrentQuadLaunches(void);
 NA_EXTERN int NA_DebugRecurrentPlan(NeuralModel* model, int out[6]);
diff --git a/neuralaudio_amd/capi.py b/neuralaudio_amd/capi.py
--- a/neuralaudio_amd/capi.py
+++ b/neuralaudio_amd/capi.py
@@ -32,6 +32,7 @@
     "NA_BatchReserveStreams", "NA_BatchActivateStream", "NA_BatchParkStream", "NA_BatchIsParked", "NA_BatchFindParked", "NA_BatchNumParked",
     "NA_DebugDeviceResourceCalls", "NA_DebugRecurrentPlan", "NA_DebugRecurrentShapePlan",
     "NA_BatchEnableOutputStage", "NA_BatchSetStreamGain", "NA_BatchGetStreamGain", "NA_BatchHandover", "NA_BatchHandoverRemaining",
+    "NA_DebugChainVmem",
 ]
 
 
@@ -127,6 +128,7 @@
         "NA_BatchStreamKernelName": (C.c_char_p, [vp, C.c_int]),
         "NA_DebugSetTraceBuffer": (None, [vp]),
         "NA_DebugSetWaveNetSpec": (None, [C.c_int]),
+        "NA_DebugChainVmem": (C.c_int, [C.c_int, C.c_int, C.POINTER(C.c_int), C.c_int]),
         "NA_DebugSetRcclApi": (None, [C.c_int, C.c_int, C.c_int]),
         "NA_DebugSetRecurrentQuadMin": (C.c_int, [C.c_int]),
         "NA_DebugRecurrentQuadLaunches": (C.c_longlong, []),
diff --git a/neuralaudio_amd/csrc/capi.cpp b/neuralaudio_amd/csrc/capi.cpp
--- a/neuralaudio_amd/csrc/capi.cpp
+++ b/neuralaudio_amd/csrc/capi.cpp
@@ -929,6 +929,7 @@
 
 #ifndef NA_RELEASE
 void NA_DebugSetWaveNetSpec(int on) { na::SetWaveNetSpecEnabled(on != 0); }
+int NA_DebugChainVmem(int frames, int streamsPerWorkgroup, int* out, int capacity) { return na::WaveNetSpecVmemTable(frames, streamsPerWorkgroup, out, capacity); }
 #endif
 
 #ifndef NA_RELEASE
diff --git a/neuralaudio_amd/csrc/wavenet_launch.h b/neuralaudio_amd/csrc/wavenet_launch.h
--- a/neuralaudio_amd/csrc/wavenet_launch.h
+++ b/neuralaudio_amd/csrc/wavenet_launch.h
@@ -137,6 +137,7 @@
 	bool WaveNetSpecEnabled();
 	void SetWaveNetSpecEnabled(bool on);
 	int WaveNetSpecArchId(const WnSplitStage* stages, int nstages, int stateF4, int wsplitQuads);
+	int WaveNetSpecVmemTable(int nf, int spb, int* out, int capacity);
 
 	hipError_t LaunchWaveNetGeneric(const WnPrewarmLayer* layers, int numLayers, const float* weights, const int* ringOffF4, const int* ringFrames,
 		const int* ringG, int nrings, int stateF4, int maxChannels, float headScale, float condLimit, bool saturate, float* state, const int* slots, const int* rows,
diff --git a/neuralaudio_amd/csrc/wavenet_spec_impl.h b/neuralaudio_amd/csrc/wavenet_spec_impl.h
--- a/neuralaudio_amd/csrc/wavenet_spec_impl.h
+++ b/neuralaudio_amd/csrc/wavenet_spec_impl.h
@@ -380,13 +380,20 @@
 			return (int)__builtin_elementwise_min(a, a - (unsigned)(R * GP * 16));
 		}
 
+		template <class C, int RG>
+		constexpr bool HistIssued(int wr, int shift, int i)
+		{
+			return WaveTapClass<C>(wr, Geo<C::TB::RingG(RG), C::T>::P, i, shift, SmallRing<C, RG>()) != TAP_LDS;
+		}
+
 		template <class C, int RG, int WR>
 		__device__ __forceinline__ u32x4 HistLoadAt(const Ctx& cx, unsigned laneRing, int fl, int shift, int i)
 		{
 			typedef typename C::TB TB;
 			constexpr int GP = TB::RingG(RG), P = Geo<GP, C::T>::P, R = TB::RingFrames(RG), OFF = TB::RingOff(RG);
 			const int cls = WaveTapClass<C>(WR, P, i, shift, SmallRing<C, RG>());
-			if ((NA_ABL & 4) || cls == TAP_LDS) return RingLoad(cx.srsrc, OOB);
+			if (cls == TAP_LDS) return u32x4{ 0, 0, 0, 0 };
+			if (NA_ABL & 4) return RingLoad(cx.srsrc, OOB);
 			const int pos0 = __builtin_amdgcn_readlane(cx.myPos, RG);
 			int base = pos0 - shift + C::FW * cx.wave + 16 * P * i;
 			if (base < 0) base += R;
@@ -406,19 +413,16 @@
 		template <class C, int L>
 		constexpr int ShiftOf(int k) { return C::TB::Dil(L) * (C::TB::KS(L) - 1 - k); }
 
-		template <class C, int GP>
-		constexpr bool HistNeededAt(int shift, int i, bool small) { return !small && TapClassOf(0, Geo<GP, C::T>::P, i, shift) != TAP_LDS; }
-
 		template <class C, int L>
 		constexpr int PrefetchTaps() { return (C::TB::KS(L) - 1) < C::HPF ? (C::TB::KS(L) - 1) : C::HPF; }
 		template <class C, int L>
-		constexpr int HistLoadsOf()
+		constexpr int HistLoadsOf(int wr)
 		{
 			typedef typename C::TB TB;
 			constexpr int GP = TB::GPof(TB::ArrOf(L)), S = Geo<GP, C::T>::S;
 			int n = 0;
 			for (int k = 0; k < PrefetchTaps<C, L>(); k++)
-				for (int i = 0; i < S; i++) n += HistNeededAt<C, GP>(ShiftOf<C, L>(k), i, SmallRing<C, L>()) ? 1 : 0;
+				for (int i = 0; i < S; i++) n += HistIssued<C, L>(wr, ShiftOf<C, L>(k), i) ? 1 : 0;
 			return n;
 		}
 
@@ -430,34 +434,53 @@
 			for (int k = 0; k < PrefetchTaps<C, L>(); k++)
 #pragma unroll
 				for (int i = 0; i < S; i++)
-					if (HistNeededAt<C, GP>(ShiftOf<C, L>(k), i, SmallRing<C, L>())) st.hist[k][i] = HistLoadAt<C, L, WR>(cx, laneRing, fl, ShiftOf<C, L>(k), i);
+					if (HistIssued<C, L>(WR, ShiftOf<C, L>(k), i)) st.hist[k][i] = HistLoadAt<C, L, WR>(cx, laneRing, fl, ShiftOf<C, L>(k), i);
 		}
 
 		template <class C, int RG>
-		constexpr bool StoreNeeded(int i)
+		constexpr bool StoreIssued(int w, int i)
 		{
 			typedef typename C::TB TB;
 			constexpr int P = Geo<TB::RingG(RG), C::T>::P, KEEP = TB::RingKeep(RG);
-			return (C::NF - C::FW) + 16 * P * (i + 1) - 1 >= C::NF - KEEP;
+			return !(NA_ABL & 4) && C::FW * w + 16 * P * (i + 1) - 1 >= C::NF - KEEP;
 		}
 		template <class C, int RG>
-		constexpr int StoresOf()
+		constexpr int StoresOf(int w)
 		{
 			constexpr int S = Geo<C::TB::RingG(RG), C::T>::S;
 			int n = 0;
-			for (int i = 0; i < S; i++) n += StoreNeeded<C, RG>(i) ? 1 : 0;
+			for (int i = 0; i < S; i++) n += StoreIssued<C, RG>(w, i) ? 1 : 0;
 			return n;
 		}
+		template <class C, int RG>
+		constexpr int FirstStoreWave(int i) { int w = 0; while (w < C::WPS && !StoreIssued<C, RG>(w, i)) w++; return w; }
+		template <class C, int RG>
+		constexpr int FirstWaveWithStores(int n) { int w = 0; while (w < C::WPS && StoresOf<C, RG>(w) < n) w++; return w; }
+		constexpr unsigned AllWaves(int wps) { return (1u << wps) - 1u; }
+		template <class C, int RG>
+		constexpr int MinStores(unsigned mask) { int m = 1 << 20; for (int w = 0; w < C::WPS; w++) if ((mask >> w) & 1u) m = StoresOf<C, RG>(w) < m ? StoresOf<C, RG>(w) : m; return m; }
+		template <class C, int RG>
+		constexpr int MaxStores(unsigned mask) { int m = 0; for (int w = 0; w < C::WPS; w++) if ((mask >> w) & 1u) m = StoresOf<C, RG>(w) > m ? StoresOf<C, RG>(w) : m; return m; }
 
 		template <class C, int RG, int GP, int MINSHIFT>
-		__device__ __forceinline__ void Publish(const Ctx& cx, const Lanes<C, GP>& ln, u32x4 v, int i, int imgWrite)
+		__device__ __forceinline__ void LdsPublish(const Lanes<C, GP>& ln, u32x4 v, int i, int imgWrite)
+		{
+			constexpr int P = Geo<GP, C::T>::P;
+			if (!(NA_ABL & 64) && MINSHIFT < C::NF)
+				LdsWrite16(ln.img + (unsigned)(imgWrite * C::IMG_ONE + 16 * P * i * 16), v);
+		}
+
+		template <class C, int RG, int GP, unsigned MASK>
+		__device__ __forceinline__ void RingPublish(const Ctx& cx, const Lanes<C, GP>& ln, u32x4 v, int i)
 		{
 			typedef typename C::TB TB;
 			constexpr int P = Geo<GP, C::T>::P, R = TB::RingFrames(RG), OFF = TB::RingOff(RG), KEEP = TB::RingKeep(RG);
 			static_assert(GP == TB::RingG(RG), "lane mode of the receiving ring");
-			if (!(NA_ABL & 64) && MINSHIFT < C::NF)
-				LdsWrite16(ln.img + (unsigned)(imgWrite * C::IMG_ONE + 16 * P * i * 16), v);
-			if ((NA_ABL & 4) || !StoreNeeded<C, RG>(i)) return;
+			bool any = false, all = true;
+			for (int w = 0; w < C::WPS; w++)
+				if ((MASK >> w) & 1u) { any = any || StoreIssued<C, RG>(w, i); all = all && StoreIssued<C, RG>(w, i); }
+			if (!any) return;
+			if (!all && cx.wave < FirstStoreWave<C, RG>(i)) return;
 			const int pos0 = __builtin_amdgcn_readlane(cx.myPos, RG);
 			int base;
 			if constexpr (TB::CompactRing(RG))
@@ -482,6 +505,13 @@
 			}
 			if (KEEP >= C::NF) RingStore(cx.srsrc, v, addr, OFF * 16);
 			else RingStore(cx.srsrc, v, (C::FW * cx.wave + 16 * P * i + ln.fl >= C::NF - KEEP) ? addr : OOB, OFF * 16);
+		}
+
+		template <class C, int RG, int GP, int MINSHIFT, unsigned MASK>
+		__device__ __forceinline__ void Publish(const Ctx& cx, const Lanes<C, GP>& ln, u32x4 v, int i, int imgWrite)
+		{
+			LdsPublish<C, RG, GP, MINSHIFT>(ln, v, i, imgWrite);
+			RingPublish<C, RG, GP, MASK>(cx, ln, v, i);
 		}
 
 		template <class C, int RG, int GP>
@@ -522,13 +552,29 @@
 			static constexpr int QUADS = (TB::ChunkEnd(SN, CN) - TB::ChunkBegin(SN, CN)) * 64;
 			static constexpr int SRC = TB::AOff(SN) + TB::ChunkBegin(SN, CN) * 64;
 			static constexpr int BUF = TB::ChunkIndex(SN, CN) & 1;
-			static constexpr int NCOPY = (QUADS + C::STG_THREADS - 1) / C::STG_THREADS;
+			static constexpr int LYR = TB::LayerOfStage(SN) < 0 ? 0 : TB::LayerOfStage(SN);
+			static constexpr bool FOLDED = TB::LayerOfStage(SN) >= 0 && LayerSig<C, LYR>::FOLD;
+			static constexpr int NREAD = (TB::LastOfArr(LYR) && TB::ArrOf(LYR) == TB::NA - 1) ? 5 : 7;
+			static constexpr unsigned READ_OPS = 0x8754210u;
+			static constexpr int NWAVES = C::STG_THREADS / 64;
+			static constexpr int NCOPY = FOLDED ? (NREAD + NWAVES - 1) / NWAVES : (QUADS + C::STG_THREADS - 1) / C::STG_THREADS;
+			static_assert(!FOLDED || (TB::NumChunks(SN) == 1 && TB::StageOps(SN) == 10), "folded operands: a K = 3 layer in one chunk");
 			static __device__ __forceinline__ void Begin(const Ctx& cx)
 			{
 				if (NA_ABL & 16) return;
 #pragma unroll
 				for (int c = 0; c < NCOPY; c++)
 				{
+					if constexpr (FOLDED)
+					{
+						const int j = c * NWAVES + cx.stgWave;
+						const bool mine = j < NREAD;
+						const int i0 = (int)((READ_OPS >> (4 * (j & 7))) & 15u) * 64;
+						const unsigned dst = mine ? cx.wbuf + (unsigned)(BUF * C::WBUF_ONE) + (unsigned)i0 * 16u : (unsigned)C::DUMP_OFF;
+						__builtin_amdgcn_raw_ptr_buffer_load_lds(cx.wrsrc, (__attribute__((address_space(3))) void*)(LdsPtr)(size_t)dst, 16,
+							mine ? (SRC + i0 + cx.lane) * 16 : OOB, 0, 0, 0);
+						continue;
+					}
 					const int i0 = c * C::STG_THREADS + cx.stgWave * 64;
 					const bool mine = i0 < QUADS;
 					const unsigned dst = mine ? cx.wbuf + (unsigned)(BUF * C::WBUF_ONE) + (unsigned)i0 * 16u : (unsigned)C::DUMP_OFF;
@@ -542,6 +588,34 @@
 				__builtin_amdgcn_s_waitcnt((LATER & 15) | ((LATER >> 4) << 14) | (7 << 4) | (15 << 8));
 			}
 		};
+		template <class C, int RG>
+		constexpr int EndImmediate(unsigned mask, int loads, int w)
+		{
+			if constexpr (RG < 0) return loads;
+			else
+			{
+				for (int n = MaxStores<C, RG>(mask); n > MinStores<C, RG>(mask); n--)
+					if (w >= FirstWaveWithStores<C, RG>(n)) return loads + n;
+				return loads + MinStores<C, RG>(mask);
+			}
+		}
+		template <class C, class NS, int RG, unsigned MASK, int LOADS, int N>
+		__device__ __forceinline__ void EndCountedFrom(const Ctx& cx)
+		{
+			if constexpr (N <= MinStores<C, RG>(MASK)) NS::template End<LOADS + N>();
+			else
+			{
+				if (cx.wave >= FirstWaveWithStores<C, RG>(N)) NS::template End<LOADS + N>();
+				else EndCountedFrom<C, NS, RG, MASK, LOADS, N - 1>(cx);
+			}
+		}
+		template <class C, class NS, int RG, unsigned MASK, int LOADS>
+		__device__ __forceinline__ void EndCounted(const Ctx& cx)
+		{
+			if constexpr (RG < 0) NS::template End<LOADS>();
+			else EndCountedFrom<C, NS, RG, MASK, LOADS, MaxStores<C, RG>(MASK)>(cx);
+		}
+
 		template <class C, int s, int c>
 		struct NextChunk
 		{
@@ -603,18 +677,14 @@
 		{
 			constexpr int P = Geo<GP, C::T>::P;
 			const int cls = WaveTapClass<C>(WR, P, i, shift, SmallRing<C, RG>());
-			th = u32x2{ 0, 0 };
-			if (cls != TAP_LDS)
-			{
-				acc = Mfma(ah, hist, acc);
-				th = u32x2{ hist.x, hist.y };
-			}
+			u32x4 b = hist;
 			if (cls != TAP_HIST)
 			{
-				const u32x4 b = TapLds<C, GP>(cx, ln, imgRead, shift, i, cls);
-				acc = Mfma(ah, b, acc);
-				th = cls == TAP_LDS ? u32x2{ b.x, b.y } : u32x2{ th.x | b.x, th.y | b.y };
-			}
+				b = TapLds<C, GP>(cx, ln, imgRead, shift, i, cls);
+				if (cls == TAP_BOTH) b = u32x4{ b.x | hist.x, b.y | hist.y, b.z | hist.z, b.w | hist.w };
+			}
+			acc = Mfma(ah, b, acc);
+			th = u32x2{ b.x, b.y };
 			return acc;
 		}
 
@@ -630,7 +700,8 @@
 			constexpr int NEXTMINSHIFT = SG::NEXT ? TB::Dil(LN) : (1 << 20);
 			constexpr bool OWN = 2 * (K - 1) >= CB && 2 * (K - 1) < CE;
 			constexpr bool TAIL = 2 * K >= CB && 2 * K < CE;
-			constexpr int LATER = ((OWN && SG::NEXT) ? HistLoadsOf<C, LN>() : 0) + ((TAIL && SG::NEXT && !LASTLAYER) ? StoresOf<C, LN>() : 0);
+			constexpr unsigned MASK = SG::MaskOf(WR);
+			constexpr int LOADS = (OWN && SG::NEXT) ? HistLoadsOf<C, LN>(WR) : 0, STRING = (TAIL && SG::NEXT && !LASTLAYER) ? LN : -1;
 			typedef typename NextChunk<C, s, c>::St NextStager;
 			if constexpr (c == 0)
 			{
@@ -652,7 +723,7 @@
 				if (k < C::HPF) continue;
 #pragma unroll
 				for (int i = 0; i < S; i++)
-					if (WaveTapClass<C>(WR, SG::P, i, ShiftOf<C, L>(k), SmallRing<C, L>()) != TAP_LDS) hx[k - (KLO > C::HPF ? KLO : C::HPF)][i] = HistLoadAt<C, L, WR>(cx, ln.ring, ln.fl, ShiftOf<C, L>(k), i);
+					if (HistIssued<C, L>(WR, ShiftOf<C, L>(k), i)) hx[k - (KLO > C::HPF ? KLO : C::HPF)][i] = HistLoadAt<C, L, WR>(cx, ln.ring, ln.fl, ShiftOf<C, L>(k), i);
 			}
 			static_assert(!SG::FOLD || (NCH == 1 && K == 3), "folded operands: K = 3 layers in one chunk");
 			u32x2 th[SG::FOLD ? 2 : 1][S];
@@ -664,7 +735,7 @@
 				for (int i = 0; i < S; i++)
 				{
 					u32x4 h = u32x4{ 0, 0, 0, 0 };
-					if (WaveTapClass<C>(WR, SG::P, i, ShiftOf<C, L>(k), SmallRing<C, L>()) != TAP_LDS)
+					if (HistIssued<C, L>(WR, ShiftOf<C, L>(k), i))
 						h = (k < C::HPF) ? st.hist[k < C::HPF ? k : 0][i] : hx[k >= C::HPF ? k - (KLO > C::HPF ? KLO : C::HPF) : 0][i];
 					if constexpr (SG::FOLD) acc[i] = ConvTapFold<C, L, GP, WR>(cx, ln, imgRead, ShiftOf<C, L>(k), i, ah, h, acc[i], th[k < 2 ? k : 0][i]);
 					else acc[i] = ConvTap<C, L, GP, WR>(cx, ln, imgRead, ShiftOf<C, L>(k), i, ah, al, h, acc[i]);
@@ -727,13 +798,18 @@
 						if constexpr (SG::NEXT)
 						{
 							st.xs[i] = Split<C>(y, cx);
-							Publish<C, LN, GP, NEXTMINSHIFT>(cx, ln, st.xs[i], i, imgWrite);
+							LdsPublish<C, LN, GP, NEXTMINSHIFT>(ln, st.xs[i], i, imgWrite);
 						}
 					}
 				}
+				if constexpr (STRING >= 0)
+				{
+#pragma unroll
+					for (int i = 0; i < S; i++) RingPublish<C, STRING < 0 ? LN : STRING, GP, MASK>(cx, ln, st.xs[i], i);
+				}
 				SPK_STAMP(s, 3);
 			}
-			NextStager::template End<LATER>();
+			EndCounted<C, NextStager, STRING, MASK, LOADS>(cx);
 			SPK_STAMP(s, 4);
 			BlockBarrier<C::NTHREADS / 64>();
 			if constexpr (c + 1 < NCH) LayerChunk<C, L, WR, c + 1>(cx, ln, st, ax, acc);
@@ -769,25 +845,41 @@
 			}
 		}
 
-		template <class C, int L, int W>
-		__device__ __forceinline__ void FirstHistDispatch(const Ctx& cx, unsigned laneRing, int fl, State& st)
+		template <class C, int L>
+		constexpr bool FirstHistSame(int W)
 		{
 			typedef typename C::TB TB;
 			constexpr int GP = TB::GPof(TB::ArrOf(L)), P = Geo<GP, C::T>::P, S = Geo<GP, C::T>::S;
+			bool r = true;
+			for (int w = W + 1; w < C::WPS; w++)
+				for (int k = 0; k < PrefetchTaps<C, L>(); k++)
+					for (int i = 0; i < S; i++) r = r && WaveTapClass<C>(w, P, i, ShiftOf<C, L>(k), SmallRing<C, L>()) == WaveTapClass<C>(W, P, i, ShiftOf<C, L>(k), SmallRing<C, L>());
+			return r;
+		}
+		template <class C, int L>
+		constexpr int FirstHistRep(int w) { int W = 0; while (W < w && !FirstHistSame<C, L>(W)) W++; return W; }
+		template <class C, int L>
+		constexpr unsigned FirstHistMask(int W) { return FirstHistSame<C, L>(W) ? AllWaves(C::WPS) & ~AllWaves(W) : 1u << W; }
+
+		template <class C, int L, int W, int SN>
+		__device__ __forceinline__ void FirstHistDispatch(const Ctx& cx, unsigned laneRing, int fl, State& st)
+		{
 			if constexpr (W < C::WPS)
 			{
-				constexpr bool same = [] {
-					bool r = true;
-					for (int w = W + 1; w < C::WPS; w++)
-						for (int k = 0; k < PrefetchTaps<C, L>(); k++)
-							for (int i = 0; i < S; i++) r = r && WaveTapClass<C>(w, P, i, ShiftOf<C, L>(k), SmallRing<C, L>()) == WaveTapClass<C>(W, P, i, ShiftOf<C, L>(k), SmallRing<C, L>());
-					return r;
-				}();
-				if constexpr (same) HistPrefetch<C, L, W>(cx, laneRing, fl, st);
+				constexpr bool same = FirstHistSame<C, L>(W);
+				if constexpr (same)
+				{
+					HistPrefetch<C, L, W>(cx, laneRing, fl, st);
+					EndCounted<C, Stager<C, SN, 0>, L, FirstHistMask<C, L>(W), HistLoadsOf<C, L>(W)>(cx);
+				}
 				else
 				{
-					if (cx.wave == W) HistPrefetch<C, L, W>(cx, laneRing, fl, st);
-					else FirstHistDispatch<C, L, W + 1>(cx, laneRing, fl, st);
+					if (cx.wave == W)
+					{
+						HistPrefetch<C, L, W>(cx, laneRing, fl, st);
+						EndCounted<C, Stager<C, SN, 0>, L, FirstHistMask<C, L>(W), HistLoadsOf<C, L>(W)>(cx);
+					}
+					else FirstHistDispatch<C, L, W + 1, SN>(cx, laneRing, fl, st);
 				}
 			}
 		}
@@ -808,11 +900,10 @@
 				st.xc[i] = x;
 				st.hd[i] = f32x4{ 0.0f, 0.0f, 0.0f, 0.0f };
 				st.xs[i] = Split<C>(x, cx);
-				Publish<C, 0, GP, C::TB::Dil(0)>(cx, ln, st.xs[i], i, 1);
-			}
-			FirstHistDispatch<C, 0, 0>(cx, ln.ring, ln.fl, st);
+				Publish<C, 0, GP, C::TB::Dil(0), AllWaves(C::WPS)>(cx, ln, st.xs[i], i, 1);
+			}
 			SPK_STAMP(0, 1); SPK_STAMP(0, 2); SPK_STAMP(0, 3);
-			Stager<C, 1, 0>::template End<StoresOf<C, 0>() + HistLoadsOf<C, 0>()>();
+			FirstHistDispatch<C, 0, 0, 1>(cx, ln.ring, ln.fl, st);
 			SPK_STAMP(0, 4);
 			BlockBarrier<C::NTHREADS / 64>();
 			SPK_STAMP(0, 5);
@@ -858,11 +949,10 @@
 				st.hd[i] = hn[i];
 				st.xc[i] = xn[i];
 				st.xs[i] = Split<C>(xn[i], cx);
-				Publish<C, LN, GPN, TB::Dil(LN)>(cx, ln, st.xs[i], i, (s + 1) & 1);
-			}
-			FirstHistDispatch<C, LN, 0>(cx, ln.ring, ln.fl, st);
+				Publish<C, LN, GPN, TB::Dil(LN), AllWaves(C::WPS)>(cx, ln, st.xs[i], i, (s + 1) & 1);
+			}
 			SPK_STAMP(s, 1); SPK_STAMP(s, 2); SPK_STAMP(s, 3);
-			Stager<C, s + 1, 0>::template End<StoresOf<C, LN>() + HistLoadsOf<C, LN>()>();
+			FirstHistDispatch<C, LN, 0, s + 1>(cx, ln.ring, ln.fl, st);
 			SPK_STAMP(s, 4);
 			BlockBarrier<C::NTHREADS / 64>();
 			SPK_STAMP(s, 5);
@@ -896,7 +986,7 @@
 					if (c == 0)
 					{
 #pragma unroll
-						for (int i = 0; i < S; i++) Publish<C, RG, GP, 1>(cx, ln, hs[i], i, imgHead);
+						for (int i = 0; i < S; i++) Publish<C, RG, GP, 1, AllWaves(C::WPS)>(cx, ln, hs[i], i, imgHead);
 						BlockBarrier<C::NTHREADS / 64>();
 					}
 #pragma unroll
@@ -908,7 +998,7 @@
 						for (int i = 0; i < S; i++)
 						{
 							u32x4 h = u32x4{ 0, 0, 0, 0 };
-							if (WaveTapClass<C>(WR, P, i, K - 1 - k, SmallRing<C, RG>()) != TAP_LDS) h = HistLoadAt<C, RG, WR>(cx, ln.ring, ln.fl, K - 1 - k, i);
+							if (HistIssued<C, RG>(WR, K - 1 - k, i)) h = HistLoadAt<C, RG, WR>(cx, ln.ring, ln.fl, K - 1 - k, i);
 							acc[i] = ConvTap<C, RG, GP, WR>(cx, ln, imgHead, K - 1 - k, i, ah, al, h, acc[i]);
 						}
 					}
@@ -1269,6 +1359,57 @@
 			}
 		}
 
+		template <class C, int s>
+		static void VmemRows(int* out)
+		{
+			typedef typename C::TB TB;
+			static_assert(TB::HEADK == 1, "dense head");
+			if constexpr (s < TB::NSTAGES)
+			{
+				constexpr int L = TB::LayerOfStage(s);
+				static_assert(TB::NumChunks(s) == 1, "one-chunk stages");
+				for (int w = 0; w < C::WPS; w++)
+				{
+					int loads = 0, stores = 0, dma = 0, later = -1;
+					if constexpr (s == TB::NSTAGES - 1) {}
+					else if constexpr (L >= 0)
+					{
+						typedef LayerSig<C, L> SG;
+						dma = Stager<C, s + 1, 0>::NCOPY;
+						later = 0;
+						if constexpr (SG::NEXT)
+						{
+							const int wr = SG::Rep(w);
+							loads = HistLoadsOf<C, L + 1>(wr);
+							stores = StoresOf<C, L + 1>(w);
+							later = EndImmediate<C, L + 1>(SG::MaskOf(wr), loads, w);
+						}
+					}
+					else
+					{
+						constexpr int LN = s == 0 ? 0 : TB::LayerOfStage(s + 1);
+						const int wr = FirstHistRep<C, LN>(w);
+						dma = Stager<C, s + 1, 0>::NCOPY;
+						loads = HistLoadsOf<C, LN>(wr);
+						stores = StoresOf<C, LN>(w);
+						later = EndImmediate<C, LN>(FirstHistMask<C, LN>(wr), loads, w);
+					}
+					int* r = out + (s * C::WPS + w) * 4;
+					r[0] = loads; r[1] = stores; r[2] = dma; r[3] = later;
+				}
+				VmemRows<C, s + 1>(out);
+			}
+		}
+		template <class C>
+		static int VmemTable(int* out, int capacity)
+		{
+			const int rows = C::TB::NSTAGES * C::WPS;
+			if (out == nullptr) return rows;
+			if (capacity < rows * 4) return -1;
+			VmemRows<C, 0>(out);
+			return rows;
+		}
+
 		template <class A>
 		static bool Matches(const WnSplitStage* st, int nstages, int stateF4, int wsplitQuads)
 		{
diff --git a/neuralaudio_amd/csrc/wavenet_spec_kernels.hip b/neuralaudio_amd/csrc/wavenet_spec_kernels.hip
--- a/neuralaudio_amd/csrc/wavenet_spec_kernels.hip
+++ b/neuralaudio_amd/csrc/wavenet_spec_kernels.hip
@@ -18,6 +18,15 @@
 		if (spk::Matches<spk::ArchA2Full>(stages, nstages, stateF4, wsplitQuads)) return WN_SPEC_A2FULL;
 		if (spk::Matches<spk::ArchA2Lite>(stages, nstages, stateF4, wsplitQuads)) return WN_SPEC_A2LITE;
 		return WN_SPEC_NONE;
+	}
+
+	int WaveNetSpecVmemTable(int nf, int spb, int* out, int capacity)
+	{
+		if (spb != 1 && spb != 2) return -1;
+		if (nf == 128) return spb == 2 ? spk::VmemTable<spk::Cfg<spk::ArchStd, 128, 2, false>>(out, capacity) : spk::VmemTable<spk::Cfg<spk::ArchStd, 128, 1, false>>(out, capacity);
+		if (nf == 64) return spb == 2 ? spk::VmemTable<spk::Cfg<spk::ArchStd, 64, 2, false>>(out, capacity) : spk::VmemTable<spk::Cfg<spk::ArchStd, 64, 1, false>>(out, capacity);
+		if (nf == 32) return spb == 2 ? spk::VmemTable<spk::Cfg<spk::ArchStd, 32, 2, false>>(out, capacity) : spk::VmemTable<spk::Cfg<spk::ArchStd, 32, 1, false>>(out, capacity);
+		return -1;
 	}
 
 	hipError_t LaunchWaveNetSpecTable(const WnFrameGroup* groups, int numGroups, const float* in, float* out, long inStride, long outStride, int n,
```

After: 3818, median of 4. 1.04x the previous value.
